# robustrobotics/flame

Measured on AMD Instinct MI355X. Metric: NLTGV2 primal-dual iters/sec on 640x480 Delaunay graph; depth RMS vs CPU, higher is better.
Workload: dtype f32

## Files before the change

flame_amd/csrc/flame_nltgv2_test_options.h:

```cpp
#ifndef FLAME_NLTGV2_TEST_OPTIONS_H_
#define FLAME_NLTGV2_TEST_OPTIONS_H_

enum {
  FLAME_NLTGV2_OPT_BLOCK_WAVES = 103,
  FLAME_NLTGV2_OPT_UNROLL = 104,
  FLAME_NLTGV2_OPT_DUAL_PUBLISH = 106,
  FLAME_NLTGV2_OPT_PRESLEEP = 108,
  FLAME_NLTGV2_OPT_XCDS = 109,
  FLAME_NLTGV2_OPT_FAULT_INJECT = 110,
  FLAME_NLTGV2_OPT_POLL_GAP = 113
};

#endif
```

flame_amd/csrc/nltgv2_context.hip:

```cpp
#include "nltgv2_context.hpp"

namespace flame_hip {
namespace host {

int fail(flame_nltgv2_ctx* ctx, int status) {
  if (ctx) ctx->last_error = status;
  return status;
}

void request_open_stop(flame_nltgv2_ctx* ctx) {
  if (!ctx->open_inflight || ctx->open_stop_sent || !ctx->stop_dev.p || !ctx->ctl_stream) return;
  *ctx->h_stop = ctx->open_tag0;
  if (hipMemcpyAsync(ctx->stop_dev.p, ctx->h_stop, sizeof(unsigned), hipMemcpyHostToDevice, ctx->ctl_stream) != hipSuccess) (void)hipGetLastError();
  ctx->open_stop_sent = true;
}

hipError_t wait_solver_stream(flame_nltgv2_ctx* ctx) {
  request_open_stop(ctx);
  return hipStreamSynchronize(ctx->stream);
}

int ensure(flame_nltgv2_ctx* ctx, DevBuf& b, size_t bytes) {
  if (bytes == 0) bytes = 16;
  if (b.cap >= bytes) return 0;
// ... 170 lines not shown
  const size_t lanes = (size_t)L.wg_count * kWave;
  const size_t fV = sizeof(float) * (size_t)V, fE = sizeof(float) * (size_t)E, iV = sizeof(int32_t) * (size_t)V;
  struct { DevBuf* b; size_t bytes; } req[] = {
      {&ctx->pos, 2 * fV}, {&ctx->src, fE}, {&ctx->dst, fE},
      {&ctx->row_ptr, sizeof(int32_t) * ((size_t)V + 1)}, {&ctx->half, 2 * fE},
      {&ctx->slice_row, sizeof(int32_t) * ((size_t)L.n_slices + 1)}, {&ctx->perm, sizeof(int32_t) * n_packed},
      {&ctx->pdeg, sizeof(int32_t) * n_packed}, {&ctx->iperm, iV}, {&ctx->order_m, iV}, {&ctx->rid_of, iV},
      {&ctx->rec_nbr, sizeof(uint32_t) * n_slots}, {&ctx->rec_edge, sizeof(int32_t) * n_slots}, {&ctx->edge_src_slot, fE},
      {&ctx->hrec, sizeof(int4) * n_slots}, {&ctx->hq, sizeof(float4) * n_slots},
      {&ctx->vstate, sizeof(float4) * n_packed}, {&ctx->vaux, sizeof(float2) * n_packed},
      {&ctx->hq_alt, sizeof(float4) * n_slots}, {&ctx->vstate_alt, sizeof(float4) * n_packed}, {&ctx->photo_err, fV},
      {&ctx->bar0, sizeof(float4) * n_packed}, {&ctx->bar1, sizeof(float4) * n_packed},
      {&ctx->vprev, sizeof(float4) * n_packed}, {&ctx->xbuf, kXbufBytesPerVertex * records_capacity(L) + 64},
      {&ctx->wg_v0, sizeof(int32_t) * n_wg_v0},
      {&ctx->wg_vfirst, n_wg_vfirst + 16}, {&ctx->abort_flag, sizeof(int)}, {&ctx->err, kErrBytes}, {&ctx->cost_out, 2 * sizeof(float)},
      {&ctx->wg_slot, sizeof(int32_t) * lanes}, {&ctx->wg_vid, sizeof(int32_t) * lanes}, {&ctx->wg_meta, sizeof(uint32_t) * lanes},
      {&ctx->wg_nbr, sizeof(int32_t) * lanes}, {&ctx->wg_fetch, sizeof(int32_t) * lanes},
      {&ctx->wg_info, sizeof(int32_t) * n_wg_info}};
  for (auto& r : req) {
    const int rc = ensure(ctx, *r.b, r.bytes);
    if (rc) return rc;
  }
  if (want_e2) {
    const size_t lanes2 = (size_t)L.wg2_count * kWave;
    struct { DevBuf* b; size_t bytes; } req2[] = {
        {&ctx->wg2_info, sizeof(int32_t) * n_wg2_info}, {&ctx->wg2_vfirst, n_wg2_vfirst + 16}, {&ctx->wg2_rmax, 64},
        {&ctx->wg2_slot, sizeof(int32_t) * 2 * lanes2}, {&ctx->wg2_nbr, sizeof(int32_t) * 2 * lanes2}, {&ctx->wg2_vid, sizeof(int32_t) * lanes2},
        {&ctx->wg2_meta, sizeof(uint32_t) * lanes2}, {&ctx->wg2_fetch, sizeof(int32_t) * lanes2}};
    for (auto& r : req2) {
      const int rc = ensure(ctx, *r.b, r.bytes);
      if (rc) return rc;
    }
  }
  ctx->topo++;
  ctx->layout_pos_saved = false;
  ctx->tv_built = ctx->wg2_built = false;
  drop_graphs(ctx);
  refresh_args(ctx);
  return 0;
}

void expansion_fills(const PackedLayout& L, void* rec_edge, void* rec_nbr, void* wg2_rmax, std::vector<StageFill>* fills) {
  fills->push_back(StageFill{(char*)rec_edge + sizeof(int32_t) * (size_t)L.rows * kWave, sizeof(int32_t) * kRowPad * kWave, 0xffffffffu});
  fills->push_back(StageFill{(char*)rec_nbr + sizeof(uint32_t) * (size_t)L.rows * kWave, sizeof(uint32_t) * kRowPad * kWave, 0u});
  if (wg2_rmax) fills->push_back(StageFill{wg2_rmax, 64, 0u});
}

void topology_fills(flame_nltgv2_ctx* ctx, bool want_e2, std::vector<StageFill>* fills, bool early) {
  const PackedLayout& L = ctx->L;
  const size_t n_slots = (size_t)(L.rows + kRowPad) * kWave, n_packed = (size_t)L.n_slices * kWave;
  const StageFill base[] = {
      {ctx->err.p, kErrBytes, 0u}, {ctx->abort_flag.p, sizeof(int), 0u}, {ctx->xbuf.p, kXbufBytesPerVertex * records_capacity(L) + 64, 0u},
      {ctx->hq_alt.p, sizeof(float4) * n_slots, 0u}, {ctx->vstate_alt.p, sizeof(float4) * n_packed, 0u}};
  fills->insert(fills->end(), base, base + sizeof(base) / sizeof(base[0]));
  if (!early) expansion_fills(L, ctx->rec_edge.p, ctx->rec_nbr.p, want_e2 ? ctx->wg2_rmax.p : nullptr, fills);
  if (ctx->place_base) {
    fills->push_back(StageFill{ctx->place_base, (size_t)2 * kPlacePages * 4096, 0u});
    fills->push_back(StageFill{(int*)ctx->place_fill.p + 2 * kPlacePages, 64, 0u});
  }
}

bool placement_applies(const flame_nltgv2_ctx* ctx, const PackedLayout& L) {
  return L.wg_ok && ctx->place_state == 1 && ctx->opt_place && L.wg_count > 2 * (ctx->prop.multiProcessorCount / 8) &&
         (ctx->opt_xcds == 0 || ctx->opt_xcds == 8);
}

ExpandTables live_tables(flame_nltgv2_ctx* ctx) {
  ExpandTables t;
  t.c = ctx->c, t.f = ctx->f;
  t.iperm = (const int32_t*)ctx->iperm.p, t.wg_v0 = (const int32_t*)ctx->wg_v0.p, t.order_m = (const int32_t*)ctx->order_m.p;
  t.rid_of = (const int32_t*)ctx->rid_of.p, t.wg_vfirst = (const uint8_t*)ctx->wg_vfirst.p;
  t.wg2_info = (int32_t*)ctx->wg2_info.p, t.wg2_vfirst = (const uint8_t*)ctx->wg2_vfirst.p;
  t.wg2_slot = (int32_t*)ctx->wg2_slot.p, t.wg2_vid = (int32_t*)ctx->wg2_vid.p, t.wg2_nbr = (int32_t*)ctx->wg2_nbr.p;
  t.wg2_fetch = (int32_t*)ctx->wg2_fetch.p, t.wg2_meta = (uint32_t*)ctx->wg2_meta.p, t.wg2_rmax = (int*)ctx->wg2_rmax.p;
  return t;
}

int expand_launches(flame_nltgv2_ctx* ctx, const PackedLayout& L, const ExpandTables& t, bool want_e2, hipStream_t stream) {
  LAUNCHCHK(ctx, launch_build_sell(t.c, t.f, t.iperm, stream));
  if (L.wg_ok) LAUNCHCHK(ctx, launch_build_patches(t.c, t.f, t.wg_v0, t.order_m, t.rid_of, t.wg_vfirst, t.iperm, stream));
  if (want_e2)
    LAUNCHCHK(ctx, launch_build_patches2(t.c, t.f, L.wg2_count, t.wg2_info, t.order_m, t.rid_of, t.wg2_vfirst, t.iperm, t.wg2_slot, t.wg2_vid,
                                         t.wg2_meta, t.wg2_nbr, t.wg2_fetch, t.wg2_rmax, stream));
  if (t.rec_off)
    LAUNCHCHK(ctx, launch_place_records(t.c, t.f, t.per_xcd, t.order_m, t.rid_of, t.place_patch, (int8_t*)(t.place_patch + t.stride),
                                        (const uint16_t*)ctx->place_rank.p, kPlacePages, t.place_fill, t.rec_off, (int)t.stride, stream));
  return 0;
}

int topology_expand(flame_nltgv2_ctx* ctx, bool want_e2, bool launched) {
  const PackedLayout& L = ctx->L;
  if (!launched) {
    const int rc = expand_launches(ctx, L, live_tables(ctx), want_e2, ctx->stream);
    if (rc) return rc;
  }
  ctx->pv2_args = Pv2Args{};
  ctx->wg2_usable = false;
  if (want_e2) {
    ctx->pv2_args.slot = (const int32_t*)ctx->wg2_slot.p, ctx->pv2_args.vid = (const int32_t*)ctx->wg2_vid.p;
    ctx->pv2_args.meta = (const uint32_t*)ctx->wg2_meta.p, ctx->pv2_args.nbr = (const int32_t*)ctx->wg2_nbr.p;
    ctx->pv2_args.fetch = (const int32_t*)ctx->wg2_fetch.p, ctx->pv2_args.info = (const int32_t*)ctx->wg2_info.p;
    ctx->pv2_args.count = L.wg2_count, ctx->pv2_args.lcap = L.wg2_lcap;
    if (ctx->pv2_occ == 0 || ctx->pv2_occ_lcap != L.wg2_lcap)
      ctx->pv2_occ = pv2_patches_per_cu(L.wg2_lcap, false), ctx->pv2_occ_verify = pv2_patches_per_cu(L.wg2_lcap, true), ctx->pv2_occ_lcap = L.wg2_lcap;
    ctx->wg2_built = true;
  }
  if (!launched && placement_applies(ctx, L)) {
    refresh_args(ctx);
    const int rc = place_records(ctx, (L.wg_count + 7) / 8);
    if (rc) return rc;
  }
  ctx->pending = flame_nltgv2_ctx::PendingRun{};
  ctx->tag_next = 1;
  ctx->xbuf_form = 0;
  ctx->static_stale = false;
  return 0;
}

bool wants_e2(const flame_nltgv2_ctx* ctx) { return wants_e2(ctx, ctx->L); }
bool wants_e2(const flame_nltgv2_ctx* ctx, const PackedLayout& L) {
  const int cus = ctx->prop.multiProcessorCount;
  const int64_t est_patches = L.wg_rowpack ? (int64_t)L.wg_count : ((static_cast<int64_t>(2) * L.E + L.V / 32) / 54 + 1);
  return L.wg_ok && L.max_degree <= 32 && ctx->opt_probe == 0 &&
         (ctx->opt_persistent == 6 || (ctx->opt_persistent == 1 && est_patches > (int64_t)kPv2FromPerCu * cus));
}

int upload_topology(flame_nltgv2_ctx* ctx, const flame_nltgv2_graph* g, const StageCopy* extra, size_t n_extra, bool long_lived) {
  const int32_t V = g->V, E = g->E;
  (void)long_lived;
  int rc = cancel_prepared(ctx);
  if (!rc) rc = wait_raster(ctx);
  if (rc) return rc;
  rc = build_layout(g, &ctx->L, false, true,
                        ctx->opt_persistent == 4 ? 0x7fffffff : kPvDensePerCu * ctx->prop.multiProcessorCount);
  if (rc) return fail(ctx, rc);
  if (ctx->L.wg_ok && ctx->L.wg_rowpack && ctx->opt_persistent != 4 && ctx->L.wg_count > kPvDensePerCu * ctx->prop.multiProcessorCount) {
    rc = build_layout(g, &ctx->L, false, false, 0);
    if (rc) return fail(ctx, rc);
  }
  bool want_e2 = wants_e2(ctx);
  if (want_e2) {
    build_patch_walk2(&ctx->L);
    want_e2 = ctx->L.wg2_ok && ctx->L.wg2_count <= kPv2WavesPerCu * ctx->prop.multiProcessorCount * 4;
  }
  const PackedLayout& L = ctx->L;
  rc = topology_buffers(ctx, want_e2, L.wg_info.size(), L.wg_v0.size(), L.wg_vfirst.size(), L.wg2_info.size(), L.wg2_vfirst.size());
  if (rc) return rc;
  const size_t n_packed = (size_t)L.n_slices * kWave;
  const size_t fV = sizeof(float) * (size_t)V, fE = sizeof(float) * (size_t)E, iV = sizeof(int32_t) * (size_t)V;
  std::vector<StageCopy> cp = {
      {&ctx->pos, g->pos, 2 * fV}, {&ctx->src, g->src, fE}, {&ctx->dst, g->dst, fE},
      {&ctx->row_ptr, L.row_ptr.data(), sizeof(int32_t) * ((size_t)V + 1)}, {&ctx->half, L.half.data(), 2 * fE},
      {&ctx->slice_row, L.slice_row.data(), sizeof(int32_t) * ((size_t)L.n_slices + 1)},
      {&ctx->perm, L.perm.data(), sizeof(int32_t) * n_packed}, {&ctx->pdeg, L.pdeg.data(), sizeof(int32_t) * n_packed},
      {&ctx->iperm, L.iperm.data(), iV}, {&ctx->order_m, L.order_m.data(), iV}, {&ctx->rid_of, L.rid_of.data(), iV},
      {&ctx->wg_info, L.wg_info.data(), sizeof(int32_t) * L.wg_info.size()},
      {&ctx->wg_v0, L.wg_v0.data(), sizeof(int32_t) * L.wg_v0.size()},
      {&ctx->wg_vfirst, L.wg_vfirst.data(), L.wg_vfirst.size()}};
  if (want_e2) {
    cp.push_back(StageCopy{&ctx->wg2_info, L.wg2_info.data(), sizeof(int32_t) * L.wg2_info.size()});
    cp.push_back(StageCopy{&ctx->wg2_vfirst, L.wg2_vfirst.data(), L.wg2_vfirst.size()});
  }
  cp.insert(cp.end(), extra, extra + n_extra);
  std::vector<StageFill> fills;
  topology_fills(ctx, want_e2, &fills);
  rc = staged_h2d(ctx, cp.data(), cp.size(), fills.data(), fills.size());
  if (rc) return rc;
  rc = topology_expand(ctx, want_e2);
  if (rc) return rc;
  ctx->h_src.assign(g->src, g->src + E);
  ctx->h_dst.assign(g->dst, g->dst + E);
  ctx->host_layout_valid = true;
  ctx->feat_dev_valid = false;
  HIPCHK(ctx, hipEventRecord(ctx->ev_topo_ready, ctx->stream));
  return 0;
}

int ensure_form_rows(flame_nltgv2_ctx* ctx, int form) {
  PackedLayout& L = ctx->L;
  if ((form == 4 && !ctx->wg2_built) || (form == 2 && !ctx->tv_built)) {
    const int rc = ensure_host_layout(ctx);
    if (rc) return rc;
  }
  if (form == 4 && !ctx->wg2_built) {
    build_patch_rows2(&L);
    ctx->pv2_args = Pv2Args{};
    if (L.wg2_ok) {
      struct { DevBuf* b; const void* src; size_t bytes; } cp[] = {
          {&ctx->wg2_slot, L.wg2_slot.data(), sizeof(int32_t) * L.wg2_slot.size()}, {&ctx->wg2_vid, L.wg2_vid.data(), sizeof(int32_t) * L.wg2_vid.size()},
          {&ctx->wg2_meta, L.wg2_meta.data(), sizeof(uint32_t) * L.wg2_meta.size()}, {&ctx->wg2_nbr, L.wg2_nbr.data(), sizeof(int32_t) * L.wg2_nbr.size()},
          {&ctx->wg2_fetch, L.wg2_fetch.data(), sizeof(int32_t) * L.wg2_fetch.size()}, {&ctx->wg2_info, L.wg2_info.data(), sizeof(int32_t) * L.wg2_info.size()}};
// ... 9 lines not shown
      ctx->pv2_args.count = L.wg2_count, ctx->pv2_args.lcap = L.wg2_lcap;
      ctx->pv2_occ = pv2_patches_per_cu(L.wg2_lcap, false), ctx->pv2_occ_verify = pv2_patches_per_cu(L.wg2_lcap, true), ctx->pv2_occ_lcap = L.wg2_lcap;
    }
    ctx->wg2_built = true;
    ctx->wg2_usable = L.wg2_ok, ctx->wg2_checked_topo = ctx->topo;
  }
  if (form == 2 && !ctx->tv_built) {
    build_tv_rows(&L);
    struct { DevBuf* b; const void* src; size_t bytes; } cp[] = {
        {&ctx->tv_slot, L.tv_slot.data(), sizeof(int32_t) * L.tv_slot.size()}, {&ctx->tv_vid, L.tv_vid.data(), sizeof(int32_t) * L.tv_vid.size()},
        {&ctx->tv_meta, L.tv_meta.data(), sizeof(uint32_t) * L.tv_meta.size()}, {&ctx->tv_wave, L.tv_wave.data(), sizeof(uint32_t) * L.tv_wave.size()}};
    HIPCHK(ctx, wait_solver_stream(ctx));
    for (auto& c : cp) {
      int rc = ensure(ctx, *c.b, c.bytes);
      if (!rc) rc = h2d(ctx, *c.b, c.src, c.bytes);
      if (rc) return rc;
    }
    HIPCHK(ctx, wait_solver_stream(ctx));
    ctx->tv_built = true;
    refresh_args(ctx);
  }
  return 0;
}

bool params_ok(const flame_nltgv2_params* p) { return p != nullptr; }

}
}

extern "C" {

int flame_nltgv2_abi_version(void) { return FLAME_NLTGV2_ABI_VERSION; }

void flame_nltgv2_default_params(flame_nltgv2_params* p) {
  if (!p) return;
  p->data_factor = 0.1f, p->step_x = 0.001f, p->step_q = 125.0f;
  p->theta = 0.25f, p->x_min = 0.0f, p->x_max = 10.0f;
}

const char* flame_nltgv2_status_string(int status) {
  switch (status) {
    case FLAME_NLTGV2_OK: return "ok";
    case FLAME_NLTGV2_ERR_INVALID_ARG: return "invalid argument";
    case FLAME_NLTGV2_ERR_NO_DEVICE: return "no usable HIP device";
    case FLAME_NLTGV2_ERR_HIP: return "HIP runtime error";
    case FLAME_NLTGV2_ERR_NO_GRAPH: return "no graph uploaded";
    case FLAME_NLTGV2_ERR_NAN: return "dual variable became NaN/Inf (reference FLAME_ASSERT, h:174)";
    case FLAME_NLTGV2_ERR_OOM: return "out of device memory";
    case FLAME_NLTGV2_ERR_TIMEOUT: return "persistent run: neighbour wait timed out";
    case FLAME_NLTGV2_ERR_ASSERT: return "input on which the reference asserts (FLAME_ASSERT)";
    default: return "unknown status";
  }
}

int flame_nltgv2_create(flame_nltgv2_ctx** out, int device) {
  if (!out) return FLAME_NLTGV2_ERR_INVALID_ARG;
  *out = nullptr;
  int count = 0;
  if (hipGetDeviceCount(&count) != hipSuccess || count <= 0) return FLAME_NLTGV2_ERR_NO_DEVICE;
  if (device < 0 || device >= count) return FLAME_NLTGV2_ERR_NO_DEVICE;
  flame_nltgv2_ctx* ctx = new (std::nothrow) flame_nltgv2_ctx();
  if (!ctx) return FLAME_NLTGV2_ERR_OOM;
  ctx->device = device;
  bool ok = hipSetDevice(device) == hipSuccess;
  ok = ok && hipGetDeviceProperties(&ctx->prop, device) == hipSuccess;
  int prio_least = 0, prio_greatest = 0;
  ok = ok && hipDeviceGetStreamPriorityRange(&prio_least, &prio_greatest) == hipSuccess;
  ok = ok && hipStreamCreateWithPriority(&ctx->own_stream, hipStreamNonBlocking, prio_greatest) == hipSuccess;
  ok = ok && hipEventCreate(&ctx->ev0) == hipSuccess && hipEventCreate(&ctx->ev1) == hipSuccess;
  ok = ok && hipStreamCreateWithFlags(&ctx->topo_stream, hipStreamNonBlocking) == hipSuccess;
  ok = ok && hipStreamCreateWithFlags(&ctx->raster_stream, hipStreamNonBlocking) == hipSuccess;
  ok = ok && hipEventCreateWithFlags(&ctx->ev_canon, hipEventDisableTiming) == hipSuccess;
  ok = ok && hipEventCreateWithFlags(&ctx->ev_snap, hipEventDisableTiming) == hipSuccess;
  ok = ok && hipEventCreateWithFlags(&ctx->ev_raster_done, hipEventDisableTiming) == hipSuccess;
  ok = ok && hipEventCreateWithFlags(&ctx->ev_topo_ready, hipEventDisableTiming) == hipSuccess;
  ok = ok && hipEventCreate(&ctx->ev_mesh0) == hipSuccess && hipEventCreate(&ctx->ev_mesh1) == hipSuccess;
  ok = ok && hipEventCreate(&ctx->ev_dbg0) == hipSuccess && hipEventCreate(&ctx->ev_dbg1) == hipSuccess;
  ok = ok && hipEventCreateWithFlags(&ctx->ev_expanded, hipEventDisableTiming) == hipSuccess;
  ok = ok && hipEventCreateWithFlags(&ctx->ev_run[0], hipEventDisableTiming) == hipSuccess;
  ok = ok && hipEventCreateWithFlags(&ctx->ev_run[1], hipEventDisableTiming) == hipSuccess;
  ok = ok && hipHostMalloc((void**)&ctx->h_err, kErrBytes, hipHostMallocDefault) == hipSuccess;
  ok = ok && hipHostMalloc((void**)&ctx->h_cost, 2 * sizeof(float), hipHostMallocDefault) == hipSuccess;
  ok = ok && hipHostMalloc((void**)&ctx->h_stop, 64, hipHostMallocDefault) == hipSuccess;
  if (ctx->h_stop) *ctx->h_stop = 0u;
  ok = ok && hipStreamCreateWithPriority(&ctx->ctl_stream, hipStreamNonBlocking, -1) == hipSuccess;
  if (!ok) {
    flame_nltgv2_destroy(ctx);
    return FLAME_NLTGV2_ERR_HIP;
  }
  ctx->stream = ctx->own_stream;
  *ctx->h_err = 0;
  {
    static std::once_flag warm;
    if (!std::getenv("FLAME_NLTGV2_NO_WARM"))
    std::call_once(warm, [ctx] {
      warm_module_kernels(), warm_module_persistent(ctx->own_stream, cooperative_allowed()), warm_module_persistent_tv(), warm_module_persistent_pv2();
      warm_module_layout(), warm_module_topo();
    });
    if (!std::getenv("FLAME_NLTGV2_LAZY_CALIBRATION") && ctx->prop.multiProcessorCount >= 64 && place_calibrate_at_create(device) && place_calibrate(ctx) != 0) {
      ctx->last_error = 0, ctx->last_hip = 0;
      (void)hipGetLastError();
    }
    if (ctx->place_state < 0) ctx->place_state = 0;
  }
  ctx->all = {&ctx->pos, &ctx->x, &ctx->w1, &ctx->w2, &ctx->xb, &ctx->w1b, &ctx->w2b, &ctx->xp, &ctx->w1p,
              &ctx->w2p, &ctx->data, &ctx->weight, &ctx->src, &ctx->dst, &ctx->alpha, &ctx->beta, &ctx->q1,
              &ctx->q2, &ctx->q3, &ctx->row_ptr, &ctx->half, &ctx->slice_row, &ctx->perm, &ctx->pdeg,
              &ctx->rec_nbr, &ctx->rec_edge, &ctx->edge_src_slot, &ctx->hrec, &ctx->hq, &ctx->vstate, &ctx->hq_alt, &ctx->vstate_alt, &ctx->cost_terms, &ctx->run_tail,
              &ctx->vaux, &ctx->bar0, &ctx->bar1, &ctx->vprev, &ctx->xbuf, &ctx->abort_flag, &ctx->tv_slot, &ctx->tv_vid, &ctx->tv_meta, &ctx->tv_wave, &ctx->wg2_slot, &ctx->wg2_vid, &ctx->wg2_meta, &ctx->wg2_nbr, &ctx->wg2_fetch, &ctx->wg2_info, &ctx->wg2_vfirst, &ctx->wg2_rmax, &ctx->err,
              &ctx->cost_out, &ctx->img_ref, &ctx->img_cmp, &ctx->photo_err, &ctx->r_tris, &ctx->r_valid, &ctx->r_tvalid, &ctx->r_keys,
              &ctx->r_img, &ctx->r_cov, &ctx->r_vtx, &ctx->r_val, &ctx->wg_slot, &ctx->wg_vid, &ctx->wg_meta, &ctx->wg_nbr,
              &ctx->wg_fetch, &ctx->wg_info, &ctx->wg_v0, &ctx->probe, &ctx->snap_hq, &ctx->snap_vstate, &ctx->snap_bar, &ctx->iperm,
              &ctx->order_m, &ctx->rid_of, &ctx->stage[0].d, &ctx->stage[1].d, &ctx->sync_init, &ctx->sync_vmap, &ctx->sync_emap, &ctx->sync_need,
              &ctx->wg_vfirst, &ctx->place_pool, &ctx->place_rank, &ctx->place_fill, &ctx->place_rec_off, &ctx->place_patch, &ctx->place_meas, &ctx->progress};
  for (DevBuf* b : {&ctx->feat_stamp_d, &ctx->feat_key_d, &ctx->feat_val_d, &ctx->topo_scratch, &ctx->topo_dims, &ctx->layout_pos}) ctx->all.push_back(b);
  for (auto& b : ctx->nx) ctx->all.push_back(&b);
  for (auto& b : ctx->ex) ctx->all.push_back(&b);
  ctx->all.push_back(&ctx->pos_undo);
  for (DevBuf* b : {&ctx->m_P, &ctx->m_idepth, &ctx->m_normals, &ctx->m_tvalid, &ctx->m_nvalid, &ctx->m_tnormal, &ctx->m_offset, &ctx->m_cursor,
                    &ctx->m_incident, &ctx->m_keys, &ctx->m_img, &ctx->m_cov})
    ctx->all.push_back(b);
  for (DevBuf* b : {&ctx->d_gray, &ctx->d_idimg, &ctx->d_nimg, &ctx->d_w1map, &ctx->d_w2map, &ctx->d_keys, &ctx->d_cov}) ctx->all.push_back(b);
  ctx->all.push_back(&ctx->stop_dev);
  ctx->all.push_back(&ctx->place_patch_nx), ctx->all.push_back(&ctx->place_fill_nx);
  for (auto& b : ctx->sp_v) ctx->all.push_back(&b);
  for (auto& b : ctx->sp_q) ctx->all.push_back(&b);
  for (auto& b : ctx->sp_ab) ctx->all.push_back(&b);
  *out = ctx;
  return FLAME_NLTGV2_OK;
}

int flame_nltgv2_destroy(flame_nltgv2_ctx* ctx) {
  if (!ctx) return FLAME_NLTGV2_OK;
  (void)hipSetDevice(ctx->device);
  request_open_stop(ctx);
  if (ctx->stream) (void)hipStreamSynchronize(ctx->stream);
  place_pool_release(ctx);
  drop_graphs(ctx);
  for (DevBuf* b : ctx->all)
    if (b->p) (void)hipFree(b->p);
  if (ctx->h_err) (void)hipHostFree(ctx->h_err);
  if (ctx->h_cost) (void)hipHostFree(ctx->h_cost);
  if (ctx->h_keep) (void)hipHostFree(ctx->h_keep);
  if (ctx->h_stop) (void)hipHostFree(ctx->h_stop);
  if (ctx->ctl_stream) (void)hipStreamSynchronize(ctx->ctl_stream), (void)hipStreamDestroy(ctx->ctl_stream);
  for (auto& st : ctx->stage)
    if (st.h) (void)hipHostFree(st.h);
  if (ctx->topo_stream) (void)hipStreamSynchronize(ctx->topo_stream), (void)hipStreamDestroy(ctx->topo_stream);
  if (ctx->ev_topo_ready) (void)hipEventDestroy(ctx->ev_topo_ready);
  if (ctx->ev_expanded) (void)hipEventDestroy(ctx->ev_expanded);
  if (ctx->raster_stream) (void)hipStreamSynchronize(ctx->raster_stream), (void)hipStreamDestroy(ctx->raster_stream);
  if (ctx->ev_canon) (void)hipEventDestroy(ctx->ev_canon);
  if (ctx->ev_snap) (void)hipEventDestroy(ctx->ev_snap);
  if (ctx->ev_raster_done) (void)hipEventDestroy(ctx->ev_raster_done);
  for (hipEvent_t e : ctx->ev_run)
    if (e) (void)hipEventDestroy(e);
  if (ctx->h_img) (void)hipHostFree(ctx->h_img);
  if (ctx->h_mesh) (void)hipHostFree(ctx->h_mesh);
  if (ctx->ev_mesh0) (void)hipEventDestroy(ctx->ev_mesh0);
  if (ctx->ev_mesh1) (void)hipEventDestroy(ctx->ev_mesh1);
  if (ctx->h_dbg) (void)hipHostFree(ctx->h_dbg);
  if (ctx->ev_dbg0) (void)hipEventDestroy(ctx->ev_dbg0);
  if (ctx->ev_dbg1) (void)hipEventDestroy(ctx->ev_dbg1);
  if (ctx->h_dims) (void)hipHostFree(ctx->h_dims);
  if (ctx->ev0) (void)hipEventDestroy(ctx->ev0);
  if (ctx->ev1) (void)hipEventDestroy(ctx->ev1);
  if (ctx->own_stream) (void)hipStreamDestroy(ctx->own_stream);
  delete ctx;
  return FLAME_NLTGV2_OK;
}

int flame_nltgv2_set_stream(flame_nltgv2_ctx* ctx, void* hip_stream) {
  int rc = enter(ctx);
  if (rc) return rc;
  HIPCHK(ctx, wait_solver_stream(ctx));
  ctx->stream = hip_stream ? (hipStream_t)hip_stream : ctx->own_stream;
  return FLAME_NLTGV2_OK;
}

int flame_nltgv2_set_option(flame_nltgv2_ctx* ctx, int option, int value) {
  if (!ctx) return FLAME_NLTGV2_ERR_INVALID_ARG;
  switch (option) {
    case FLAME_NLTGV2_OPT_SOLVER:
      if (value != 0 && value != 1) return fail(ctx, FLAME_NLTGV2_ERR_INVALID_ARG);
      ctx->opt_solver = value;
      return 0;
    case FLAME_NLTGV2_OPT_USE_HIPGRAPH:
      ctx->opt_use_graph = value ? 1 : 0;
      return 0;
    case FLAME_NLTGV2_OPT_BLOCK_WAVES:
      if (value != 0 && value != 1 && value != 2 && value != 4) return fail(ctx, FLAME_NLTGV2_ERR_INVALID_ARG);
      ctx->opt_block_waves = value;
      return 0;
    case FLAME_NLTGV2_OPT_PERSISTENT:
      if (value < 0 || value > 6 || value == 2 || value == 5) return fail(ctx, FLAME_NLTGV2_ERR_INVALID_ARG);
      ctx->opt_persistent = value;
      return 0;
    case FLAME_NLTGV2_OPT_PLACEMENT:
      if (value < 0 || value > 1) return fail(ctx, FLAME_NLTGV2_ERR_INVALID_ARG);
      ctx->opt_place = value;
      return 0;
    case FLAME_NLTGV2_OPT_POLL_GAP:
      if (value < 0 || value > 256) return fail(ctx, FLAME_NLTGV2_ERR_INVALID_ARG);
      ctx->opt_poll_gap = value;
      return 0;
    case FLAME_NLTGV2_OPT_VERIFY_RECORDS:
      if (value < 0 || value > 2) return fail(ctx, FLAME_NLTGV2_ERR_INVALID_ARG);
      ctx->opt_verify = value;
      if (value != 2) ctx->persist_refused_topo = ctx->persist_backoff_topo = ~0ull;
      return 0;
    case FLAME_NLTGV2_OPT_PROBE:
      ctx->opt_probe = value ? 1 : 0;
      return 0;
    case FLAME_NLTGV2_OPT_DUAL_PUBLISH:
      if (value < 0 || value > 2) return fail(ctx, FLAME_NLTGV2_ERR_INVALID_ARG);
      ctx->opt_dual = value;
      return 0;
    case FLAME_NLTGV2_OPT_FAULT_INJECT:
      if (value < 0 || value > (1 << 24)) return fail(ctx, FLAME_NLTGV2_ERR_INVALID_ARG);
      ctx->opt_fault = value;
      if (value == 0) ctx->persist_refused_topo = ctx->persist_backoff_topo = ~0ull;
      return 0;
    case FLAME_NLTGV2_OPT_XCDS:
      if (value < 0 || value > 8) return fail(ctx, FLAME_NLTGV2_ERR_INVALID_ARG);
      ctx->opt_xcds = value;
      ctx->coop_checked_key = ~0ull;
      return 0;
    case FLAME_NLTGV2_OPT_PRESLEEP:
      if (value < 0 || value > 256) return fail(ctx, FLAME_NLTGV2_ERR_INVALID_ARG);
      ctx->opt_presleep = value;
      return 0;
    case FLAME_NLTGV2_OPT_MESH_STATE:
      if (value < 0 || value > 1) return fail(ctx, FLAME_NLTGV2_ERR_INVALID_ARG);
      ctx->opt_mesh_state = value;
      return 0;
    case FLAME_NLTGV2_OPT_COST_SUM:
      if (value < 0 || value > 1) return fail(ctx, FLAME_NLTGV2_ERR_INVALID_ARG);
      ctx->opt_cost_sum = value;
      return 0;
    case FLAME_NLTGV2_OPT_SYNC_PATH:
      if (value < 0 || value > 2) return fail(ctx, FLAME_NLTGV2_ERR_INVALID_ARG);
      ctx->opt_sync_path = value;
      return 0;
    case FLAME_NLTGV2_OPT_UNROLL:
      if (value != 0 && value != 4 && value != 8 && value != 16) return fail(ctx, FLAME_NLTGV2_ERR_INVALID_ARG);
      ctx->opt_unroll = value;
      return 0;
    default:
      return fail(ctx, FLAME_NLTGV2_ERR_INVALID_ARG);
  }
}


int flame_nltgv2_get_info(flame_nltgv2_ctx* ctx, flame_nltgv2_info* info) {
  if (!ctx || !info) return FLAME_NLTGV2_ERR_INVALID_ARG;
  std::memset(info, 0, sizeof(*info));
  info->abi_version = FLAME_NLTGV2_ABI_VERSION;
  info->device = ctx->device;
  info->V = ctx->L.V, info->E = ctx->L.E;
  info->n_slices = ctx->L.n_slices;
  info->max_degree = ctx->L.max_degree;
  info->padded_half_edges = ctx->L.rows * kWave;
  info->device_bytes = (int64_t)ctx->device_bytes;
  info->algorithmic_bytes_per_iter = 64ll * ctx->L.V + 40ll * ctx->L.E;
  info->compute_units = ctx->prop.multiProcessorCount;
  std::snprintf(info->device_name, sizeof(info->device_name), "%s", ctx->prop.name);
  std::snprintf(info->gcn_arch, sizeof(info->gcn_arch), "%s", ctx->prop.gcnArchName);
  info->last_run_path = ctx->last_run_path;
  info->he_waves = 0;
  if (ctx->have_graph && !ctx->tv_built && ctx->tv_counted_topo != ctx->topo) {
    if (ensure_host_layout(ctx) == 0) {
      ctx->L.tv_waves = 0;
      build_tv_rows(&ctx->L);
      ctx->tv_counted_topo = ctx->topo;
    }
  }
  info->tv_waves = ctx->L.tv_ok ? ctx->L.tv_waves : 0;
  info->patches = ctx->L.wg_ok ? ctx->L.wg_count : 0;
  info->tv_wave_capacity = kTvLdsWavesPerCu * ctx->prop.multiProcessorCount;
  info->last_run_groups = ctx->last_run_groups;
  info->timeouts_recovered = ctx->timeouts_recovered;
  info->torn_records_detected = ctx->torn_records_detected;
  info->last_sync_path = ctx->last_sync_path;
// ... 31 lines not shown
  rc = ensure_canon(ctx);
  if (!rc) rc = ensure_host_layout(ctx);
  if (rc) return rc;
  const int32_t V = ctx->L.V, E = ctx->L.E;
  std::vector<float> pos(2 * (size_t)V);
  HIPCHK(ctx, hipMemcpyAsync(pos.data(), ctx->layout_pos_saved ? ctx->layout_pos.p : ctx->pos.p, sizeof(float) * pos.size(), hipMemcpyDeviceToHost, ctx->stream));
  HIPCHK(ctx, wait_solver_stream(ctx));
  flame_nltgv2_graph g{};
  g.V = V, g.E = E, g.pos = pos.data(), g.src = ctx->h_src.data(), g.dst = ctx->h_dst.data();
  PackedLayout H;
  rc = build_layout(&g, &H, true, ctx->L.wg_rowpack);
  if (rc) return fail(ctx, rc);
  int64_t bad = 0;
  auto cmp = [&](const DevBuf& b, const void* host, size_t bytes) -> int {
    if (bytes == 0) return 0;
    std::vector<uint32_t> d(bytes / 4);
    if (hipMemcpy(d.data(), b.p, bytes, hipMemcpyDeviceToHost) != hipSuccess) return 1;
    const uint32_t* h = static_cast<const uint32_t*>(host);
    for (size_t i = 0; i < d.size(); ++i) bad += d[i] != h[i];
    return 0;
  };
  const PackedLayout& L = ctx->L;
  bad += (H.rows != L.rows) + (H.n_slices != L.n_slices) + (H.wg_ok != L.wg_ok) + (H.wg_count != L.wg_count) +
         (H.wg_lcap != L.wg_lcap) + (H.wg_slab_slots != L.wg_slab_slots) + (H.n_rec != L.n_rec) +
         (H.wg_v0 != L.wg_v0) + (H.wg_vfirst != L.wg_vfirst) + (H.wg_rowpack != L.wg_rowpack);
  if (bad == 0) {
    const size_t iV = 4 * (size_t)V;
    int e = cmp(ctx->row_ptr, H.row_ptr.data(), iV + 4) | cmp(ctx->half, H.half.data(), 8 * (size_t)E) | cmp(ctx->order_m, H.order_m.data(), iV) |
            cmp(ctx->rid_of, H.rid_of.data(), iV) | cmp(ctx->iperm, H.iperm.data(), iV) | cmp(ctx->pdeg, H.pdeg.data(), 4 * H.pdeg.size()) |
            cmp(ctx->wg_v0, H.wg_v0.data(), 4 * H.wg_v0.size()) | cmp(ctx->wg_vfirst, H.wg_vfirst.data(), H.wg_vfirst.size() & ~size_t(3));
    if (e) return fail(ctx, FLAME_NLTGV2_ERR_HIP);
    std::vector<int32_t> hs(ctx->h_src.size()), hd(ctx->h_dst.size());
    if (E && (hipMemcpy(hs.data(), ctx->src.p, 4 * (size_t)E, hipMemcpyDeviceToHost) != hipSuccess ||
              hipMemcpy(hd.data(), ctx->dst.p, 4 * (size_t)E, hipMemcpyDeviceToHost) != hipSuccess))
      return fail(ctx, FLAME_NLTGV2_ERR_HIP);
    bad += (hs != ctx->h_src) + (hd != ctx->h_dst);
  }
  if (bad == 0) {
    const size_t n = (size_t)L.rows * kWave, lanes = (size_t)L.wg_count * kWave;
    int e = cmp(ctx->rec_nbr, H.rec_nbr.data(), 4 * n) | cmp(ctx->rec_edge, H.rec_edge.data(), 4 * n) |
            cmp(ctx->edge_src_slot, H.edge_src_slot.data(), 4 * (size_t)E) | cmp(ctx->perm, H.perm.data(), 4 * H.perm.size()) |
            cmp(ctx->slice_row, H.slice_row.data(), 4 * H.slice_row.size());
    if (L.wg_ok)
      e |= cmp(ctx->wg_slot, H.wg_slot.data(), 4 * lanes) | cmp(ctx->wg_vid, H.wg_vid.data(), 4 * lanes) |
           cmp(ctx->wg_meta, H.wg_meta.data(), 4 * lanes) | cmp(ctx->wg_nbr, H.wg_nbr.data(), 4 * lanes) |
           cmp(ctx->wg_fetch, H.wg_fetch.data(), 4 * lanes) | cmp(ctx->wg_info, H.wg_info.data(), 4 * H.wg_info.size());
    if (ctx->wg2_built) {
      build_patch_rows2(&H);
      bad += (H.wg2_ok != L.wg2_ok) + (H.wg2_count != L.wg2_count) + (H.wg2_lcap != L.wg2_lcap) + (H.wg2_vfirst != L.wg2_vfirst);
      if (bad == 0 && H.wg2_ok) {
        const size_t lanes2 = (size_t)H.wg2_count * kWave;
        e |= cmp(ctx->wg2_slot, H.wg2_slot.data(), 8 * lanes2) | cmp(ctx->wg2_nbr, H.wg2_nbr.data(), 8 * lanes2) |
             cmp(ctx->wg2_vid, H.wg2_vid.data(), 4 * lanes2) | cmp(ctx->wg2_meta, H.wg2_meta.data(), 4 * lanes2) |
             cmp(ctx->wg2_fetch, H.wg2_fetch.data(), 4 * lanes2) | cmp(ctx->wg2_info, H.wg2_info.data(), 4 * H.wg2_info.size());
      }
    }
    if (e) return fail(ctx, FLAME_NLTGV2_ERR_HIP);
  }
  if (bad == 0 && ctx->place_state == 1 && ctx->place_topo == ctx->topo && L.wg_ok) {
    const size_t stride = records_capacity(L);
    std::vector<int32_t> off(2 * stride);
    if (hipMemcpy(off.data(), ctx->place_rec_off.p, sizeof(int32_t) * off.size(), hipMemcpyDeviceToHost) != hipSuccess)
      return fail(ctx, FLAME_NLTGV2_ERR_HIP);
    std::vector<int32_t> patch_of_rec((size_t)V, -1);
    for (int32_t q = 0; q < H.wg_count; ++q)
      for (int32_t i = 0; i < (H.wg_info[(size_t)q * 4 + 2] & 0xffff); ++i) patch_of_rec[(size_t)H.wg_info[(size_t)q * 4] + i] = q;
    const int32_t per = ctx->place_per_xcd;
    for (int par = 0; par < 2; ++par) {
      std::vector<int32_t> used;
      for (int32_t u = 0; u < V; ++u) {
        const int32_t r = H.rid_of[(size_t)u], a = patch_of_rec[(size_t)r] / per;
        bool crosses = false;
        for (int32_t h = H.row_ptr[(size_t)u]; h < H.row_ptr[(size_t)u + 1] && !crosses; ++h)
          crosses = patch_of_rec[(size_t)H.rid_of[(size_t)H.half_nbr[(size_t)h]]] / per != a;
        const int32_t o = off[(size_t)par * stride + r];
        bad += crosses != (o >= 0);
        if (o < 0) continue;
        bad += (o & 15) != 0 || o < par * kPlacePages * 4096 || o >= (par + 1) * kPlacePages * 4096;
        used.push_back(o);
      }
      std::sort(used.begin(), used.end());
      for (size_t i = 1; i < used.size(); ++i) bad += used[i] == used[i - 1];
    }
  }
  *mismatches = bad;
  return FLAME_NLTGV2_OK;
}

int flame_nltgv2_placement_info(flame_nltgv2_ctx* ctx, int32_t* state, int32_t* placed_records, float* us) {
  int rc = enter(ctx);
  if (rc) return rc;
  if (state) *state = ctx->place_state;
  if (us) us[0] = ctx->place_best_us, us[1] = ctx->place_mean_us, us[2] = ctx->place_worst_us;
  if (placed_records) {
    *placed_records = 0;
    if (ctx->have_graph && ctx->place_state == 1 && ctx->place_topo == ctx->topo) {
      std::vector<int32_t> off((size_t)ctx->L.V);
      HIPCHK(ctx, hipMemcpyAsync(off.data(), ctx->place_rec_off.p, sizeof(int32_t) * off.size(), hipMemcpyDeviceToHost, ctx->stream));
      HIPCHK(ctx, wait_solver_stream(ctx));
      for (int32_t o : off) *placed_records += o >= 0;
    }
  }
  return FLAME_NLTGV2_OK;
}

int flame_nltgv2_pack_probe(const flame_nltgv2_graph* g, int32_t* perm, int32_t* slice_row, int32_t* rec_nbr,
                            int32_t* rec_edge, int64_t capacity_rows, int64_t* rows_out) {
  PackedLayout L;
  int rc = build_layout(g, &L);
  if (rc) return rc;
  if (rows_out) *rows_out = L.rows;
  if (perm) std::memcpy(perm, L.perm.data(), sizeof(int32_t) * L.perm.size());
  if (slice_row) std::memcpy(slice_row, L.slice_row.data(), sizeof(int32_t) * L.slice_row.size());
  if ((rec_nbr || rec_edge) && capacity_rows < L.rows) return FLAME_NLTGV2_ERR_INVALID_ARG;
  const size_t n = (size_t)L.rows * kWave;
  if (rec_nbr) std::memcpy(rec_nbr, L.rec_nbr.data(), sizeof(int32_t) * n);
  if (rec_edge) std::memcpy(rec_edge, L.rec_edge.data(), sizeof(int32_t) * n);
  return L.n_slices;
}

}
```

flame_amd/csrc/nltgv2_context.hpp:

```cpp
#ifndef FLAME_AMD_NLTGV2_CONTEXT_HPP_
#define FLAME_AMD_NLTGV2_CONTEXT_HPP_

#include <hip/hip_runtime.h>

#include <cstdio>
#include <cstdlib>
#include <cstring>
#include <algorithm>
#include <chrono>
#include <cmath>
#include <new>
#include <memory>
#include <mutex>
#include <functional>
#include <vector>

#include "flame_nltgv2.h"
#include "flame_nltgv2_test_options.h"
#include "nltgv2_kernels.h"
#include "nltgv2_pack.hpp"
#include "roctx_ranges.hpp"

namespace flame_hip {
namespace host {

constexpr int kGraphChunk = 256;
constexpr int kMaxCachedGraphs = 6;
constexpr int kTvLdsWavesPerCu = 16;
constexpr size_t kXbufBytesPerVertex = 8 * 16 + 4;
constexpr int kPv2FromPerCu = 14;
constexpr int kPv2PaceAbovePerCu = 10, kPv2DensePreSleep = 2, kPv2DenseGap = 2;
constexpr int kPv2MaxGroups = 2;
constexpr int kPv2WavesPerCu = 19;
constexpr int kCrowdedWavesPerCu = 16, kCrowdedTopologies = 64;
constexpr int kPvDensePerCu = 27;
constexpr int kPvPaceAbovePerCu = 13;
constexpr int kPvDensePreSleep = 3, kPvDenseGap = 2;
constexpr int kPvPaceMoreAbovePerCu = 23;
constexpr int kPvDenserPreSleep = 5, kPvDenserGap = 4;
constexpr int kPvPreSleep = 0;
constexpr int kPvPollGap = 2;
constexpr int kDualMinWavesPerCu = 0;
constexpr int kPreSleepTv = 2;
constexpr int32_t kFeatDirectMax = 1 << 22;
constexpr size_t kErrBytes = 16 * sizeof(int);
constexpr unsigned kMaxSpins = 1u << 20;

struct DevBuf {
  void* p = nullptr;
  size_t cap = 0;
};

struct CachedGraph {
  hipGraphExec_t exec = nullptr;
  int n = 0, parity = 0, unroll = 0, wpb = 0, gen = 0;
  uint64_t topo = 0;
  flame_nltgv2_params params{};
  uint64_t stamp = 0;
};

class FlatMap {
 public:
  FlatMap() = default;
  explicit FlatMap(size_t n) { reset(n); }
  void reset(size_t n) {
    size_t cap = 16;
    while (cap < 2 * n + 2) cap <<= 1;
    if (cap > slots_.size() || gen_ == 0xffffffffu) {
      slots_.assign(std::max(cap, slots_.size()), Slot{0, 0, 0});
      gen_ = 0;
    }
    mask_ = slots_.size() - 1;
    ++gen_;
  }
  std::pair<int32_t*, bool> emplace(uint64_t k, int32_t v) {
    size_t i = hash(k) & mask_;
    for (;; i = (i + 1) & mask_) {
      Slot& s = slots_[i];
      if (s.gen != gen_) {
        s = Slot{k, v, gen_};
        return {&s.val, true};
      }
      if (s.key == k) return {&s.val, false};
    }
  }
  const int32_t* find(uint64_t k) const {
    size_t i = hash(k) & mask_;
    for (;; i = (i + 1) & mask_) {
      const Slot& s = slots_[i];
      if (s.gen != gen_) return nullptr;
      if (s.key == k) return &s.val;
    }
  }

 private:
  struct Slot {
    uint64_t key;
    int32_t val;
    uint32_t gen;
  };
  static size_t hash(uint64_t z) {
    z = (z ^ (z >> 30)) * 0xbf58476d1ce4e5b9ull;
    z = (z ^ (z >> 27)) * 0x94d049bb133111ebull;
    return (size_t)(z ^ (z >> 31));
  }
  size_t mask_ = 0;
  uint32_t gen_ = 0;
  std::vector<Slot> slots_;
};

}
}

using namespace flame_hip;
using namespace flame_hip::host;

struct flame_nltgv2_ctx {
  int device = 0;
  hipStream_t own_stream = nullptr;
  hipStream_t stream = nullptr;
  hipEvent_t ev0 = nullptr, ev1 = nullptr;
  int last_error = 0;
  int last_hip = 0;
  hipDeviceProp_t prop{};

  bool have_graph = false;
  bool canon_valid = false, fused_valid = false, have_prev = false;
  DevBuf sp_v[9], sp_q[3], sync_init, sync_vmap, sync_emap, sync_need;
  DevBuf sp_ab[2];
  std::vector<int32_t> h_old_of_new, h_old_of_new_edge, h_old_edge_of_pair, h_first_pair_of_old, h_bucket_start, h_bucket_item, h_bucket_at;
  FlatMap feat_maps[3];
  int feat_cur = 0;
  bool feat_map_valid = false;
  std::vector<int32_t> feat_tab;
  std::vector<uint32_t> feat_stamp;
  uint32_t feat_stamp_now = 0;
  bool feat_tab_valid = false;
  int parity = 0;
  uint64_t topo = 0, stamp = 0;

  int opt_solver = 0, opt_use_graph = 1, opt_block_waves = 0, opt_unroll = 0, opt_persistent = 1, opt_dual = 1;
  int xbuf_form = 0;
  int opt_xcds = 0;
  bool photo_fused = false;
  PhotoGeometry photo_geo{};
  float photo_scale = 1.0f;
  int photo_border = 3;
  bool photo_fresh = false;
  float* export_ptr = nullptr;
  float export_scale = 1.0f;
  int opt_fault = 0;
  int opt_presleep = 0;
  int opt_poll_gap = 0;
  mutable int pv_occ = 0;
  mutable uint64_t pv_occ_topo = ~0ull;
  int opt_probe = 0;
  size_t probe_words = 0;
  uint32_t tag_next = 1;
  int last_run_path = 0, last_run_groups = 0;
  uint64_t persist_refused_topo = ~0ull;
  uint64_t persist_backoff_topo = ~0ull;
  int persist_backoff_left = 0, persist_timeout_streak = 0;
  int replaying = 0;
  uint64_t crowded_until_topo = 0;
  int last_run_waves_per_cu = 0;
  bool static_stale = false;
  uint64_t coop_checked_key = 0;
  int buf_gen = 0;
  int replay_attempt = 0;
  int replays_per_step = 0;
  int timeouts_recovered = 0;
  int torn_records_detected = 0;
  int opt_verify = 0;
  int opt_place = 1;
  int place_state = 0;
  uint64_t place_topo = ~0ull;
  int place_per_xcd = 0;
  char* place_base = nullptr;
  float place_best_us = 0.0f, place_mean_us = 0.0f, place_worst_us = 0.0f;
  DevBuf place_pool, place_rank, place_fill, place_rec_off, place_patch, place_meas;
  std::vector<uint16_t> place_rank_host;
  struct PendingOp {
    int kind = 0;
    flame_nltgv2_params params{};
    int n = 0;
    bool open = false;
    uint32_t tag0 = 0;
    float* dst = nullptr;
    float scale = 1.0f;
  };
  struct PendingRun {
    bool active = false;
    bool snapshotted = false;
    int parity_before = 0;
    bool have_prev_before = false;
    std::vector<PendingOp> ops;
  } pending;
  DevBuf snap_hq, snap_vstate, snap_bar;
  DevBuf iperm, order_m, rid_of;
  bool tv_built = false;
  bool wg2_built = false;
  Pv2Args pv2_args;
  int pv2_occ_lcap = -1;
  int pv2_occ = 0, pv2_occ_verify = 0;
  uint64_t wg2_checked_topo = ~0ull;
  bool wg2_usable = false;
  struct StageSlot {
    void* h = nullptr;
    size_t cap = 0;
    DevBuf d;
  } stage[2];

  PackedLayout L;
  std::vector<int32_t> h_src, h_dst, h_feat;
  DevBuf layout_pos;
  bool layout_pos_saved = false;
  bool host_layout_valid = true;
  uint64_t tv_counted_topo = ~0ull;
  int opt_mesh_state = 0;
  uint64_t snap_topo = ~0ull;
  hipEvent_t ev_snap = nullptr;
  int opt_cost_sum = 0;
  int opt_sync_path = 0;
  int last_sync_path = 0;
  DevBuf feat_stamp_d, feat_key_d, feat_val_d, topo_scratch, topo_dims;
  std::vector<int32_t> dup_key;
  std::vector<uint32_t> dup_stamp;
  uint32_t dup_now = 0;
  enum { NX_POS, NX_SRC, NX_DST, NX_ROW_PTR, NX_HALF, NX_ORDER_M, NX_RID_OF, NX_PERM, NX_IPERM, NX_PDEG, NX_SLICE_ROW, NX_WG_INFO, NX_WG_V0,
         NX_WG_VFIRST, NX_WG2_INFO, NX_WG2_VFIRST, NX_DATA, NX_WEIGHT, NX_COUNT };
  DevBuf nx[NX_COUNT];
  DevBuf* nx_live(int i) {
    DevBuf* const live[NX_COUNT] = {&pos, &src, &dst, &row_ptr, &half, &order_m, &rid_of, &perm, &iperm, &pdeg, &slice_row, &wg_info, &wg_v0,
                                    &wg_vfirst, &wg2_info, &wg2_vfirst, &data, &weight};
    return live[i];
  }
  enum { EX_REC_NBR, EX_REC_EDGE, EX_EDGE_SRC_SLOT, EX_WG_SLOT, EX_WG_VID, EX_WG_META, EX_WG_NBR, EX_WG_FETCH, EX_WG2_SLOT, EX_WG2_NBR,
         EX_WG2_VID, EX_WG2_META, EX_WG2_FETCH, EX_WG2_RMAX, EX_PLACE_REC_OFF, EX_COUNT };
  DevBuf ex[EX_COUNT];
  DevBuf* ex_live(int i) {
    DevBuf* const live[EX_COUNT] = {&rec_nbr, &rec_edge, &edge_src_slot, &wg_slot, &wg_vid, &wg_meta, &wg_nbr, &wg_fetch, &wg2_slot, &wg2_nbr,
                                    &wg2_vid, &wg2_meta, &wg2_fetch, &wg2_rmax, &place_rec_off};
    return live[i];
  }
  DevBuf place_patch_nx, place_fill_nx;
  hipEvent_t ev_expanded = nullptr;
  std::vector<char> prep_host;
  const void *prep_vmap = nullptr, *prep_emap = nullptr, *prep_init = nullptr;
  hipStream_t raster_stream = nullptr;
  hipEvent_t ev_canon = nullptr, ev_raster_done = nullptr;
  bool raster_inflight = false;
  float* h_img = nullptr;
  size_t h_img_cap = 0;
  int map_rows = 0, map_cols = 0;
  int img_pending_rows = 0, img_pending_cols = 0;
  int32_t tris_T = -1;
  uint64_t tris_topo = ~0ull;
  DevBuf m_P, m_idepth, m_normals, m_tvalid, m_nvalid, m_tnormal, m_offset, m_cursor, m_incident, m_keys, m_img, m_cov;
  char* h_mesh = nullptr;
  size_t h_mesh_cap = 0;
  struct MeshPending {
    bool active = false;
    int32_t V = 0, T = 0;
    int rows = 0, cols = 0;
// ... 57 lines not shown
  unsigned* h_stop = nullptr;
  DevBuf stop_dev;
  hipStream_t ctl_stream = nullptr;
  bool open_inflight = false;
  bool open_stop_sent = false;
  uint32_t open_tag0 = 0;
  int want_open = 0;
  int last_open_iters = 0;
  int64_t iters_total = 0;
  DevBuf pos_undo;
  size_t h_keep_cap = 0;
  std::vector<CachedGraph> graphs;
  size_t device_bytes = 0;
};

#define HIPCHK(ctx, expr)                              \
  do {                                                 \
    hipError_t _e = (expr);                            \
    if (_e != hipSuccess) {                            \
      (ctx)->last_hip = (int)_e;                       \
      (ctx)->last_error = FLAME_NLTGV2_ERR_HIP;        \
      return FLAME_NLTGV2_ERR_HIP;                     \
    }                                                  \
  } while (0)

#define LAUNCHCHK(ctx, expr)                           \
  do {                                                 \
    int _e = (expr);                                   \
    if (_e != 0) {                                     \
      (ctx)->last_hip = _e;                            \
      (ctx)->last_error = FLAME_NLTGV2_ERR_HIP;        \
      return FLAME_NLTGV2_ERR_HIP;                     \
    }                                                  \
  } while (0)

namespace flame_hip {
namespace host {

int fail(flame_nltgv2_ctx* ctx, int status);
int ensure(flame_nltgv2_ctx* ctx, DevBuf& b, size_t bytes);
void drop_graphs(flame_nltgv2_ctx* ctx);
SolverParams to_sp(const flame_nltgv2_params* p);
int enter(flame_nltgv2_ctx* ctx);
void refresh_args(flame_nltgv2_ctx* ctx);
int h2d(flame_nltgv2_ctx* ctx, DevBuf& b, const void* src, size_t bytes);
size_t records_capacity(const PackedLayout& L);
int wait_raster(flame_nltgv2_ctx* ctx);
enum { kBehindNotLaunched = 0, kBehindDone = 1, kBehindSpoiled = 2 };
int ensure_canon(flame_nltgv2_ctx* ctx, const std::function<int()>* behind = nullptr, int* behind_state = nullptr);
void request_open_stop(flame_nltgv2_ctx* ctx);
hipError_t wait_solver_stream(flame_nltgv2_ctx* ctx);
int ensure_fused(flame_nltgv2_ctx* ctx);
bool params_ok(const flame_nltgv2_params* p);
struct StageCopy {
  DevBuf* b;
  const void* src;
  size_t bytes;
};
struct StageFill {
  void* dst;
  size_t bytes;
  uint32_t word;
};
int staged_h2d(flame_nltgv2_ctx* ctx, const StageCopy* cp, size_t n, const StageFill* fills = nullptr, size_t n_fills = 0, int slot = 0,
               hipStream_t stream = nullptr, size_t* host_off = nullptr);
int upload_topology(flame_nltgv2_ctx* ctx, const flame_nltgv2_graph* g, const StageCopy* extra, size_t n_extra, bool long_lived);
int topology_buffers(flame_nltgv2_ctx* ctx, bool want_e2, size_t n_wg_info, size_t n_wg_v0, size_t n_wg_vfirst, size_t n_wg2_info,
                     size_t n_wg2_vfirst);
struct ExpandTables {
  CanonArgs c;
  FusedArgs f;
  const int32_t *iperm = nullptr, *wg_v0 = nullptr, *order_m = nullptr, *rid_of = nullptr;
  const uint8_t* wg_vfirst = nullptr;
  int32_t* wg2_info = nullptr;
  const uint8_t* wg2_vfirst = nullptr;
  int32_t *wg2_slot = nullptr, *wg2_vid = nullptr, *wg2_nbr = nullptr, *wg2_fetch = nullptr;
  uint32_t* wg2_meta = nullptr;
  int* wg2_rmax = nullptr;
  int32_t* rec_off = nullptr;
  int32_t* place_patch = nullptr;
  int* place_fill = nullptr;
  int per_xcd = 0;
  size_t stride = 0;
};
ExpandTables live_tables(flame_nltgv2_ctx* ctx);
bool placement_applies(const flame_nltgv2_ctx* ctx, const PackedLayout& L);
void topology_fills(flame_nltgv2_ctx* ctx, bool want_e2, std::vector<StageFill>* fills, bool early = false);
void expansion_fills(const PackedLayout& L, void* rec_edge, void* rec_nbr, void* wg2_rmax, std::vector<StageFill>* fills);
int expand_launches(flame_nltgv2_ctx* ctx, const PackedLayout& L, const ExpandTables& t, bool want_e2, hipStream_t stream);
int topology_expand(flame_nltgv2_ctx* ctx, bool want_e2, bool launched = false);
bool wants_e2(const flame_nltgv2_ctx* ctx);
bool wants_e2(const flame_nltgv2_ctx* ctx, const PackedLayout& L);
int ensure_host_layout(flame_nltgv2_ctx* ctx);
int topo_prepare(flame_nltgv2_ctx* ctx, const flame_nltgv2_sync_input* in, bool* applicable);
int topo_upload(flame_nltgv2_ctx* ctx, const flame_nltgv2_graph* g, const StageCopy* extra, size_t n_extra, bool* done);
int topo_commit(flame_nltgv2_ctx* ctx, bool* done);
int cancel_prepared(flame_nltgv2_ctx* ctx);
int sync_graph_host(flame_nltgv2_ctx* ctx, const flame_nltgv2_sync_input* in);
void set_init_map(flame_nltgv2_ctx* ctx, bool on, SyncArgs* sa);
int ensure_form_rows(flame_nltgv2_ctx* ctx, int form);

constexpr size_t kMaxChain = 256;
bool persistent_eligible(flame_nltgv2_ctx* ctx, int n);
int prepare_run(flame_nltgv2_ctx* ctx, const flame_nltgv2_params* p, int n);
PhotoFuse photo_target(const flame_nltgv2_ctx* ctx);
struct PhotoStale {
  flame_nltgv2_ctx* ctx;
  ~PhotoStale() { ctx->photo_fresh = false; }
};
int enqueue_photo_sweep(flame_nltgv2_ctx* ctx, bool packed_current);
int enqueue_run(flame_nltgv2_ctx* ctx, const flame_nltgv2_params* p, int n);
int finish(flame_nltgv2_ctx* ctx, bool unpack_behind = false, bool* unpacked = nullptr, const std::function<int()>* behind = nullptr,
           bool* behind_launched = nullptr);
int snapshot_chain_start(flame_nltgv2_ctx* ctx);
int place_records(flame_nltgv2_ctx* ctx, int per_xcd);
int place_calibrate(flame_nltgv2_ctx* ctx);
void place_pool_release(flame_nltgv2_ctx* ctx);
bool cooperative_allowed();
bool place_calibrate_at_create(int device);

}
}

#endif
```

flame_amd/csrc/nltgv2_kernels.h:

```cpp
#pragma once

#include <hip/hip_runtime.h>
#include <hip/hip_ext.h>
#include <stdint.h>

namespace flame_hip {

struct SolverParams {
  float data_factor, step_x, step_q, theta, x_min, x_max;
};

struct PhotoGeometry {
  float KRKinv[9];
  float Kt[3];
};

struct PhotoFuse {
  const float2* pos = nullptr;
  const uint8_t* ref = nullptr;
  const uint8_t* cmp = nullptr;
  float* err = nullptr;
  PhotoGeometry geo{};
  float graph_scale = 1.0f;
  int rows = 0, cols = 0, step = 0, border = 0;
};

struct RunTail {
  float* export_out = nullptr;
  float export_scale = 1.0f;
  int reserved_ = 0;
  PhotoFuse photo;
  unsigned* progress = nullptr;
  const unsigned* stop_req = nullptr;
};

struct ProjectGeometry {
  float K[9], Kinv[9], KRKinv[9];
  float q[4];
  float t[3];
  float rx, ry, rw, rh;
};

struct CanonArgs {
  int V = 0, E = 0;
  float2* pos = nullptr;
  float *x = nullptr, *w1 = nullptr, *w2 = nullptr;
  float *xb = nullptr, *w1b = nullptr, *w2b = nullptr;
  float *xp = nullptr, *w1p = nullptr, *w2p = nullptr;
  float *data = nullptr, *weight = nullptr;
  int32_t *src = nullptr, *dst = nullptr;
  float *alpha = nullptr, *beta = nullptr;
  float *q1 = nullptr, *q2 = nullptr, *q3 = nullptr;
  int32_t* row_ptr = nullptr;
  uint32_t* half = nullptr;
  int* err = nullptr;
};

struct FusedArgs {
  hipEvent_t stop_event = nullptr;
  int open_run = 0;
  int n_slices = 0;
  int64_t n_slots = 0;
  int32_t* slice_row = nullptr;
  int32_t* perm = nullptr;
  int32_t* pdeg = nullptr;
  uint32_t* rec_nbr = nullptr;
  int32_t* rec_edge = nullptr;
  int32_t* edge_src_slot = nullptr;
  int4* hrec = nullptr;
  float4* hq = nullptr;
  float4* vstate = nullptr;
  float4* hq_out = nullptr;
  float4* vstate_out = nullptr;
  float2* vaux = nullptr;
  float4* bar[2] = {nullptr, nullptr};
  float4* vprev = nullptr;
  void* xbuf = nullptr;
  int tv_waves = 0;
  int32_t* tv_slot = nullptr;
  int32_t* tv_vid = nullptr;
  uint32_t* tv_meta = nullptr;
  uint32_t* tv_wave = nullptr;
  int wg_count = 0, wg_lcap = 0, wg_slab_slots = 0;
  int wg_rowpack = 0;
  int32_t* wg_slot = nullptr;
  int32_t* wg_vid = nullptr;
  uint32_t* wg_meta = nullptr;
  int32_t* wg_nbr = nullptr;
  int32_t* wg_fetch = nullptr;
  int32_t* wg_info = nullptr;
  int n_rec = 0;
  int wg_poll_gap = 1;
  char* place_pool = nullptr;
  const int32_t* rec_off = nullptr;
  int rec_off_stride = 0;
  unsigned* rot_word = nullptr;
  unsigned* probe = nullptr;
  int* abort_flag = nullptr;
  int* err = nullptr;
};
inline int persistent_rec_bytes(const FusedArgs& a) { return (a.n_rec > a.n_slices * 64 ? a.n_rec : a.n_slices * 64) * 16; }

int launch_fused_step(const FusedArgs& a, const SolverParams& p, int parity, bool write_prev, int unroll,
                      int waves_per_block, hipStream_t stream);
int launch_persistent_run(const FusedArgs& a, const SolverParams& p, int form, int wave_begin, int n_waves,
                          int parity_in, unsigned tag0, int n_iters, int waves_per_block, unsigned max_spins,
                          int presleep, int dual, int xcds, const RunTail* tail, bool cooperative,
                          hipStream_t stream);
constexpr int kPlacePages = 96;
int launch_place_calibrate(char* pool, int n_pages, int iters, unsigned* out, int* xcc_out, int* fail, hipStream_t s);
int launch_place_records(const CanonArgs& c, const FusedArgs& a, int per_xcd, const int32_t* order_m, const int32_t* rid_of,
                         int32_t* patch_of_rec, int8_t* cls, const uint16_t* ranking, int n_pages, int* fill, int32_t* rec_off,
                         int stride, hipStream_t s);
constexpr uint32_t kScatterFill = 0xffffffffu;
struct ScatterEntry {
  void* dst;
  uint32_t src_off;
  uint32_t fill;
  size_t bytes;
};
constexpr int kScatterMax = 48;
struct ScatterTable {
  int n = 0;
  ScatterEntry e[kScatterMax];
};
int launch_scatter(const ScatterTable& t, const void* blob, hipStream_t s);
struct CopyTable {
  int n = 0;
  struct { void* dst; const void* src; size_t bytes; } e[4];
};
int launch_copy_arrays(const CopyTable& t, hipStream_t s);
struct SyncArgs {
  int V = 0, E = 0;
  const int32_t* old_of_new = nullptr;
  const int32_t* old_of_new_edge = nullptr;
  const float* data = nullptr;
  const float* weight = nullptr;
  const float* init_x = nullptr;
  const float* init_map = nullptr;
  int map_rows = 0, map_cols = 0;
  int check_sticky = 0;
  float sticky_threshold = 0.0f;
  float graph_scale = 0.0f;
  const float* o[9] = {};
  float* n[9] = {};
  const float* oq[3] = {};
  float* nq[3] = {};
  const int32_t *src = nullptr, *dst = nullptr, *row_ptr = nullptr;
  const uint32_t* half = nullptr;
  const float2* pos = nullptr;
  float *alpha = nullptr, *beta = nullptr;
  uint8_t* need_nbr = nullptr;
};
int launch_sync_state(const SyncArgs& a, hipStream_t s);
int pv_patches_per_cu(const FusedArgs& a, bool verify);
struct Pv2Args {
  const int32_t* slot = nullptr;
  const int32_t* vid = nullptr;
  const uint32_t* meta = nullptr;
  const int32_t* nbr = nullptr;
  const int32_t* fetch = nullptr;
  const int32_t* info = nullptr;
  int count = 0, lcap = 0;
};
int launch_build_patches2(const CanonArgs& c, const FusedArgs& a, int n_patches, int32_t* wg_info, const int32_t* order_m, const int32_t* rid_tab,
                          const uint8_t* vfirst, const int32_t* iperm, int32_t* wg_slot, int32_t* wg_vid, uint32_t* wg_meta, int32_t* wg_nbr,
                          int32_t* wg_fetch, int* rmax, hipStream_t s);
int pv2_patches_per_cu(int lcap, bool verify);
int launch_persistent_pv2(const FusedArgs& a, const Pv2Args& w, const SolverParams& p, int wg_begin, int n_wgs, int parity_in, unsigned tag0,
                          int n_iters, unsigned max_spins, int poll_gap, int dual, const RunTail* tail, bool cooperative, hipStream_t stream);
int pv_real_waves_per_simd(bool verify_or_probe);
const void* persistent_tv_kernel(int waves_per_block, unsigned* lds_bytes);
int launch_build_sell(const CanonArgs& c, const FusedArgs& a, const int32_t* iperm, hipStream_t s);
int launch_build_patches(const CanonArgs& c, const FusedArgs& a, const int32_t* wg_v0, const int32_t* order_m,
                         const int32_t* rid_tab, const uint8_t* vfirst, const int32_t* iperm, hipStream_t s);
struct TopoDims {
  int32_t n_edges;
  int32_t n_keep;
  int32_t rows;
  int32_t max_degree;
  int32_t wg_count, wg_lcap;
  int32_t wg2_count, wg2_lcap;
  int32_t flags;
  int32_t pad_[7];
};
constexpr int32_t kTopoBadDegree = 1;
constexpr int32_t kTopoBadEdges = 2;
constexpr int kTopoInf = 0x7f7f7f7f;
struct TopoBuild {
  int V = 0, E = 0;
  int Vo = 0, Eo = 0;
  int n_slices = 0;
  const int32_t* fid = nullptr;
  const float2* pos = nullptr;
// ... 69 lines not shown
```

flame_amd/csrc/nltgv2_layout.hip:

```cpp
#include <hip/hip_runtime.h>
#include <stdint.h>

#include "nltgv2_kernels.h"

namespace flame_hip {

namespace {

constexpr uint32_t kRole = 0x80000000u;
constexpr uint32_t kWgTail = 1u << 24, kWgActive = 1u << 25, kWgValid = 1u << 26, kWgPublish = 1u << 27, kWgHead = 1u << 28;

__global__ void __launch_bounds__(256)
k_build_sell(const int n_packed, const int32_t* __restrict__ perm, const int32_t* __restrict__ slice_row,
             const int32_t* __restrict__ row_ptr, const uint32_t* __restrict__ half, const int32_t* __restrict__ src,
             const int32_t* __restrict__ dst, const int32_t* __restrict__ iperm, uint32_t* __restrict__ rec_nbr,
             int32_t* __restrict__ rec_edge, int32_t* __restrict__ edge_src_slot) {
  const int p = blockIdx.x * blockDim.x + threadIdx.x;
  if (p >= n_packed) return;
  const int s = p >> 6, l = p & 63;
  const int row0 = slice_row[s], row1 = slice_row[s + 1];
  const int o = perm[p];
  int base = 0, deg = 0;
  if (o >= 0) {
    base = row_ptr[o];
// ... 200 lines not shown
      int lo = 0, hi = n_list - 1;
      while (lo < hi) {
        const int mid = (lo + hi) >> 1;
        if (s_list[mid] < cand[sl]) lo = mid + 1; else hi = mid;
      }
      nbr[sl] = (int)(0x80000000u | (unsigned)lo);
    }
    wg_slot[hl2 + (size_t)sl * 64] = slot[sl];
    wg_nbr[hl2 + (size_t)sl * 64] = nbr[sl];
  }
  if (j >= 0 && s_pub[j]) meta |= kWgPublish;
  wg_vid[hl] = vid, wg_meta[hl] = meta;
  if (lane == 0) {
    wg_info[4 * p + 1] = n_fetch;
    if (n_fetch > 64) atomicMax(rmax, n_fetch);
  }
}

__device__ __forceinline__ unsigned place_xcc_id() {
  unsigned v;
  asm volatile("s_getreg_b32 %0, hwreg(HW_REG_XCC_ID)" : "=s"(v));
  return v & 15u;
}

__global__ void __launch_bounds__(64)
k_place_calibrate(char* pool, const int n_pages, const int iters, unsigned* __restrict__ out, int* __restrict__ xcc_out,
                  int* fail) {
  const int b = blockIdx.x, x = b & 7, j = b >> 3;
  if (threadIdx.x == 0) xcc_out[b] = (int)place_xcc_id();
  if (j == 0) return;
  const int pb = ((8 - j) & 7) * 8 + ((x + j) & 7);
  const bool first = b < pb;
  const int line = (first ? b : pb) * 64;
  const __amdgpu_buffer_rsrc_t r = __builtin_amdgcn_make_buffer_rsrc(pool, 0, 0x7fffffff, 0x00020000);
  typedef int v4i_t __attribute__((ext_vector_type(4)));
  int tag = 0;
  bool dead = false;
  unsigned stamp = 0;
  auto wait_tag = [&](const int off, const int want) {
    for (unsigned spin = 0; spin < (1u << 17); ++spin) {
      int o = off;
      asm volatile("" : "+v"(o)::"memory");
      const v4i_t g = __builtin_amdgcn_raw_buffer_load_b128(r, o, 0, 16);
      if (g.w == want) {
        stamp = (unsigned)g.x;
        return true;
      }
      if ((spin & 1023u) == 1023u && __hip_atomic_load(fail, __ATOMIC_RELAXED, __HIP_MEMORY_SCOPE_AGENT) != 0) break;
    }
    return false;
  };
  for (int pg = 0; pg < n_pages && !dead; ++pg) {
    const int mine = pg * 4096 + line + (first ? 0 : 16), theirs = pg * 4096 + line + (first ? 16 : 0);
    unsigned sum = 0;
    for (int it = 0; it < iters + 2; ++it) {
      ++tag;
      if (!first) {
        if (!wait_tag(theirs, tag)) {
          dead = true;
          break;
        }
        if (it >= 2) sum += (unsigned)wall_clock64() - stamp;
      }
      const v4i_t rec = {(int)(unsigned)wall_clock64(), 0, 0, tag};
      __builtin_amdgcn_raw_buffer_store_b128(rec, r, mine, 0, 16);
      if (first) {
        if (!wait_tag(theirs, tag)) {
          dead = true;
          break;
        }
        if (it >= 2) sum += (unsigned)wall_clock64() - stamp;
      }
    }
    if (threadIdx.x == 0) out[(size_t)b * n_pages + pg] = dead ? 0u : sum;
  }
  if (dead && threadIdx.x == 0) __hip_atomic_store(fail, 1, __ATOMIC_RELAXED, __HIP_MEMORY_SCOPE_AGENT);
}

__global__ void __launch_bounds__(256)
k_place_patch_of_record(const int n_patches, const int32_t* __restrict__ wg_info, int32_t* __restrict__ patch_of_rec,
                        int32_t* __restrict__ rec_off, const int stride, int* __restrict__ fill, const int n_fill) {
  const int p = blockIdx.x * blockDim.x + threadIdx.x;
  if (p < n_fill) fill[p] = 0;
  if (p < 128) fill[n_fill + 16 + p] = 0;
  if (p >= n_patches) return;
  const int r0 = wg_info[4 * p], n = wg_info[4 * p + 2] & 0xffff;
  for (int i = 0; i < n; ++i) patch_of_rec[r0 + i] = p, rec_off[r0 + i] = -1, rec_off[stride + r0 + i] = -1;
}

__global__ void __launch_bounds__(256)
k_place_classify(const int V, const int per_xcd, const int32_t* __restrict__ order_m, const int32_t* __restrict__ rid_of,
                 const int32_t* __restrict__ row_ptr, const uint32_t* __restrict__ half, const int32_t* __restrict__ src,
                 const int32_t* __restrict__ dst, const int32_t* __restrict__ patch_of_rec, int8_t* __restrict__ cls) {
  const int r = blockIdx.x * blockDim.x + threadIdx.x;
  if (r >= V) return;
  const int o = order_m[r];
  const int a = patch_of_rec[r] / per_xcd;
  int c = -1;
  for (int h = row_ptr[o]; h < row_ptr[o + 1] && c < 0; ++h) {
    const uint32_t hh = half[h];
    const int e = (int)(hh & ~kRole);
    const int other = (hh & kRole) ? src[e] : dst[e];
    const int xb = patch_of_rec[rid_of[other]] / per_xcd;
    if (xb != a) c = a * 8 + xb;
  }
  cls[r] = (int8_t)c;
}

__global__ void __launch_bounds__(64)
k_place_assign(const int n_patches, const int32_t* __restrict__ wg_info, const int8_t* __restrict__ cls_of_rec,
               const uint16_t* __restrict__ ranking, const int n_pages, int* __restrict__ fill, int32_t* __restrict__ rec_off,
               const int stride) {
  const int p = blockIdx.x, lane = threadIdx.x;
  if (p >= n_patches) return;
  const int r0 = wg_info[4 * p], n = min(wg_info[4 * p + 2] & 0xffff, 64);
  const int c_mine = lane < n ? (int)cls_of_rec[r0 + lane] : -1;
  unsigned long long todo = __ballot(c_mine >= 0);
  while (todo) {
    const int leader = __ffsll((long long)todo) - 1;
    const int c = __shfl(c_mine, leader, 64);
    const unsigned long long members = __ballot(c_mine == c);
    todo &= ~members;
    const int m = __popcll(members);
    const int m8 = (m + 7) & ~7;
    for (int par = 0; par < 2; ++par) {
      int base = -1;
      if (lane == leader) {
        const uint16_t* const rk = ranking + ((size_t)par * 64 + c) * n_pages;
        int* const cursor = fill + 2 * n_pages + 16 + par * 64 + c;
        for (int t = __hip_atomic_load(cursor, __ATOMIC_RELAXED, __HIP_MEMORY_SCOPE_AGENT); t < n_pages && base < 0; ++t) {
          const int pg = rk[t];
          const int s0 = atomicAdd(&fill[par * n_pages + pg], m8);
          if (s0 + m8 <= 256) base = (par * n_pages + pg) * 4096 + s0 * 16;
          else atomicMax(cursor, t + 1);
        }
      }
      base = __shfl(base, leader, 64);
      if (c_mine == c && base >= 0)
        rec_off[(size_t)par * stride + r0 + lane] = base + 16 * __popcll(members & ((1ull << lane) - 1ull));
    }
  }
}

inline dim3 grid1d(long n, int block = 256) { return dim3((unsigned)((n + block - 1) / block)); }

}


int launch_build_sell(const CanonArgs& c, const FusedArgs& a, const int32_t* iperm, hipStream_t s) {
  const int n_packed = a.n_slices * 64;
  if (n_packed <= 0) return 0;
  hipLaunchKernelGGL(k_build_sell, grid1d(n_packed), dim3(256), 0, s, n_packed, a.perm, a.slice_row, c.row_ptr, c.half,
                     c.src, c.dst, iperm, a.rec_nbr, a.rec_edge, a.edge_src_slot);
  return (int)hipGetLastError();
}

int launch_place_calibrate(char* pool, int n_pages, int iters, unsigned* out, int* xcc_out, int* fail, hipStream_t s) {
  hipLaunchKernelGGL(k_place_calibrate, dim3(64), dim3(64), 0, s, pool, n_pages, iters, out, xcc_out, fail);
  return (int)hipGetLastError();
}

int launch_place_records(const CanonArgs& c, const FusedArgs& a, int per_xcd, const int32_t* order_m, const int32_t* rid_of,
                         int32_t* patch_of_rec, int8_t* cls, const uint16_t* ranking, int n_pages, int* fill, int32_t* rec_off,
                         int stride, hipStream_t s) {
  if (a.wg_count <= 0 || per_xcd <= 0) return 0;
  const int n0 = a.wg_count > 2 * n_pages ? a.wg_count : 2 * n_pages;
  hipLaunchKernelGGL(k_place_patch_of_record, grid1d(n0), dim3(256), 0, s, a.wg_count, a.wg_info, patch_of_rec, rec_off, stride, fill,
                     2 * n_pages);
  hipLaunchKernelGGL(k_place_classify, grid1d(c.V), dim3(256), 0, s, c.V, per_xcd, order_m, rid_of, c.row_ptr, c.half, c.src, c.dst,
                     patch_of_rec, cls);
  hipLaunchKernelGGL(k_place_assign, dim3((unsigned)a.wg_count), dim3(64), 0, s, a.wg_count, a.wg_info, cls, ranking, n_pages, fill, rec_off,
                     stride);
  return (int)hipGetLastError();
}

int launch_build_patches2(const CanonArgs& c, const FusedArgs& a, int n_patches, int32_t* wg_info, const int32_t* order_m, const int32_t* rid_tab,
                          const uint8_t* vfirst, const int32_t* iperm, int32_t* wg_slot, int32_t* wg_vid, uint32_t* wg_meta, int32_t* wg_nbr,
                          int32_t* wg_fetch, int* rmax, hipStream_t s) {
  if (n_patches <= 0) return 0;
  hipLaunchKernelGGL(k_build_patch2, dim3((unsigned)n_patches), dim3(64), 0, s, n_patches, wg_info, order_m, rid_tab, vfirst, iperm,
                     a.slice_row, c.row_ptr, c.half, c.src, c.dst, wg_slot, wg_vid, wg_meta, wg_nbr, wg_fetch, rmax);
  return (int)hipGetLastError();
}

int launch_build_patches(const CanonArgs& c, const FusedArgs& a, const int32_t* wg_v0, const int32_t* order_m,
                         const int32_t* rid_tab, const uint8_t* vfirst, const int32_t* iperm, hipStream_t s) {
  if (a.wg_count <= 0) return 0;
  hipLaunchKernelGGL(k_build_patch, dim3((unsigned)a.wg_count), dim3(64), 0, s, a.wg_count, a.wg_info, wg_v0, order_m, rid_tab, vfirst,
                     c.V, iperm, a.slice_row, c.row_ptr, c.half, c.src, c.dst, a.wg_slot, a.wg_vid, a.wg_meta, a.wg_nbr,
                     a.wg_fetch);
  return (int)hipGetLastError();
}

}

namespace flame_hip {
namespace {
__global__ void __launch_bounds__(256) k_scatter(const ScatterTable t, const uint8_t* __restrict__ blob) {
  const ScatterEntry e = t.e[blockIdx.y];
  const size_t n16 = e.bytes >> 4;
  uint4* __restrict__ d16 = static_cast<uint4*>(e.dst);
  const size_t stride = (size_t)gridDim.x * blockDim.x;
  const size_t i0 = (size_t)blockIdx.x * blockDim.x + threadIdx.x;
  if (e.src_off == kScatterFill) {
    const uint4 v = make_uint4(e.fill, e.fill, e.fill, e.fill);
    for (size_t i = i0; i < n16; i += stride) d16[i] = v;
    uint32_t* d4 = static_cast<uint32_t*>(e.dst);
    for (size_t i = (n16 << 2) + i0; i < (e.bytes >> 2); i += stride) d4[i] = e.fill;
  } else {
    const uint4* __restrict__ s16 = reinterpret_cast<const uint4*>(blob + e.src_off);
    for (size_t i = i0; i < n16; i += stride) d16[i] = s16[i];
    uint32_t* d4 = static_cast<uint32_t*>(e.dst);
    const uint32_t* s4 = reinterpret_cast<const uint32_t*>(blob + e.src_off);
    for (size_t i = (n16 << 2) + i0; i < (e.bytes >> 2); i += stride) d4[i] = s4[i];
    if (i0 == 0)
      for (size_t b = e.bytes & ~size_t(3); b < e.bytes; ++b) static_cast<uint8_t*>(e.dst)[b] = blob[e.src_off + b];
  }
}
}

namespace {
__global__ void __launch_bounds__(256) k_copy_arrays(const CopyTable t) {
  const uint4* __restrict__ src = static_cast<const uint4*>(t.e[blockIdx.y].src);
  uint4* __restrict__ dst = static_cast<uint4*>(t.e[blockIdx.y].dst);
  const size_t n16 = t.e[blockIdx.y].bytes >> 4, stride = (size_t)gridDim.x * blockDim.x;
  for (size_t i = (size_t)blockIdx.x * blockDim.x + threadIdx.x; i < n16; i += stride) dst[i] = src[i];
}
}

int launch_copy_arrays(const CopyTable& t, hipStream_t s) {
  if (t.n <= 0) return 0;
  size_t mx = 0;
  for (int i = 0; i < t.n; ++i) mx = t.e[i].bytes > mx ? t.e[i].bytes : mx;
  unsigned gx = (unsigned)((mx / 16 + 4 * 256 - 1) / (4 * 256));
  gx = gx < 1 ? 1 : (gx > 512 ? 512 : gx);
  hipLaunchKernelGGL(k_copy_arrays, dim3(gx, (unsigned)t.n), dim3(256), 0, s, t);
  return (int)hipGetLastError();
}

int launch_scatter(const ScatterTable& t, const void* blob, hipStream_t s) {
  if (t.n <= 0) return 0;
  size_t mx = 0;
  for (int i = 0; i < t.n; ++i) mx = t.e[i].bytes > mx ? t.e[i].bytes : mx;
  unsigned gx = (unsigned)((mx / 16 + 4 * 256 - 1) / (4 * 256));
  gx = gx < 1 ? 1 : (gx > 256 ? 256 : gx);
  hipLaunchKernelGGL(k_scatter, dim3(gx, (unsigned)t.n), dim3(256), 0, s, t, static_cast<const uint8_t*>(blob));
  return (int)hipGetLastError();
}
}

namespace flame_hip {
namespace {

// ... 108 lines not shown
```

flame_amd/csrc/nltgv2_persistent.hip:

```cpp
#include "nltgv2_persistent_common.hpp"

namespace flame_hip {

namespace {


template <bool PROBE, bool VERIFY, bool OPEN = false>
__global__ void __launch_bounds__(64) __attribute__((amdgpu_num_sgpr(92)))
k_persistent_pv(const int wg_begin, const int n_wgs, const int wgs_per_xcd, const int lcap, const int slab_slots,
                const int32_t* __restrict__ wg_slot, const int32_t* __restrict__ wg_vid,
                const uint32_t* __restrict__ wg_meta, const int32_t* __restrict__ wg_nbr,
                const int32_t* __restrict__ wg_fetch, const int32_t* __restrict__ wg_info, const int4* hrec,
                const float4* hq, const float4* vstate,
                float4* hq_out, float4* vstate_out, const float2* vaux, const float4* bar_in, float4* bar_out, float4* vprev,
                void* xbuf, const int rec_bytes, const int dual_arg, const unsigned tag0, const int n_iters,
                const unsigned max_spins_arg, const int poll_gap_arg, const SolverParams p,
                int* __restrict__ err, int* __restrict__ abort_flag, const int32_t* __restrict__ perm,
                const RunTail* __restrict__ tail, unsigned* __restrict__ probe, char* place_pool,
                const int32_t* __restrict__ rec_off, const int rec_off_stride, unsigned* rot_word) {
  extern __shared__ float4 lds[];
  constexpr int T = 64;
  const unsigned max_spins = max_spins_arg & 0x7fffffffu;
  const int dual = dual_arg & 1, verify = VERIFY ? dual_arg >> 1 : 0;
  const int poll_gap = poll_gap_arg & 255, pv_presleep = (poll_gap_arg >> 8) & 255;
  const int lane = (int)threadIdx.x;
  int b = blockIdx.x;
  if (rot_word) {
    const unsigned want = (tag0 & 0x0fffffffu) << 4;
    if (b == 0 && lane == 0) __hip_atomic_store(rot_word, want | read_xcc_id(), __ATOMIC_RELAXED, __HIP_MEMORY_SCOPE_AGENT);
    unsigned v = 0;
    for (unsigned spins = 0;; ++spins) {
      v = __builtin_amdgcn_readfirstlane(__hip_atomic_load(rot_word, __ATOMIC_RELAXED, __HIP_MEMORY_SCOPE_AGENT));
      if ((v & ~15u) == want) break;
      if (spins > (max_spins_arg & 0x7fffffffu)) {
        if (lane == 0) {
          give_up(abort_flag, err, false);
          report_expired(err, 1, (int)blockIdx.x, -1, 0ull, -1, v, want);
        }
        return;
      }
      __builtin_amdgcn_s_sleep(2);
    }
    b += (int)(v & 7u);
    if (b >= (int)gridDim.x) b -= (int)gridDim.x;
  }
  const int xcd = b & 7, idx = b >> 3;
  if (idx >= wgs_per_xcd) return;
  if (xcd * wgs_per_xcd + idx >= n_wgs) return;
  const int wg = wg_begin + xcd * wgs_per_xcd + idx;
  const int rid_base = wg_info[4 * wg], n_fetch = wg_info[4 * wg + 1];
  const int count_flags = wg_info[4 * wg + 2];
  if ((count_flags & 0xffff) == 0) return;
  if (unsigned* const pg = tail->progress) {
    if (lane == 0) pg[n_wgs + (wg - wg_begin)] = (unsigned)(wall_clock64() / 100u) | 1u;
  }
  const int stride = wg_info[4 * wg + 3];
  const int rec_stride = lcap + T;
  const int o_ovfA = 2 * rec_stride + slab_slots;
  const __amdgpu_buffer_rsrc_t rx = make_rsrc(xbuf);

  constexpr int kPar = 2;
  const int S = rec_bytes, par = 2 * rec_bytes, tab_off = kPar * par;
  const unsigned xcc_want = (tag0 & 0x0fffffffu) << 4;
  const unsigned p0 = tag0 & 1u;

  const size_t hl = (size_t)wg * T + lane;
  const unsigned meta = wg_meta[hl];
  const int slot = wg_slot[hl];
  const int pv = wg_vid[hl];
  const int nbr_code = wg_nbr[hl];
  const int frid = (lane < n_fetch) ? wg_fetch[hl] : -1;
  const int loc = (int)((meta >> 13) & 2047u);
  const bool active = (meta & kWgActiveBit) != 0u;
  const bool valid = (meta & kWgValidBit) != 0u, publishes = (meta & kWgPublishBit) != 0u;
  const bool state_lane = (meta & kWgHeadBit) != 0u;
  const unsigned degx = (meta & kWgHeadBit) ? ((meta >> 6) & 127u) : (active ? 255u : 0u);
  const unsigned long long rm1 = __ballot(degx > 1u), rm2 = __ballot(degx > 2u), rm3 = __ballot(degx > 3u), rm4 = __ballot(degx > 4u),
                           rm5 = __ballot(degx > 5u), rm6 = __ballot(degx > 6u), rm7 = __ballot(degx > 7u), rm8 = __ballot(degx > 8u);
  const int nbr_idx = active ? ((nbr_code < 0) ? lcap + (nbr_code & 0x7fffffff) : nbr_code) : (valid ? loc : 0);

  int4 rec = make_int4(0, 0, 0, 0);
  float4 q = make_float4(0.f, 0.f, 0.f, 0.f);
  if (active) {
    rec = hrec[slot];
    q = hq[slot];
  }
  const bool is_target = rec.x < 0;
  const float alpha = __int_as_float(rec.y), dx = __int_as_float(rec.z), dy = __int_as_float(rec.w);
  const float beta = q.w;
  float q1 = q.x;
  v2f_t q23 = {q.y, q.z};
  const float as = is_target ? -alpha : alpha, bs = is_target ? -beta : beta, ac = is_target ? alpha : -alpha;
  const v2f_t P12 = {alpha * dx, alpha * dy};
  const v2f_t C2 = !active ? v2f_t{0.0f, 0.0f} : is_target ? v2f_t{beta, beta} : v2f_t{-dx, -dy};
  const float nbeta = -beta;

  float4 st = make_float4(0.f, 0.f, 0.f, 0.f), bs4 = make_float4(0.f, 0.f, 0.f, 0.f);
  float2 aux = make_float2(0.f, 0.f);
  if (valid) {
    st = vstate[pv];
    aux = vaux[pv];
    bs4 = bar_in[pv];
  }
  const float data = st.w;
  const float thr = p.step_x * (p.data_factor * aux.x);
  float x = st.x;
  v2f_t w12 = {st.y, st.z};
  float xb = bs4.x;
  v2f_t wb12 = {bs4.y, bs4.z};
  float x_prev = x;
  v2f_t w_prev = w12;
  bool ok = true;
  bool timed_out = n_fetch > T;
  bool torn = false;

  const int my_off = (rid_base + loc) << 4;
  const int rec_w = valid ? loc : o_ovfA + lane, rec_wstride = valid ? rec_stride : 0;

  lds[lcap + lane] = make_float4(0.f, 0.f, 0.f, 0.f);
  lds[rec_stride + lcap + lane] = make_float4(0.f, 0.f, 0.f, 0.f);

  int off0 = (frid >= 0) ? (frid << 4) : 0;
  bool fetch_remote = frid >= 0;
  if (dual) {
    const unsigned my_xcc = read_xcc_id();
    if (state_lane && publishes)
      __builtin_amdgcn_raw_buffer_store_b32((int)(xcc_want | my_xcc), rx, tab_off + (my_off >> 2), 0, kAuxSc1);
    if (n_fetch > 0 && !timed_out) {
      bool pend = frid >= 0;
      unsigned g0 = 0, spins = 0;
      for (;;) {
        if (pend) {
// ... 300 lines not shown
      step(tag0 + (unsigned)it + 1u, rdB_nbr, dstB, wrA_rec, areaB + lcap, it + 1, srcB, pubA, wrB_rec);
    }
    if (it < n_iters && !timed_out) step(tag0 + (unsigned)it, rdA_nbr, dstA, wrB_rec, areaA + lcap, it, srcA, pubB, wrA_rec);
  }
  asm volatile("s_waitcnt vmcnt(0)" ::: "memory");

  if (timed_out) {
    if (lane == 0) {
      give_up(abort_flag, err, torn);
      unsigned* const pg = tail->progress;
      if (pg) pg[wg - wg_begin] = 0x80000000u | (unsigned)(it + 1);
    }
    return;
  }

  if (state_lane) write_back_vertex(pv, x, w12, xb, wb12, x_prev, w_prev, data, vstate_out, bar_out, vprev, perm, tail);
  if (active) hq_out[slot] = make_float4(q1, q23.x, q23.y, beta);
  if (!ok && active) atomicOr(err, 1);
}

}

int pv_real_waves_per_simd(bool verify_or_probe) {
  return verify_or_probe ? 5 : 7;
}

static unsigned pv_lds_bytes(int lcap, int slab_slots) { return 16u * (unsigned)(2 * (lcap + 64) + slab_slots + 64); }

int pv_patches_per_cu(const FusedArgs& a, bool verify) {
  if (!a.wg_rowpack) return 0;
  const size_t ldsv = pv_lds_bytes(a.wg_lcap, a.wg_slab_slots);
  int n = 0;
  const void* fv = verify ? (const void*)k_persistent_pv<false, true> : (const void*)k_persistent_pv<false, false>;
  if (hipOccupancyMaxActiveBlocksPerMultiprocessor(&n, fv, 64, ldsv) != hipSuccess) {
    (void)hipGetLastError();
    return 0;
  }
  return n < 4 * pv_real_waves_per_simd(verify) ? n : 4 * pv_real_waves_per_simd(verify);
}

int launch_persistent_run(const FusedArgs& a, const SolverParams& p, int form, int wave_begin, int n_waves,
                          int parity_in, unsigned tag0, int n_iters, int waves_per_block, unsigned max_spins,
                          int presleep, int dual, int xcds, const RunTail* tail, bool cooperative,
                          hipStream_t stream) {
  if (n_waves <= 0 || n_iters <= 0) return (int)hipSuccess;
  if (xcds < 1 || xcds > 8) xcds = 8;
  int wpx = (n_waves + xcds - 1) / xcds;
  const int bpx = (wpx + waves_per_block - 1) / waves_per_block;
  const dim3 grid((unsigned)(bpx * 8)), block((unsigned)(64 * waves_per_block));
  if (form != 2 && form != 3) return (int)hipErrorInvalidValue;
  const int32_t* i0 = a.tv_slot;
  const int32_t* i1 = a.tv_vid;
  const uint32_t* i2 = a.tv_meta;
  const void* i3 = (const void*)a.tv_wave;
  const int4* hrec = a.hrec;
  const float4* hq = a.hq;
  const float4* vstate = a.vstate;
  float4* hq_out = a.hq_out;
  float4* vstate_out = a.vstate_out;
  const float2* vaux = a.vaux;
  const float4* bin = a.bar[parity_in];
  float4* bout = a.bar[parity_in ^ 1];
  float4* vprev = a.vprev;
  void* xbuf = a.xbuf;
  int rec_bytes = persistent_rec_bytes(a);
  SolverParams pp = p;
  int* err = a.err;
  int* abort_flag = a.abort_flag;
  const int32_t* perm = a.perm;
  void* args[] = {&wave_begin, &n_waves, &wpx, &i0, &i1, &i2, &i3, &hrec, &hq, &vstate, &hq_out, &vstate_out, &vaux,
                  &bin, &bout, &vprev, &xbuf, &rec_bytes, &dual, &tag0, &n_iters, &max_spins, &presleep, &pp, &err,
                  &abort_flag, &perm, &tail};
  if (form == 3) {
    int wgx = (n_waves + xcds - 1) / xcds;
    const dim3 gv((unsigned)(wgx * 8)), bv(64u);
    int lcap = a.wg_lcap, slab_slots = a.wg_slab_slots, poll_gap = a.wg_poll_gap;
    const int32_t *w0 = a.wg_slot, *w1 = a.wg_vid, *w3 = a.wg_nbr, *w4 = a.wg_fetch, *w5 = a.wg_info;
    const uint32_t* w2 = a.wg_meta;
    unsigned* probe = a.probe;
    char* place_pool = (a.rec_off && wave_begin == 0 && xcds == 8) ? a.place_pool : nullptr;
    const int32_t* rec_off = a.rec_off;
    int rec_off_stride = a.rec_off_stride;
    unsigned* rot_word = place_pool ? a.rot_word : nullptr;
    const unsigned ldsv = pv_lds_bytes(lcap, slab_slots);
    void* vargs[] = {&wave_begin, &n_waves, &wgx, &lcap, &slab_slots, &w0, &w1, &w2, &w3, &w4, &w5, &hrec, &hq, &vstate,
                     &hq_out, &vstate_out, &vaux, &bin, &bout, &vprev, &xbuf, &rec_bytes, &dual, &tag0, &n_iters,
                     &max_spins, &poll_gap, &pp, &err, &abort_flag, &perm, &tail, &probe, &place_pool, &rec_off, &rec_off_stride, &rot_word};
    const bool vr = (dual >> 1) != 0;
    if (!a.wg_rowpack) return (int)hipErrorInvalidConfiguration;
    const void* fv = probe ? (const void*)k_persistent_pv<true, true>
                           : vr ? (const void*)k_persistent_pv<false, true>
                                : a.open_run ? (const void*)k_persistent_pv<false, false, true> : (const void*)k_persistent_pv<false, false>;
    if (cooperative) return (int)hipLaunchCooperativeKernel(fv, gv, bv, vargs, ldsv, stream);
    return (int)hipExtLaunchKernel(fv, gv, bv, vargs, ldsv, stream, nullptr, a.stop_event, 0);
  }
  unsigned lds_bytes = 0u;
  const void* fn = persistent_tv_kernel(waves_per_block, &lds_bytes);
  if (cooperative) return (int)hipLaunchCooperativeKernel(fn, grid, block, args, lds_bytes, stream);
  return (int)hipExtLaunchKernel(fn, grid, block, args, lds_bytes, stream, nullptr, a.stop_event, 0);
}

namespace {
__global__ void k_warm_cooperative() {}
}
void warm_module_persistent(hipStream_t stream, bool cooperative) {
  hipFuncAttributes fa;
  if (hipFuncGetAttributes(&fa, (const void*)k_persistent_pv<false, false>) != hipSuccess) (void)hipGetLastError();
  FusedArgs a;
  a.wg_rowpack = 1, a.wg_lcap = 16;
  (void)pv_patches_per_cu(a, false);
  void* no_args[] = {nullptr};
  if (cooperative && hipLaunchCooperativeKernel((const void*)k_warm_cooperative, dim3(8), dim3(64), no_args, 0, stream) != hipSuccess) (void)hipGetLastError();
}

}
```

flame_amd/csrc/nltgv2_run.hip:

```cpp
#include "nltgv2_context.hpp"

namespace flame_hip {
namespace host {

void pick_config(const flame_nltgv2_ctx* ctx, int* unroll, int* wpb) {
  const bool small = ctx->L.n_slices <= 8 * ctx->prop.multiProcessorCount;
  *unroll = ctx->opt_unroll ? ctx->opt_unroll : (small ? 8 : 4);
  *wpb = ctx->opt_block_waves ? ctx->opt_block_waves : (small ? 1 : 4);
}

struct WaveGroup {
  int begin, count;
};

int ensure_form_rows(flame_nltgv2_ctx* ctx, int form);
int plan_groups(flame_nltgv2_ctx* ctx, int form, int total, int cap, const std::vector<int32_t>& cw, std::vector<WaveGroup>* groups);

bool cooperative_allowed() {
  static const bool ok = [] {
    if (std::getenv("FLAME_NLTGV2_NO_COOPERATIVE")) return false;
    if (std::getenv("FLAME_NLTGV2_COOPERATIVE")) return true;
    if (std::getenv("ROCP_TOOL_LIBRARIES")) return false;
    if (void* h = dlopen("librocprofiler-sdk.so.1", RTLD_NOLOAD | RTLD_LAZY)) {
      dlclose(h);
// ... 150 lines not shown
      return 0;
    }
  }
  hipGraph_t graph = nullptr;
  HIPCHK(ctx, hipStreamBeginCapture(ctx->stream, hipStreamCaptureModeRelaxed));
  int rc = enqueue_fused_eager(ctx, p, n, parity, unroll, wpb, true);
  hipError_t e = hipStreamEndCapture(ctx->stream, &graph);
  if (rc != 0) {
    if (graph) (void)hipGraphDestroy(graph);
    return rc;
  }
  HIPCHK(ctx, e);
  hipGraphExec_t exec = nullptr;
  e = hipGraphInstantiate(&exec, graph, nullptr, nullptr, 0);
  (void)hipGraphDestroy(graph);
  HIPCHK(ctx, e);
  if ((int)ctx->graphs.size() >= kMaxCachedGraphs) {
    size_t victim = 0;
    for (size_t i = 1; i < ctx->graphs.size(); ++i)
      if (ctx->graphs[i].stamp < ctx->graphs[victim].stamp) victim = i;
    (void)hipGraphExecDestroy(ctx->graphs[victim].exec);
    ctx->graphs.erase(ctx->graphs.begin() + (long)victim);
  }
  CachedGraph cg;
  cg.exec = exec, cg.n = n, cg.parity = parity, cg.unroll = unroll, cg.wpb = wpb, cg.topo = ctx->topo;
  cg.gen = ctx->buf_gen;
  cg.params = *p, cg.stamp = ++ctx->stamp;
  ctx->graphs.push_back(cg);
  *out = exec;
  return 0;
}

int prepare_run(flame_nltgv2_ctx* ctx, const flame_nltgv2_params* p, int n) {
  if (ctx->opt_solver != 0 || !ctx->opt_use_graph || persistent_eligible(ctx, n)) return 0;
  int unroll, wpb;
  pick_config(ctx, &unroll, &wpb);
  int parity = ctx->parity;
  hipGraphExec_t exec;
  if (n >= kGraphChunk) {
    int rc = get_graph(ctx, p, kGraphChunk, parity, unroll, wpb, &exec);
    if (rc) return rc;
  }
  const int rem = n % kGraphChunk;
  if (rem >= 4) {
    int rc = get_graph(ctx, p, rem, parity, unroll, wpb, &exec);
    if (rc) return rc;
  }
  return 0;
}

PhotoFuse photo_target(const flame_nltgv2_ctx* ctx) {
  PhotoFuse f;
  std::memset(static_cast<void*>(&f), 0, sizeof f);
  f.graph_scale = 1.0f;
  if (!ctx->photo_fused || ctx->img_rows == 0) return f;
  f.pos = (const float2*)ctx->pos.p;
  f.ref = (const uint8_t*)ctx->img_ref.p, f.cmp = (const uint8_t*)ctx->img_cmp.p;
  f.err = (float*)ctx->photo_err.p;
  f.geo = ctx->photo_geo;
  f.graph_scale = ctx->photo_scale;
  f.rows = ctx->img_rows, f.cols = ctx->img_cols, f.step = ctx->img_step, f.border = ctx->photo_border;
  return f;
}

int enqueue_photo_sweep(flame_nltgv2_ctx* ctx, bool packed_current) {
  const PhotoFuse f = photo_target(ctx);
  if (!f.err) return 0;
  if (packed_current) {
    LAUNCHCHK(ctx, launch_photo_residual_packed(ctx->f, f, ctx->stream));
  } else {
    LAUNCHCHK(ctx, launch_photo_residual(ctx->c, f.graph_scale, f.geo, f.ref, f.cmp, f.rows, f.cols, f.step, f.border, f.err,
                                         ctx->stream));
  }
  ctx->photo_fresh = true;
  return 0;
}

namespace {
struct PlacePool {
  int device = -1;
  void* mem = nullptr;
  std::vector<uint16_t> rank;
  float best = 0.f, mean = 0.f, worst = 0.f;
};
std::mutex& g_place_mu = *new std::mutex;
std::vector<PlacePool>& g_place_free = *new std::vector<PlacePool>;
std::vector<int>& g_place_seen = *new std::vector<int>;
}

bool place_calibrate_at_create(int device) {
  std::lock_guard<std::mutex> lock(g_place_mu);
  bool first = true;
  for (int d : g_place_seen) first = first && d != device;
  if (first) g_place_seen.push_back(device);
  for (const PlacePool& e : g_place_free)
    if (e.device == device) return true;
  return first;
}

void place_pool_release(flame_nltgv2_ctx* ctx) {
  if (!ctx->place_pool.p || ctx->place_state != 1 || ctx->place_rank_host.empty()) return;
  PlacePool e;
  e.device = ctx->device, e.mem = ctx->place_pool.p, e.rank.swap(ctx->place_rank_host);
  e.best = ctx->place_best_us, e.mean = ctx->place_mean_us, e.worst = ctx->place_worst_us;
  ctx->device_bytes -= ctx->place_pool.cap;
  ctx->place_pool = DevBuf{};
  ctx->place_base = nullptr, ctx->place_state = 0;
  std::lock_guard<std::mutex> lock(g_place_mu);
  g_place_free.push_back(std::move(e));
}

int place_calibrate(flame_nltgv2_ctx* ctx) {
  ctx->place_state = -1;
  constexpr int P = kPlacePages, kIters = 12;
  const size_t pool_bytes = (size_t)2 * P * 4096;
  if (!ctx->place_pool.p && !std::getenv("FLAME_NLTGV2_RECALIBRATE")) {
    PlacePool e;
    {
      std::lock_guard<std::mutex> lock(g_place_mu);
      for (size_t i = 0; i < g_place_free.size(); ++i)
        if (g_place_free[i].device == ctx->device) {
          e = std::move(g_place_free[i]);
          g_place_free.erase(g_place_free.begin() + (long)i);
          break;
        }
    }
    if (e.mem) {
      ctx->place_pool.p = e.mem, ctx->place_pool.cap = pool_bytes + 4096;
      ctx->device_bytes += ctx->place_pool.cap;
      ctx->place_best_us = e.best, ctx->place_mean_us = e.mean, ctx->place_worst_us = e.worst;
      ctx->place_rank_host.swap(e.rank);
      int rc = ensure(ctx, ctx->place_rank, sizeof(uint16_t) * 2 * 64 * P);
      if (!rc) rc = ensure(ctx, ctx->place_fill, sizeof(int) * (2 * P + 16 + 128));
      if (rc) return rc;
      ctx->place_base = reinterpret_cast<char*>((reinterpret_cast<uintptr_t>(ctx->place_pool.p) + 4095) & ~uintptr_t(4095));
      HIPCHK(ctx, hipMemsetAsync(ctx->place_base, 0, pool_bytes, ctx->stream));
      HIPCHK(ctx, hipMemsetAsync(ctx->place_fill.p, 0, sizeof(int) * (2 * P + 16 + 128), ctx->stream));
      HIPCHK(ctx, hipMemcpyAsync(ctx->place_rank.p, ctx->place_rank_host.data(), sizeof(uint16_t) * ctx->place_rank_host.size(), hipMemcpyHostToDevice,
                                 ctx->stream));
      HIPCHK(ctx, wait_solver_stream(ctx));
      ctx->place_state = 1;
      return 0;
    }
  }
  int rc = ensure(ctx, ctx->place_pool, pool_bytes + 4096);
  if (!rc) rc = ensure(ctx, ctx->place_meas, sizeof(unsigned) * 64 * 2 * P + sizeof(int) * 64 + sizeof(int));
  if (!rc) rc = ensure(ctx, ctx->place_rank, sizeof(uint16_t) * 2 * 64 * P);
  if (!rc) rc = ensure(ctx, ctx->place_fill, sizeof(int) * (2 * P + 16 + 128));
  if (rc) return rc;
  ctx->place_base = reinterpret_cast<char*>((reinterpret_cast<uintptr_t>(ctx->place_pool.p) + 4095) & ~uintptr_t(4095));
  unsigned* d_out = (unsigned*)ctx->place_meas.p;
  int* d_xcc = (int*)(d_out + (size_t)64 * 2 * P);
  int* d_fail = d_xcc + 64;
  HIPCHK(ctx, hipMemsetAsync(ctx->place_base, 0, pool_bytes, ctx->stream));
  HIPCHK(ctx, hipMemsetAsync(ctx->place_meas.p, 0, sizeof(unsigned) * 64 * 2 * P + sizeof(int) * 65, ctx->stream));
  HIPCHK(ctx, hipMemsetAsync(ctx->place_fill.p, 0, sizeof(int) * (2 * P + 16 + 128), ctx->stream));
  LAUNCHCHK(ctx, launch_place_calibrate(ctx->place_base, 2 * P, kIters, d_out, d_xcc, d_fail, ctx->stream));
  std::vector<unsigned> out((size_t)64 * 2 * P);
  int xcc[65];
  HIPCHK(ctx, hipMemcpyAsync(out.data(), d_out, sizeof(unsigned) * out.size(), hipMemcpyDeviceToHost, ctx->stream));
  HIPCHK(ctx, hipMemcpyAsync(xcc, d_xcc, sizeof(int) * 65, hipMemcpyDeviceToHost, ctx->stream));
  HIPCHK(ctx, wait_solver_stream(ctx));
  HIPCHK(ctx, hipMemsetAsync(ctx->place_base, 0, pool_bytes, ctx->stream));
  if (xcc[64] != 0) return 0;
  std::vector<unsigned> lat((size_t)64 * 2 * P, 0u);
  bool have[64] = {false};
  for (int b = 8; b < 64; ++b) {
    const int x = b & 7, j = b >> 3, pb = ((8 - j) & 7) * 8 + ((x + j) & 7);
    const int from = xcc[pb], to = xcc[b];
    if (from < 0 || from > 7 || to < 0 || to > 7 || from == to) return 0;
    for (int pg = 0; pg < 2 * P; ++pg) {
      const unsigned t = out[(size_t)b * 2 * P + pg];
      if (t == 0u || t > (1u << 24)) return 0;
      lat[(size_t)(from * 8 + to) * 2 * P + pg] = t;
    }
    have[from * 8 + to] = true;
  }
  for (int a = 0; a < 8; ++a)
    for (int b = 0; b < 8; ++b)
      if (a != b && !have[a * 8 + b]) return 0;
  std::vector<uint16_t> rank((size_t)2 * 64 * P);
  double best = 0.0, mean = 0.0, worst = 0.0;
  for (int par = 0; par < 2; ++par)
    for (int c = 0; c < 64; ++c) {
      uint16_t* r = &rank[((size_t)par * 64 + c) * P];
      for (int t = 0; t < P; ++t) r[t] = (uint16_t)t;
      if (c / 8 == c % 8) continue;
      const unsigned* l = &lat[(size_t)c * 2 * P + (size_t)par * P];
      std::stable_sort(r, r + P, [&](uint16_t u, uint16_t v) { return l[u] < l[v]; });
      double m = 0.0;
      for (int t = 0; t < P; ++t) m += l[t];
      best += l[r[0]], worst += l[r[P - 1]], mean += m / P;
    }
  if (std::getenv("FLAME_NLTGV2_TRACE")) {
    for (int a = 0; a < 8; ++a) {
      std::fprintf(stderr, "[flame_nltgv2] hand-off from XCD %d to 0..7, best page (us):", a);
      for (int b = 0; b < 8; ++b) {
        if (a == b) { std::fprintf(stderr, "   -  "); continue; }
        const unsigned* l = &lat[(size_t)(a * 8 + b) * 2 * P];
        unsigned best_t = ~0u, worst_t = 0u;
        for (int t = 0; t < P; ++t) best_t = std::min(best_t, l[t]), worst_t = std::max(worst_t, l[t]);
        std::fprintf(stderr, " %.3f/%.3f", best_t / (100.0 * kIters), worst_t / (100.0 * kIters));
      }
      std::fprintf(stderr, "\n");
    }
  }
  const double to_us = 1.0 / (100.0 * kIters) / (2.0 * 56.0);
  ctx->place_best_us = (float)(best * to_us), ctx->place_mean_us = (float)(mean * to_us), ctx->place_worst_us = (float)(worst * to_us);
  HIPCHK(ctx, hipMemcpyAsync(ctx->place_rank.p, rank.data(), sizeof(uint16_t) * rank.size(), hipMemcpyHostToDevice, ctx->stream));
  HIPCHK(ctx, wait_solver_stream(ctx));
  ctx->place_state = 1;
  ctx->place_rank_host.swap(rank);
  return 0;
}

int place_records(flame_nltgv2_ctx* ctx, int per_xcd) {
  const size_t stride = records_capacity(ctx->L);
  int rc = ensure(ctx, ctx->place_rec_off, sizeof(int32_t) * 2 * stride);
  if (!rc) rc = ensure(ctx, ctx->place_patch, sizeof(int32_t) * stride + stride);
  if (rc) return rc;
  LAUNCHCHK(ctx, launch_place_records(ctx->c, ctx->f, per_xcd, (const int32_t*)ctx->order_m.p, (const int32_t*)ctx->rid_of.p,
                                      (int32_t*)ctx->place_patch.p, (int8_t*)((int32_t*)ctx->place_patch.p + stride),
                                      (const uint16_t*)ctx->place_rank.p, kPlacePages, (int*)ctx->place_fill.p,
                                      (int32_t*)ctx->place_rec_off.p, (int)stride, ctx->stream));
  ctx->place_topo = ctx->topo, ctx->place_per_xcd = per_xcd;
  return 0;
}

static bool open_run_applies(const flame_nltgv2_ctx* ctx, int form, const std::vector<WaveGroup>& groups) {
  if (groups.size() != 1) return false;
  const int cus = ctx->prop.multiProcessorCount;
  return (form == 3 && groups[0].count <= 20 * cus) || (form == 4 && groups[0].count <= 14 * cus);
}

int enqueue_run(flame_nltgv2_ctx* ctx, const flame_nltgv2_params* p, int n) {
  if (n <= 0) return 0;
  if (ctx->open_inflight) {
    const int rc0 = finish(ctx);
    if (rc0) return rc0;
  }
  if (ctx->opt_solver == 1) {
    int rc = ensure_canon(ctx);
    if (rc) return rc;
    const SolverParams sp = to_sp(p);
    for (int it = 0; it < n; ++it) {
      LAUNCHCHK(ctx, launch_save_prev(ctx->c, ctx->stream));
      LAUNCHCHK(ctx, launch_dual(ctx->c, sp, ctx->stream));
      LAUNCHCHK(ctx, launch_primal(ctx->c, sp, ctx->stream));
      LAUNCHCHK(ctx, launch_extragradient(ctx->c, sp, ctx->stream));
    }
    ctx->fused_valid = false;
    ctx->last_run_path = 4;
    if (ctx->replaying == 0) ctx->iters_total += n;
    if (ctx->export_ptr) LAUNCHCHK(ctx, launch_export(ctx->c, ctx->f, false, ctx->export_scale, ctx->export_ptr, ctx->stream));
    return enqueue_photo_sweep(ctx, false);
  }
  if (ctx->opt_mesh_state == 1 && ctx->canon_valid) {
    HIPCHK(ctx, hipEventRecord(ctx->ev_snap, ctx->stream));
    ctx->snap_topo = ctx->topo;
  }
  int rc = ensure_fused(ctx);
  if (rc) return rc;
  if (ctx->pending.active) {
    if (ctx->pending.ops.size() >= kMaxChain) {
      rc = finish(ctx);
    } else {
      rc = snapshot_chain_start(ctx);
    }
    if (rc) return rc;
  }
  int unroll, wpb;
  pick_config(ctx, &unroll, &wpb);
  std::vector<WaveGroup> groups;
  const int form = plan_persistent(ctx, n, &groups, true);
  const bool open_run = ctx->want_open != 0 && open_run_applies(ctx, form, groups) && !ctx->pending.active && ctx->opt_probe == 0 &&
                        ctx->opt_verify == 0 && ctx->replaying == 0 && (n & 1) == 0 && ctx->h_stop != nullptr && ctx->ctl_stream != nullptr;
  if (ctx->want_open != 0 && !open_run) {
    ctx->want_open = 0;
    return 0;
  }
  if (form != 0) {
    if ((uint64_t)ctx->tag_next + (uint64_t)n >= 0x07ff0000ull || (ctx->xbuf_form != 0 && ctx->xbuf_form != form)) {
      const size_t bytes = kXbufBytesPerVertex * records_capacity(ctx->L);
      HIPCHK(ctx, hipMemsetAsync(ctx->xbuf.p, 0, bytes, ctx->stream));
      if (ctx->place_base) {
        HIPCHK(ctx, hipMemsetAsync(ctx->place_base, 0, (size_t)2 * kPlacePages * 4096, ctx->stream));
        HIPCHK(ctx, hipMemsetAsync((int*)ctx->place_fill.p + 2 * kPlacePages, 0, 64, ctx->stream));
      }
      HIPCHK(ctx, hipMemsetAsync((int*)ctx->err.p + 12, 0, 2 * sizeof(int), ctx->stream));
      ctx->tag_next = 1;
    }
    ctx->xbuf_form = form;
    const uint32_t tag0 = ctx->tag_next + 2;
    const uint64_t key = ctx->topo * 1024 + (uint64_t)form * 64 + (ctx->opt_verify != 0 ? 16 : 0) + (ctx->opt_probe != 0 ? 8 : 0) +
                         (ctx->opt_dual == 2 ? 4 : ctx->opt_dual == 1 ? 2 : 0) + (ctx->opt_xcds > 0 ? 1 : 0);
    const RunTail* tail_dev = nullptr;
    {
      RunTail want;
      std::memset(static_cast<void*>(&want), 0, sizeof want);
      want.export_out = ctx->export_ptr, want.export_scale = ctx->export_scale;
      if (open_run) {
        const bool fresh = ctx->stop_dev.p == nullptr;
        rc = ensure(ctx, ctx->stop_dev, 64);
        if (rc) return rc;
        if (fresh) HIPCHK(ctx, hipMemsetAsync(ctx->stop_dev.p, 0, 64, ctx->stream));
        ctx->open_tag0 = tag0;
      }
      want.stop_req = open_run ? (const unsigned*)ctx->stop_dev.p : nullptr;
      const PhotoFuse pf = photo_target(ctx);
      std::memcpy(static_cast<void*>(&want.photo), &pf, sizeof pf);
      if (form == 3 && std::getenv("FLAME_NLTGV2_TRACE")) {
        rc = ensure(ctx, ctx->progress, 2 * sizeof(unsigned) * (size_t)ctx->L.wg_count);
        if (rc) return rc;
        HIPCHK(ctx, hipMemsetAsync(ctx->progress.p, 0, 2 * sizeof(unsigned) * (size_t)ctx->L.wg_count, ctx->stream));
        want.progress = (unsigned*)ctx->progress.p;
      }
      constexpr size_t kTailStride = (sizeof(RunTail) + 255) / 256 * 256;
      rc = ensure(ctx, ctx->run_tail, kTailStride * flame_nltgv2_ctx::kTailSlots);
      if (rc) return rc;
      int slot = -1;
      for (int i = 0; i < flame_nltgv2_ctx::kTailSlots && slot < 0; ++i)
        if (ctx->tail_valid[i] && std::memcmp(&want, &ctx->tail_sent[i], sizeof(RunTail)) == 0) slot = i;
      if (slot < 0) {
        slot = ctx->tail_next, ctx->tail_next = (ctx->tail_next + 1) % flame_nltgv2_ctx::kTailSlots;
        HIPCHK(ctx, hipMemcpyAsync((char*)ctx->run_tail.p + kTailStride * (size_t)slot, &want, sizeof(RunTail), hipMemcpyHostToDevice, ctx->stream));
        ctx->tail_sent[slot] = want;
        ctx->tail_valid[slot] = true;
      }
      tail_dev = (const RunTail*)((const char*)ctx->run_tail.p + kTailStride * (size_t)slot);
    }
    int e = 0;
    for (const WaveGroup& gr : groups) {
      const bool carries = &gr == &groups.back() && ctx->coop_checked_key == key && ctx->run_ev_pick >= 0 && ctx->ev_run[ctx->run_ev_pick] != nullptr;
      ctx->f.stop_event = carries ? ctx->ev_run[ctx->run_ev_pick] : nullptr;
      const int pw = gr.count <= 4 * ctx->prop.multiProcessorCount ? 1 : 4;
      const int dual = (ctx->opt_dual == 2 || (ctx->opt_dual == 1 && gr.count > kDualMinWavesPerCu * ctx->prop.multiProcessorCount) ? 1 : 0) |
                       (ctx->opt_verify == 2 ? 6 : ctx->opt_verify == 1 ? 2 : 0);
      const int cus_per_xcd = ctx->prop.multiProcessorCount / 8;
      const bool one_xcd = form == 3 && gr.count <= 2 * cus_per_xcd;
      const int xcds = ctx->opt_xcds > 0 ? ctx->opt_xcds : one_xcd ? 1 : 8;
      const int presleep = ctx->opt_presleep > 0 ? ctx->opt_presleep - 1 : kPreSleepTv;
      const unsigned spins_arg = (ctx->opt_fault > 0 && (ctx->replaying == 0 || ctx->opt_fault >= (1 << 22)))
                                     ? (0x80000000u | (unsigned)(ctx->opt_fault & ((1 << 22) - 1))) : kMaxSpins;
      if (form == 3) {
        const bool dense = gr.count > kPvPaceAbovePerCu * ctx->prop.multiProcessorCount;
        const bool denser = gr.count > kPvPaceMoreAbovePerCu * ctx->prop.multiProcessorCount;
        const int dense_gap = denser ? kPvDenserGap : kPvDenseGap, dense_pre = denser ? kPvDenserPreSleep : kPvDensePreSleep;
        const int gap = ctx->opt_poll_gap > 0 ? ctx->opt_poll_gap - 1 : dense ? (3 | ((dense_gap - 1) << 4)) : kPvPollGap;
        ctx->f.wg_poll_gap = gap | ((ctx->opt_presleep > 0 ? ctx->opt_presleep - 1 : dense ? dense_pre : kPvPreSleep) << 8);
        ctx->f.rec_off = nullptr, ctx->f.place_pool = nullptr;
        if (ctx->opt_place && groups.size() == 1 && gr.begin == 0 && xcds == 8 && (dual & 1)) {
          if (ctx->place_state == 0) {
            rc = place_calibrate(ctx);
            if (rc) return rc;
          }
          const int per_xcd = (gr.count + xcds - 1) / xcds;
          if (ctx->place_state == 1 && (ctx->place_topo != ctx->topo || ctx->place_per_xcd != per_xcd)) {
            rc = place_records(ctx, per_xcd);
            if (rc) return rc;
          }
          if (ctx->place_state == 1) {
            ctx->f.place_pool = ctx->place_base, ctx->f.rec_off = (const int32_t*)ctx->place_rec_off.p;
            ctx->f.rec_off_stride = (int)records_capacity(ctx->L);
            ctx->f.rot_word = (unsigned*)ctx->place_fill.p + 2 * kPlacePages;
          }
        }
        ctx->f.probe = nullptr;
        if (ctx->opt_probe) {
          const size_t words = (size_t)ctx->L.wg_count * (size_t)n * 8;
          rc = ensure(ctx, ctx->probe, words * sizeof(unsigned));
          if (rc) return rc;
          ctx->f.probe = (unsigned*)ctx->probe.p;
          ctx->probe_words = words;
          HIPCHK(ctx, hipMemsetAsync(ctx->probe.p, 0, words * sizeof(unsigned), ctx->stream));
        }
      }
      if (form == 4) {
        const bool dense = gr.count > kPv2PaceAbovePerCu * ctx->prop.multiProcessorCount;
        const int gap = ctx->opt_poll_gap > 0 ? ctx->opt_poll_gap - 1 : dense ? (3 | ((kPv2DenseGap - 1) << 4)) : kPvPollGap;
        const int poll_gap = gap | ((ctx->opt_presleep > 0 ? ctx->opt_presleep - 1 : dense ? kPv2DensePreSleep : kPvPreSleep) << 8);
        ctx->f.open_run = open_run ? 1 : 0;
        e = launch_persistent_pv2(ctx->f, ctx->pv2_args, to_sp(p), gr.begin, gr.count, ctx->parity, tag0, n, spins_arg, poll_gap, dual,
                                  tail_dev, cooperative_allowed() && ctx->coop_checked_key != key, ctx->stream);
        ctx->f.open_run = 0;
        if (e != 0) break;
        continue;
      }
      ctx->f.open_run = open_run ? 1 : 0;
      e = launch_persistent_run(ctx->f, to_sp(p), form, gr.begin, gr.count, ctx->parity, tag0, n, pw, spins_arg, presleep, dual,
                                xcds, tail_dev, cooperative_allowed() && ctx->coop_checked_key != key, ctx->stream);
      ctx->f.open_run = 0;
      if (e != 0) break;
    }
    ctx->run_event_bound = e == 0 && ctx->f.stop_event != nullptr;
    ctx->f.stop_event = nullptr;
    ctx->tag_next = tag0 + (uint32_t)n;
    if (e == 0) {
      if (!ctx->pending.active) {
        ctx->pending.active = true, ctx->pending.snapshotted = false;
        ctx->pending.ops.clear();
        ctx->pending.parity_before = ctx->parity, ctx->pending.have_prev_before = ctx->have_prev;
      }
      {
        flame_nltgv2_ctx::PendingOp op;
        op.kind = 0, op.params = *p, op.n = n;
        op.open = open_run, op.tag0 = tag0;
        op.dst = ctx->export_ptr, op.scale = ctx->export_scale;
        ctx->pending.ops.push_back(op);
      }
      ctx->photo_fresh = photo_target(ctx).err != nullptr;
      ctx->open_inflight = open_run, ctx->open_stop_sent = false;
      if (open_run) ctx->want_open = 2;
      if (!open_run && ctx->replaying == 0) ctx->iters_total += n;
      std::swap(ctx->hq, ctx->hq_alt);
      std::swap(ctx->vstate, ctx->vstate_alt);
      ctx->buf_gen ^= 1;
      refresh_args(ctx);
      ctx->coop_checked_key = key;
      ctx->last_run_path = form == 4 ? 7 : form == 3 ? 6 : 5;
      ctx->last_run_groups = (int)groups.size();
      ctx->last_run_waves_per_cu = 0;
      for (const WaveGroup& gr : groups) ctx->last_run_waves_per_cu = std::max(ctx->last_run_waves_per_cu, (gr.count + ctx->prop.multiProcessorCount - 1) / ctx->prop.multiProcessorCount);
      ctx->parity ^= 1;
      ctx->have_prev = true;
      ctx->canon_valid = false;
      return 0;
    }
    if (std::getenv("FLAME_NLTGV2_TRACE")) std::fprintf(stderr, "[flame_nltgv2] persistent launch refused: hip error %d (%s), form %d, pv_occ %d\n", e, hipGetErrorString((hipError_t)e), form, ctx->pv_occ);
    (void)hipGetLastError();
    ctx->persist_refused_topo = ctx->topo;
    if (groups.size() > 1 && !ctx->pending.active) {
      HIPCHK(ctx, hipMemsetAsync(ctx->abort_flag.p, 0xff, sizeof(int), ctx->stream));
      HIPCHK(ctx, wait_solver_stream(ctx));
      HIPCHK(ctx, hipMemsetAsync(ctx->err.p, 0, kErrBytes, ctx->stream));
      HIPCHK(ctx, hipMemsetAsync(ctx->abort_flag.p, 0, sizeof(int), ctx->stream));
    }
  }
  if (ctx->pending.active) {
    flame_nltgv2_ctx::PendingOp op;
    op.kind = 0, op.params = *p, op.n = n;
    op.dst = ctx->export_ptr, op.scale = ctx->export_scale;
    ctx->pending.ops.push_back(op);
  }
  int left = n;
  while (left > 0) {
    const int chunk = left >= kGraphChunk ? kGraphChunk : left;
    if (ctx->opt_use_graph && chunk >= 4) {
// ... 368 lines not shown
```

flame_amd/csrc/nltgv2_topo_capi.hip:

```cpp
#include "nltgv2_context.hpp"

namespace flame_hip {
namespace host {

namespace {

struct Carve {
  size_t off = 0;
  size_t take(size_t bytes) {
    const size_t at = off;
    off += (bytes + 255) & ~size_t(255);
    return at;
  }
};

constexpr size_t kWalkPad = 256 * 64;

struct ScratchMap {
  size_t fid, edges, init, old_edge, first_k, scan, deg, cur, parent, minid, morton, key_out, width, wflag, vf0, vf1, seg0, seg1, counters, wg2_v0, vmap,
      emap, old_feat, sort, total, sort_bytes, vpad;
  int cc_bits, n_slices;
};
ScratchMap make_scratch(int32_t V, int32_t E, int32_t Vo, int32_t Eo, bool sync) {
  ScratchMap m{};
// ... 236 lines not shown
    rc = ensure(ctx, *r.b, r.bytes);
    if (rc) return rc;
  }
  if (!ctx->h_dims) request_open_stop(ctx);
  if (!ctx->h_dims && hipHostMalloc((void**)&ctx->h_dims, sizeof(TopoDims), hipHostMallocDefault) != hipSuccess) {
    (void)hipGetLastError();
    return fail(ctx, FLAME_NLTGV2_ERR_OOM);
  }
  if (ctx->raster_inflight) HIPCHK(ctx, hipStreamWaitEvent(ctx->stream, ctx->ev_raster_done, 0));
  std::vector<StageCopy> cp = {{&ctx->pos, g->pos, 2 * fV}, {&ctx->src, g->src, fE}, {&ctx->dst, g->dst, fE}};
  cp.insert(cp.end(), extra, extra + n_extra);
  rc = staged_h2d(ctx, cp.data(), cp.size());
  if (rc) return rc;
  char* const sc = static_cast<char*>(ctx->topo_scratch.p);
  TopoBuild t;
  t.V = V, t.E = E;
  t.pos = (const float2*)ctx->pos.p;
  t.minx = minx, t.miny = miny;
  t.sx = (maxx > minx) ? 65535.0f / (maxx - minx) : 0.0f, t.sy = (maxy > miny) ? 65535.0f / (maxy - miny) : 0.0f;
  bind_scratch(&t, sc, sm);
  t.src = (int32_t*)ctx->src.p, t.dst = (int32_t*)ctx->dst.p, t.row_ptr = (int32_t*)ctx->row_ptr.p, t.half = (uint32_t*)ctx->half.p;
  t.order_m = (int32_t*)ctx->order_m.p, t.rid_of = (int32_t*)ctx->rid_of.p, t.perm = (int32_t*)ctx->perm.p, t.iperm = (int32_t*)ctx->iperm.p;
  t.pdeg = (int32_t*)ctx->pdeg.p, t.slice_row = (int32_t*)ctx->slice_row.p;
  t.wg_info = (int32_t*)ctx->wg_info.p, t.wg_v0 = (int32_t*)ctx->wg_v0.p, t.wg_vfirst = (uint8_t*)ctx->wg_vfirst.p;
  t.wg2_info = (int32_t*)ctx->wg2_info.p, t.wg2_vfirst = (uint8_t*)ctx->wg2_vfirst.p;
  t.dims = (TopoDims*)ctx->topo_dims.p;
  LAUNCHCHK(ctx, launch_topo_upload_front(t, ctx->stream));
  LAUNCHCHK(ctx, launch_topo_back(t, ctx->stream));
  HIPCHK(ctx, hipMemcpyAsync(ctx->h_dims, ctx->topo_dims.p, sizeof(TopoDims), hipMemcpyDeviceToHost, ctx->stream));
  HIPCHK(ctx, wait_solver_stream(ctx));
  const TopoDims dm = *ctx->h_dims;
  if (dm.flags != 0 || (ctx->opt_persistent != 4 && dm.wg_count > kPvDensePerCu * cus)) return 0;
  PackedLayout& L = ctx->L;
  L.V = V, L.E = E, L.n_slices = sm.n_slices, L.rows = dm.rows, L.max_degree = dm.max_degree;
  L.wg_ok = true, L.wg_rowpack = true, L.wg_count = dm.wg_count, L.wg_lcap = dm.wg_lcap, L.wg_slab_slots = 0, L.n_rec = V;
  L.wg2_walked = true, L.wg2_ok = dm.max_degree <= 32 && dm.wg2_count > 0, L.wg2_count = dm.wg2_count, L.wg2_lcap = dm.wg2_lcap;
  L.tv_ok = false, L.tv_waves = 0;
  ctx->host_layout_valid = false;
  const bool want_e2 = wants_e2(ctx) && L.wg2_ok && L.wg2_count <= kPv2WavesPerCu * cus * 4;
  rc = topology_buffers(ctx, want_e2, 4 * (size_t)L.wg_count, (size_t)L.wg_count, (size_t)V, 4 * (size_t)L.wg2_count, (size_t)V);
  if (rc) return rc;
  std::vector<StageFill> fills;
  topology_fills(ctx, want_e2, &fills);
  rc = staged_h2d(ctx, nullptr, 0, fills.data(), fills.size());
  if (rc) return rc;
  rc = topology_expand(ctx, want_e2);
  if (rc) return rc;
  ctx->feat_dev_valid = false;
  HIPCHK(ctx, hipEventRecord(ctx->ev_topo_ready, ctx->stream));
  *done = true;
  return 0;
}

int topo_commit(flame_nltgv2_ctx* ctx, bool* done) {
  *done = false;
  using C = flame_nltgv2_ctx;
  C::PreparedSync& P = ctx->prepared;
  if (!P.active || !P.device || P.topo != ctx->topo) return fail(ctx, FLAME_NLTGV2_ERR_INVALID_ARG);
  hipStream_t ts = ctx->topo_stream;
  const bool trace = std::getenv("FLAME_NLTGV2_TRACE") != nullptr;
  const auto t0 = std::chrono::steady_clock::now();
  HIPCHK(ctx, hipStreamSynchronize(ctx->topo_stream));
  const auto t1 = std::chrono::steady_clock::now();
  P.active = false;
  const int32_t V = P.V, E = P.E;
  const TopoDims dm = *ctx->h_dims;
  const int cus = ctx->prop.multiProcessorCount;
  const bool rowpack = ctx->opt_persistent == 4 || (static_cast<int64_t>(2) * E + V / 32) / 54 + 1 <= (int64_t)kPvDensePerCu * cus;
  if (dm.flags != 0 || dm.n_edges != E || !rowpack || (ctx->opt_persistent != 4 && dm.wg_count > kPvDensePerCu * cus)) {
    if (trace) std::fprintf(stderr, "[flame_nltgv2] sync_graph: device build declined (flags %d, edges %d of %d, patches %d), host path\n", dm.flags, dm.n_edges, E, dm.wg_count);
    return 0;
  }
  if (std::getenv("FLAME_NLTGV2_LATE_EXPAND")) {
    const int rc0 = ensure_canon(ctx);
    if (rc0) return rc0;
  }
  const int n_slices = (V + kWave - 1) / kWave;
  PackedLayout Ln;
  Ln.V = V, Ln.E = E, Ln.n_slices = n_slices, Ln.rows = dm.rows, Ln.max_degree = dm.max_degree;
  Ln.wg_ok = true, Ln.wg_rowpack = true, Ln.wg_count = dm.wg_count, Ln.wg_lcap = dm.wg_lcap, Ln.wg_slab_slots = 0, Ln.n_rec = V;
  Ln.wg2_walked = true, Ln.wg2_ok = dm.max_degree <= 32 && dm.wg2_count > 0, Ln.wg2_count = dm.wg2_count, Ln.wg2_lcap = dm.wg2_lcap;
  Ln.tv_ok = false, Ln.tv_waves = 0;
  const bool want_e2 = wants_e2(ctx, Ln) && Ln.wg2_ok && Ln.wg2_count <= kPv2WavesPerCu * cus * 4;
  const bool placed = placement_applies(ctx, Ln);
  int rc = 0;
  {
    const size_t n_slots = (size_t)(Ln.rows + kRowPad) * kWave, lanes = (size_t)Ln.wg_count * kWave, lanes2 = (size_t)Ln.wg2_count * kWave;
    if (n_slots > (size_t)0x7fffffff) return fail(ctx, FLAME_NLTGV2_ERR_INVALID_ARG);
    const size_t stride = records_capacity(Ln);
    struct { int i; size_t bytes; } req[] = {
        {C::EX_REC_NBR, sizeof(uint32_t) * n_slots}, {C::EX_REC_EDGE, sizeof(int32_t) * n_slots}, {C::EX_EDGE_SRC_SLOT, sizeof(int32_t) * (size_t)E},
        {C::EX_WG_SLOT, sizeof(int32_t) * lanes}, {C::EX_WG_VID, sizeof(int32_t) * lanes}, {C::EX_WG_META, sizeof(uint32_t) * lanes},
        {C::EX_WG_NBR, sizeof(int32_t) * lanes}, {C::EX_WG_FETCH, sizeof(int32_t) * lanes},
        {C::EX_WG2_SLOT, want_e2 ? sizeof(int32_t) * 2 * lanes2 : 0}, {C::EX_WG2_NBR, want_e2 ? sizeof(int32_t) * 2 * lanes2 : 0},
        {C::EX_WG2_VID, want_e2 ? sizeof(int32_t) * lanes2 : 0}, {C::EX_WG2_META, want_e2 ? sizeof(uint32_t) * lanes2 : 0},
        {C::EX_WG2_FETCH, want_e2 ? sizeof(int32_t) * lanes2 : 0}, {C::EX_WG2_RMAX, want_e2 ? (size_t)64 : 0},
        {C::EX_PLACE_REC_OFF, placed ? sizeof(int32_t) * 2 * stride : 0}};
    for (auto& r : req)
      if (r.bytes && (rc = ensure(ctx, ctx->ex[r.i], r.bytes)) != 0) return rc;
    if (placed) {
      rc = ensure(ctx, ctx->place_patch_nx, sizeof(int32_t) * stride + stride);
      if (!rc && ctx->place_fill_nx.cap == 0) {
        rc = ensure(ctx, ctx->place_fill_nx, sizeof(int) * (2 * kPlacePages + 16 + 128));
        if (!rc) HIPCHK(ctx, hipMemsetAsync(ctx->place_fill_nx.p, 0, sizeof(int) * (2 * kPlacePages + 16 + 128), ts));
      }
      if (rc) return rc;
    }
    ExpandTables t;
    t.c = ctx->c, t.f = ctx->f;
    t.c.V = V, t.c.E = E;
    t.c.src = (int32_t*)ctx->nx[C::NX_SRC].p, t.c.dst = (int32_t*)ctx->nx[C::NX_DST].p;
    t.c.row_ptr = (int32_t*)ctx->nx[C::NX_ROW_PTR].p, t.c.half = (uint32_t*)ctx->nx[C::NX_HALF].p;
    t.f.n_slices = n_slices, t.f.n_slots = (int)n_slots;
    t.f.slice_row = (int32_t*)ctx->nx[C::NX_SLICE_ROW].p, t.f.perm = (int32_t*)ctx->nx[C::NX_PERM].p, t.f.pdeg = (int32_t*)ctx->nx[C::NX_PDEG].p;
    t.f.rec_nbr = (uint32_t*)ctx->ex[C::EX_REC_NBR].p, t.f.rec_edge = (int32_t*)ctx->ex[C::EX_REC_EDGE].p;
    t.f.edge_src_slot = (int32_t*)ctx->ex[C::EX_EDGE_SRC_SLOT].p;
    t.f.wg_count = Ln.wg_count, t.f.n_rec = Ln.n_rec, t.f.wg_lcap = Ln.wg_lcap, t.f.wg_slab_slots = 0, t.f.wg_rowpack = 1;
    t.f.wg_slot = (int32_t*)ctx->ex[C::EX_WG_SLOT].p, t.f.wg_vid = (int32_t*)ctx->ex[C::EX_WG_VID].p, t.f.wg_meta = (uint32_t*)ctx->ex[C::EX_WG_META].p;
    t.f.wg_nbr = (int32_t*)ctx->ex[C::EX_WG_NBR].p, t.f.wg_fetch = (int32_t*)ctx->ex[C::EX_WG_FETCH].p;
    t.f.wg_info = (int32_t*)ctx->nx[C::NX_WG_INFO].p;
    t.iperm = (const int32_t*)ctx->nx[C::NX_IPERM].p, t.wg_v0 = (const int32_t*)ctx->nx[C::NX_WG_V0].p;
    t.order_m = (const int32_t*)ctx->nx[C::NX_ORDER_M].p, t.rid_of = (const int32_t*)ctx->nx[C::NX_RID_OF].p;
    t.wg_vfirst = (const uint8_t*)ctx->nx[C::NX_WG_VFIRST].p;
    t.wg2_info = (int32_t*)ctx->nx[C::NX_WG2_INFO].p, t.wg2_vfirst = (const uint8_t*)ctx->nx[C::NX_WG2_VFIRST].p;
    t.wg2_slot = (int32_t*)ctx->ex[C::EX_WG2_SLOT].p, t.wg2_vid = (int32_t*)ctx->ex[C::EX_WG2_VID].p, t.wg2_nbr = (int32_t*)ctx->ex[C::EX_WG2_NBR].p;
    t.wg2_fetch = (int32_t*)ctx->ex[C::EX_WG2_FETCH].p, t.wg2_meta = (uint32_t*)ctx->ex[C::EX_WG2_META].p, t.wg2_rmax = (int*)ctx->ex[C::EX_WG2_RMAX].p;
    if (placed) {
      t.rec_off = (int32_t*)ctx->ex[C::EX_PLACE_REC_OFF].p, t.place_patch = (int32_t*)ctx->place_patch_nx.p, t.place_fill = (int*)ctx->place_fill_nx.p;
      t.per_xcd = (Ln.wg_count + 7) / 8, t.stride = stride;
    }
    std::vector<StageFill> fills;
    expansion_fills(Ln, t.f.rec_edge, t.f.rec_nbr, want_e2 ? t.wg2_rmax : nullptr, &fills);
    rc = staged_h2d(ctx, nullptr, 0, fills.data(), fills.size(), 0, ts);
    if (!rc) rc = expand_launches(ctx, Ln, t, want_e2, ts);
    if (rc) return rc;
    HIPCHK(ctx, hipEventRecord(ctx->ev_expanded, ts));
  }
  const size_t fV = sizeof(float) * (size_t)V, fE = sizeof(float) * (size_t)E;
  DevBuf* cur_v[9] = {&ctx->x, &ctx->w1, &ctx->w2, &ctx->xb, &ctx->w1b, &ctx->w2b, &ctx->xp, &ctx->w1p, &ctx->w2p};
  DevBuf* cur_q[3] = {&ctx->q1, &ctx->q2, &ctx->q3};
  for (int i = 0; i < 9 && !rc; ++i) rc = ensure(ctx, ctx->sp_v[i], fV);
  for (int i = 0; i < 3 && !rc; ++i) rc = ensure(ctx, ctx->sp_q[i], fE);
  for (int i = 0; i < 2 && !rc; ++i) rc = ensure(ctx, ctx->sp_ab[i], fE);
  if (!rc) rc = ensure(ctx, ctx->sync_need, (size_t)V);
  if (rc) return rc;
  SyncArgs sa;
  sa.V = V, sa.E = E;
  sa.old_of_new = (const int32_t*)ctx->prep_vmap, sa.old_of_new_edge = (const int32_t*)ctx->prep_emap;
  sa.data = (const float*)ctx->nx[C::NX_DATA].p, sa.weight = (const float*)ctx->nx[C::NX_WEIGHT].p;
  sa.init_x = P.has_init ? (const float*)ctx->prep_init : nullptr;
  set_init_map(ctx, P.init_from_map != 0, &sa);
  if (P.init_from_map != 0 && sa.map_rows == 0) sa.init_map = sa.data;
  sa.check_sticky = P.check_sticky, sa.sticky_threshold = P.sticky_threshold;
  sa.graph_scale = P.init_graph_scale;
  for (int i = 0; i < 9; ++i) sa.o[i] = (const float*)cur_v[i]->p, sa.n[i] = (float*)ctx->sp_v[i].p;
  for (int i = 0; i < 3; ++i) sa.oq[i] = (const float*)cur_q[i]->p, sa.nq[i] = (float*)ctx->sp_q[i].p;
  sa.src = (const int32_t*)ctx->nx[C::NX_SRC].p, sa.dst = (const int32_t*)ctx->nx[C::NX_DST].p, sa.row_ptr = (const int32_t*)ctx->nx[C::NX_ROW_PTR].p;
  sa.half = (const uint32_t*)ctx->nx[C::NX_HALF].p, sa.pos = (const float2*)ctx->nx[C::NX_POS].p;
  sa.alpha = (float*)ctx->sp_ab[0].p, sa.beta = (float*)ctx->sp_ab[1].p, sa.need_nbr = (uint8_t*)ctx->sync_need.p;
  const std::function<int()> gather = [&]() -> int {
    LAUNCHCHK(ctx, launch_sync_state(sa, ctx->stream));
    return 0;
  };
  const auto t1b = std::chrono::steady_clock::now();
  int behind = kBehindNotLaunched;
  rc = ensure_canon(ctx, &gather, &behind);
  if (rc) return rc;
  if (behind != kBehindDone) {
    rc = gather();
    if (rc) return rc;
  }
  const auto t2 = std::chrono::steady_clock::now();
  ctx->have_graph = false;
  PackedLayout& L = ctx->L;
  L.V = V, L.E = E, L.n_slices = n_slices, L.rows = dm.rows, L.max_degree = dm.max_degree;
  L.wg_ok = true, L.wg_rowpack = true, L.wg_count = dm.wg_count, L.wg_lcap = dm.wg_lcap, L.wg_slab_slots = 0, L.n_rec = V;
  L.wg2_walked = true, L.wg2_ok = Ln.wg2_ok, L.wg2_count = dm.wg2_count, L.wg2_lcap = dm.wg2_lcap;
  L.tv_ok = false, L.tv_waves = 0;
  ctx->host_layout_valid = false;
  for (int i = 0; i < C::NX_COUNT; ++i) std::swap(*ctx->nx_live(i), ctx->nx[i]);
  for (int i = 0; i < C::EX_COUNT; ++i) std::swap(*ctx->ex_live(i), ctx->ex[i]);
  rc = topology_buffers(ctx, want_e2, 4 * (size_t)L.wg_count, (size_t)L.wg_count, (size_t)V, 4 * (size_t)L.wg2_count, (size_t)V);
  if (rc) return rc;
  std::vector<StageFill> fills;
  topology_fills(ctx, want_e2, &fills, true);
  rc = staged_h2d(ctx, nullptr, 0, fills.data(), fills.size());
  if (rc) return rc;
  rc = topology_expand(ctx, want_e2, true);
  if (rc) return rc;
  if (placed) ctx->place_topo = ctx->topo, ctx->place_per_xcd = (L.wg_count + 7) / 8;
  HIPCHK(ctx, hipStreamWaitEvent(ctx->stream, ctx->ev_expanded, 0));
  for (int i = 0; i < 9; ++i) std::swap(*cur_v[i], ctx->sp_v[i]);
  for (int i = 0; i < 3; ++i) std::swap(*cur_q[i], ctx->sp_q[i]);
  std::swap(ctx->alpha, ctx->sp_ab[0]), std::swap(ctx->beta, ctx->sp_ab[1]);
  refresh_args(ctx);
  ctx->static_stale = true;
  HIPCHK(ctx, hipEventRecord(ctx->ev_topo_ready, ctx->stream));
  ctx->feat_gen += 1, ctx->feat_dev_valid = true;
  const int32_t* const fid = reinterpret_cast<const int32_t*>(static_cast<const char*>(ctx->stage[1].h) + P.off[0]);
  ctx->h_feat.assign(fid, fid + V);
  ctx->feat_map_valid = false, ctx->feat_tab_valid = false;
  ctx->canon_valid = true, ctx->fused_valid = false, ctx->have_prev = false, ctx->parity = 0;
  ctx->have_graph = true, ctx->last_error = 0, ctx->last_sync_path = 2;
  *done = true;
  if (trace) {
    const auto t2b = std::chrono::steady_clock::now();
    HIPCHK(ctx, wait_solver_stream(ctx));
    const auto t3 = std::chrono::steady_clock::now();
    auto ms = [](auto a, auto b) { return std::chrono::duration<double, std::milli>(b - a).count(); };
    std::fprintf(stderr, "[flame_nltgv2] sync_graph (device): prepare (checks, staging, builder enqueued) %.3f ms; commit: builder awaited %.3f, "
                 "expansion enqueued beside the solver %.3f, solver settled (unpack + state gather behind it) %.3f, swap + clears enqueued %.3f, device done %.3f ms later "
                 "(V=%d E=%d: %d kept, %d patches, %d two-half-edge patches)\n",
                 ms(P.t_begin, P.t_enqueued), ms(t0, t1), ms(t1, t1b), ms(t1b, t2), ms(t2, t2b), ms(t2b, t3), V, E, dm.n_keep, dm.wg_count, dm.wg2_count);
  }
  return 0;
}

}
}
```

flame_amd/regularizer.py:

```python
from __future__ import annotations

import ctypes as C
import os

import numpy as np

_HERE = os.path.dirname(os.path.abspath(__file__))
_LIB = None

_FP = C.POINTER(C.c_float)
_IP = C.POINTER(C.c_int32)

OPT_SOLVER, OPT_USE_HIPGRAPH, OPT_PERSISTENT, OPT_PROBE, OPT_VERIFY_RECORDS, OPT_PLACEMENT, OPT_SYNC_PATH, OPT_COST_SUM, OPT_MESH_STATE = 1, 2, 5, 12, 14, 16, 17, 18, 19
OPT_BLOCK_WAVES, OPT_UNROLL, OPT_DUAL_PUBLISH, OPT_PRESLEEP, OPT_XCDS, OPT_FAULT_INJECT, OPT_POLL_GAP = 103, 104, 106, 108, 109, 110, 113
RUN_PATHS = {0: "none", 1: "persistent (the lane-per-half-edge form, retired in round 3)", 2: "per-step hipGraph", 3: "per-step eager", 4: "canonical 4-sweep",
             5: "persistent-tv", 6: "persistent-pv", 7: "persistent-pv2"}
ERR_NAN = -5

VERTEX_STATE = ("x", "w1", "w2", "x_bar", "w1_bar", "w2_bar", "x_prev", "w1_prev", "w2_prev")
EDGE_STATE = ("q1", "q2", "q3")


def _rows_contiguous_u8(a) -> bool:
    return a.dtype == np.uint8 and a.ndim == 2 and a.strides[1] == 1 and a.strides[0] >= max(a.shape[1], 1)


class NLTGV2Error(RuntimeError):
    def __init__(self, status: int, what: str):
        super().__init__(f"{what}: status {status} ({status_string(status)})")
        self.status = status


class Params(C.Structure):

    _fields_ = [(n, C.c_float) for n in ("data_factor", "step_x", "step_q", "theta", "x_min", "x_max")]

    def __init__(self, data_factor=0.1, step_x=0.001, step_q=125.0, theta=0.25, x_min=0.0, x_max=10.0):
        super().__init__(data_factor, step_x, step_q, theta, x_min, x_max)


class MeshFilterParams(C.Structure):

    _fields_ = [("do_oblique_triangle_filter", C.c_int32), ("oblique_normal_thresh", C.c_float),
                ("oblique_idepth_diff_factor", C.c_float), ("oblique_idepth_diff_abs", C.c_float),
                ("do_edge_length_filter", C.c_int32), ("edge_length_thresh", C.c_float),
                ("do_idepth_triangle_filter", C.c_int32), ("min_triangle_idepth", C.c_float)]

    def __init__(self, do_oblique_triangle_filter=True, oblique_normal_thresh=1.39626, oblique_idepth_diff_factor=0.35,
                 oblique_idepth_diff_abs=0.1, do_edge_length_filter=True, edge_length_thresh=0.333,
                 do_idepth_triangle_filter=True, min_triangle_idepth=0.01):
        super().__init__(int(bool(do_oblique_triangle_filter)), oblique_normal_thresh, oblique_idepth_diff_factor,
                         oblique_idepth_diff_abs, int(bool(do_edge_length_filter)), edge_length_thresh,
                         int(bool(do_idepth_triangle_filter)), min_triangle_idepth)


class _MeshOutputsView(C.Structure):
    _fields_ = [("V", C.c_int32), ("T", C.c_int32), ("tri_valid", C.POINTER(C.c_uint8)), ("normals", _FP), ("vtx_idepth", _FP),
                ("n_valid", C.c_int32), ("rows", C.c_int32), ("cols", C.c_int32), ("filtered_map", _FP),
                ("filtered_coverage", C.c_int32), ("device_ms", C.c_float)]


class DebugImageParams(C.Structure):

    _fields_ = [("scene_color_scale", C.c_float), ("flip", C.c_int32), ("want_idepthmap", C.c_int32), ("want_normals", C.c_int32)]

    def __init__(self, scene_color_scale=1.0, flip=False, want_idepthmap=True, want_normals=True):
        super().__init__(scene_color_scale, int(bool(flip)), int(bool(want_idepthmap)), int(bool(want_normals)))


class _DebugImagesView(C.Structure):
    _fields_ = [("rows", C.c_int32), ("cols", C.c_int32), ("idepthmap_img", C.POINTER(C.c_uint8)), ("normals_img", C.POINTER(C.c_uint8)),
                ("w1_map", _FP), ("w2_map", _FP), ("device_ms", C.c_float)]


class _Graph(C.Structure):
    _fields_ = (
        [("V", C.c_int32), ("E", C.c_int32), ("pos", _FP)]
        + [(n, _FP) for n in VERTEX_STATE + ("data_term", "data_weight")]
        + [("src", _IP), ("dst", _IP)]
        + [(n, _FP) for n in ("alpha", "beta") + EDGE_STATE]
    )


class _SyncInput(C.Structure):
    _fields_ = [("V", C.c_int32), ("feat_id", _IP), ("pos", _FP), ("data_term", _FP), ("data_weight", _FP),
                ("init_x", _FP), ("E", C.c_int32), ("edges", _IP), ("check_sticky_obstacles", C.c_int32),
                ("sticky_threshold", C.c_float), ("init_graph_scale", C.c_float), ("edges_unique", C.c_int32),
                ("init_from_map", C.c_int32)]


class _Projection(C.Structure):
    _fields_ = [("K", C.c_float * 9), ("Kinv", C.c_float * 9), ("KRKinv", C.c_float * 9), ("q_ref_to_cmp", C.c_float * 4),
                ("t_ref_to_cmp", C.c_float * 3), ("region_x", C.c_float), ("region_y", C.c_float), ("region_w", C.c_float),
                ("region_h", C.c_float)]


class _Info(C.Structure):
    _fields_ = [
        ("abi_version", C.c_int32), ("device", C.c_int32), ("V", C.c_int32), ("E", C.c_int32),
        ("n_slices", C.c_int32), ("max_degree", C.c_int32), ("padded_half_edges", C.c_int64),
        ("device_bytes", C.c_int64), ("algorithmic_bytes_per_iter", C.c_int64), ("compute_units", C.c_int32),
        ("device_name", C.c_char * 64), ("gcn_arch", C.c_char * 32), ("last_run_path", C.c_int32), ("he_waves", C.c_int32), ("tv_waves", C.c_int32),
        ("tv_wave_capacity", C.c_int32), ("last_run_groups", C.c_int32), ("timeouts_recovered", C.c_int32),
        ("patches", C.c_int32), ("torn_records_detected", C.c_int32), ("last_sync_path", C.c_int32),
        ("last_run_waves_per_cu", C.c_int32), ("reserved0", C.c_int32), ("reserved1", C.c_int32), ("replays_per_step", C.c_int32),
    ]


def library_path() -> str:
    return os.environ.get("FLAME_AMD_LIBRARY") or os.path.join(_HERE, "libflame_nltgv2_hip.so")


ABI_SYMBOLS = (
    "flame_nltgv2_default_params", "flame_nltgv2_create", "flame_nltgv2_destroy", "flame_nltgv2_set_stream", "flame_nltgv2_stream_wait_run", "flame_nltgv2_runs_in_flight", "flame_nltgv2_run_open", "flame_nltgv2_iterations",
    "flame_nltgv2_upload_graph", "flame_nltgv2_update_data", "flame_nltgv2_upload_state", "flame_nltgv2_run",
    "flame_nltgv2_run_async", "flame_nltgv2_sync", "flame_nltgv2_run_timed", "flame_nltgv2_save_prev",
    "flame_nltgv2_dual_step", "flame_nltgv2_primal_step", "flame_nltgv2_extragradient_step", "flame_nltgv2_step",
    "flame_nltgv2_costs", "flame_nltgv2_download_state", "flame_nltgv2_export_idepth_device",
    "flame_nltgv2_export_idepth_device_async", "flame_nltgv2_set_export_target",
    "flame_nltgv2_set_option", "flame_nltgv2_get_info", "flame_nltgv2_last_error", "flame_nltgv2_last_hip_error",
    "flame_nltgv2_status_string", "flame_nltgv2_abi_version", "flame_nltgv2_pack_probe", "flame_nltgv2_read_probe", "flame_nltgv2_layout_selftest", "flame_nltgv2_placement_info",
    "flame_nltgv2_photo_set_images", "flame_nltgv2_photo_residual", "flame_nltgv2_photo_fuse",
    "flame_nltgv2_photo_residual_last", "flame_nltgv2_sync_graph", "flame_nltgv2_sync_prepare", "flame_nltgv2_sync_commit",
    "flame_nltgv2_get_topology", "flame_nltgv2_graph_size", "flame_nltgv2_set_feature_ids", "flame_nltgv2_interpolate_mesh",
    "flame_nltgv2_interpolate_mesh_begin", "flame_nltgv2_interpolate_mesh_end",
    "flame_nltgv2_interpolate_mesh_arrays", "flame_nltgv2_project_graph", "flame_nltgv2_rescale_data",
    "flame_delaunay_triangulate",
    "flame_nltgv2_default_mesh_filter_params", "flame_nltgv2_oblique_cos_bound", "flame_nltgv2_mesh_outputs_begin",
    "flame_nltgv2_mesh_outputs_end", "flame_nltgv2_mesh_outputs",
    "flame_nltgv2_default_debug_image_params", "flame_nltgv2_debug_images_begin", "flame_nltgv2_debug_images_end",
    "flame_nltgv2_debug_images",
)


def load_library():
    global _LIB
    if _LIB is not None:
        return _LIB
    path = library_path()
    if not os.path.exists(path):
        raise NLTGV2Error(-2, f"HIP library not built: {path} (run __graft_entry__.build())")
    L = C.CDLL(path)
    ctx = C.c_void_p
    PP, GP = C.POINTER(Params), C.POINTER(_Graph)
    sig = {
        "flame_nltgv2_default_params": (None, [PP]),
        "flame_nltgv2_create": (C.c_int, [C.POINTER(ctx), C.c_int]),
        "flame_nltgv2_destroy": (C.c_int, [ctx]),
        "flame_nltgv2_set_stream": (C.c_int, [ctx, C.c_void_p]),
        "flame_nltgv2_stream_wait_run": (C.c_int, [ctx, C.c_void_p]),
        "flame_nltgv2_runs_in_flight": (C.c_int, [ctx, C.POINTER(C.c_int32)]),
        "flame_nltgv2_run_open": (C.c_int, [ctx, C.POINTER(Params), C.c_int, C.POINTER(C.c_int32)]),
        "flame_nltgv2_iterations": (C.c_int, [ctx, C.POINTER(C.c_int64), C.POINTER(C.c_int32)]),
        "flame_nltgv2_upload_graph": (C.c_int, [ctx, GP]),
        "flame_nltgv2_update_data": (C.c_int, [ctx, _FP, _FP]),
        "flame_nltgv2_upload_state": (C.c_int, [ctx, GP]),
        "flame_nltgv2_run": (C.c_int, [ctx, PP, C.c_int]),
        "flame_nltgv2_run_async": (C.c_int, [ctx, PP, C.c_int]),
        "flame_nltgv2_sync": (C.c_int, [ctx]),
        "flame_nltgv2_run_timed": (C.c_int, [ctx, PP, C.c_int, _FP]),
        "flame_nltgv2_save_prev": (C.c_int, [ctx]),
        "flame_nltgv2_dual_step": (C.c_int, [ctx, PP]),
        "flame_nltgv2_primal_step": (C.c_int, [ctx, PP]),
        "flame_nltgv2_extragradient_step": (C.c_int, [ctx, PP]),
        "flame_nltgv2_step": (C.c_int, [ctx, PP]),
        "flame_nltgv2_costs": (C.c_int, [ctx, PP, _FP, _FP]),
        "flame_nltgv2_download_state": (C.c_int, [ctx, GP]),
        "flame_nltgv2_export_idepth_device": (C.c_int, [ctx, C.c_void_p, C.c_float]),
        "flame_nltgv2_export_idepth_device_async": (C.c_int, [ctx, C.c_void_p, C.c_float]),
        "flame_nltgv2_set_export_target": (C.c_int, [ctx, C.c_void_p, C.c_float]),
        "flame_nltgv2_set_option": (C.c_int, [ctx, C.c_int, C.c_int]),
        "flame_nltgv2_get_info": (C.c_int, [ctx, C.POINTER(_Info)]),
        "flame_nltgv2_last_error": (C.c_int, [ctx]),
        "flame_nltgv2_last_hip_error": (C.c_int, [ctx]),
        "flame_nltgv2_status_string": (C.c_char_p, [C.c_int]),
        "flame_nltgv2_abi_version": (C.c_int, []),
        "flame_nltgv2_layout_selftest": (C.c_int, [ctx, C.POINTER(C.c_int64)]),
        "flame_nltgv2_placement_info": (C.c_int, [ctx, C.POINTER(C.c_int32), C.POINTER(C.c_int32), C.POINTER(C.c_float)]),
        "flame_nltgv2_pack_probe": (C.c_int, [GP, _IP, _IP, _IP, _IP, C.c_int64, C.POINTER(C.c_int64)]),
        "flame_nltgv2_read_probe": (C.c_int, [ctx, C.POINTER(C.c_uint32), C.c_int64, C.POINTER(C.c_int64)]),
        "flame_nltgv2_photo_set_images": (C.c_int, [ctx, C.POINTER(C.c_uint8), C.POINTER(C.c_uint8), C.c_int, C.c_int, C.c_int]),
        "flame_nltgv2_photo_residual": (C.c_int, [ctx, _FP, _FP, C.c_float, C.c_int, _FP]),
        "flame_nltgv2_photo_fuse": (C.c_int, [ctx, _FP, _FP, C.c_float, C.c_int, C.c_int]),
        "flame_nltgv2_photo_residual_last": (C.c_int, [ctx, _FP]),
        "flame_nltgv2_sync_graph": (C.c_int, [ctx, C.POINTER(_SyncInput)]),
        "flame_nltgv2_sync_prepare": (C.c_int, [ctx, C.POINTER(_SyncInput)]),
        "flame_nltgv2_sync_commit": (C.c_int, [ctx]),
        "flame_nltgv2_get_topology": (C.c_int, [ctx, _IP, _IP, _IP]),
        "flame_nltgv2_graph_size": (C.c_int, [ctx, C.POINTER(C.c_int32), C.POINTER(C.c_int32)]),
        "flame_nltgv2_set_feature_ids": (C.c_int, [ctx, _IP]),
        "flame_delaunay_triangulate": (C.c_int, [_FP, C.c_int32, _IP, C.c_int32, _IP, _IP, C.c_int32, _IP]),
        "flame_nltgv2_project_graph": (C.c_int, [ctx, C.POINTER(_Projection), C.c_float, C.POINTER(C.c_uint8), _FP]),
        "flame_nltgv2_rescale_data": (C.c_int, [ctx, C.c_float, _FP, PP]),
        "flame_nltgv2_interpolate_mesh": (C.c_int, [ctx, _IP, C.c_int32, C.POINTER(C.c_uint8), C.c_int, C.c_int, C.c_float,
                                                    _FP, _IP]),
        "flame_nltgv2_interpolate_mesh_begin": (C.c_int, [ctx, _IP, C.c_int32, C.POINTER(C.c_uint8), C.c_int, C.c_int, C.c_float]),
        "flame_nltgv2_interpolate_mesh_end": (C.c_int, [ctx, C.POINTER(_FP), _IP]),
        "flame_nltgv2_interpolate_mesh_arrays": (C.c_int, [ctx, _IP, C.c_int32, _FP, _FP, C.c_int32, C.POINTER(C.c_uint8),
                                                           C.POINTER(C.c_uint8), C.c_int, C.c_int, _FP, _IP]),
        "flame_nltgv2_default_mesh_filter_params": (None, [C.POINTER(MeshFilterParams)]),
        "flame_nltgv2_oblique_cos_bound": (C.c_float, [C.c_float]),
        "flame_nltgv2_mesh_outputs_begin": (C.c_int, [ctx, _IP, C.c_int32, _FP, C.POINTER(MeshFilterParams), C.c_int, C.c_int,
                                                      C.c_float, C.c_int]),
        "flame_nltgv2_mesh_outputs_end": (C.c_int, [ctx, C.POINTER(_MeshOutputsView)]),
        "flame_nltgv2_mesh_outputs": (C.c_int, [ctx, _IP, C.c_int32, _FP, C.POINTER(MeshFilterParams), C.c_int, C.c_int, C.c_float,
                                                C.POINTER(C.c_uint8), _FP, _FP, _IP, _FP, _IP]),
        "flame_nltgv2_default_debug_image_params": (None, [C.POINTER(DebugImageParams)]),
        "flame_nltgv2_debug_images_begin": (C.c_int, [ctx, C.c_void_p, C.c_void_p, C.c_int, _FP, C.POINTER(DebugImageParams), C.c_int,
                                                      C.c_int]),
        "flame_nltgv2_debug_images_end": (C.c_int, [ctx, C.POINTER(_DebugImagesView)]),
        "flame_nltgv2_debug_images": (C.c_int, [ctx, C.c_void_p, C.c_void_p, C.c_int, _FP, C.POINTER(DebugImageParams), C.c_int, C.c_int,
                                                C.POINTER(C.c_uint8), C.POINTER(C.c_uint8), _FP, _FP]),
    }
    for name, (res, args) in sig.items():
        fn = getattr(L, name)
        fn.restype, fn.argtypes = res, args
    _LIB = L
    return L


def status_string(status: int) -> str:
    try:
        return load_library().flame_nltgv2_status_string(int(status)).decode()
    except Exception:
        return "?"


def _as(arr, dtype, n, name):
    a = np.ascontiguousarray(arr, dtype=dtype)
    if a.size != n:
        raise ValueError(f"{name}: expected {n} elements, got {a.size}")
    return a


def _graph_view(g: dict, keep: list, need_all=True) -> _Graph:
    V, E = int(g["V"]), int(g["E"])
    cg = _Graph()
    cg.V, cg.E = V, E
    sizes = {"pos": 2 * V, "data_term": V, "data_weight": V, "src": E, "dst": E, "alpha": E, "beta": E}
    sizes.update({k: V for k in VERTEX_STATE})
    sizes.update({k: E for k in EDGE_STATE})
    for name, ctype in _Graph._fields_[2:]:
        if name not in g or g[name] is None:
            if need_all and not name.endswith("_prev"):
                raise KeyError(name)
            continue
        dt = np.int32 if ctype is _IP else np.float32
        a = _as(g[name], dt, sizes[name], name)
        keep.append(a)
        setattr(cg, name, a.ctypes.data_as(ctype))
    return cg


def delaunay(pos, out=None):
    L = load_library()
    p = np.ascontiguousarray(pos, np.float32).reshape(-1, 2)
    n = p.shape[0]
    nt, ne = C.c_int32(0), C.c_int32(0)
    if out is not None and out[0].shape[0] >= 2 * n and out[1].shape[0] >= 3 * n and out[0].dtype == np.int32 and out[1].dtype == np.int32:
        tri, edg = out
    else:
# ... 29 lines not shown

class Regularizer:

    def __init__(self, device: int = 0):
        self._L = load_library()
        self._ctx = C.c_void_p()
        self._mesh_T = -1
        rc = self._L.flame_nltgv2_create(C.byref(self._ctx), int(device))
        if rc != 0:
            self._ctx = None
            raise NLTGV2Error(rc, "flame_nltgv2_create")
        self.V = self.E = 0

    def close(self):
        if getattr(self, "_ctx", None):
            self._L.flame_nltgv2_destroy(self._ctx)
            self._ctx = None

    __del__ = close

    def __enter__(self):
        return self

    def __exit__(self, *a):
        self.close()

    def _chk(self, rc, what):
        if rc != 0:
            raise NLTGV2Error(rc, what)

    def upload_graph(self, g: dict):
        keep = []
        cg = _graph_view(g, keep)
        self._chk(self._L.flame_nltgv2_upload_graph(self._ctx, C.byref(cg)), "upload_graph")
        self.V, self.E = int(g["V"]), int(g["E"])

    def sync_prepare(self, *args, **kw):
        self._sync(self._L.flame_nltgv2_sync_prepare, "sync_prepare", *args, **kw)

    def sync_commit(self):
        self._chk(self._L.flame_nltgv2_sync_commit(self._ctx), "sync_commit")
        self._refresh_size()

    def _refresh_size(self):
        nv, ne = C.c_int32(0), C.c_int32(0)
        self._chk(self._L.flame_nltgv2_graph_size(self._ctx, C.byref(nv), C.byref(ne)), "graph_size")
        self.V, self.E = int(nv.value), int(ne.value)

    def sync_graph(self, *args, **kw):
        self._sync(self._L.flame_nltgv2_sync_graph, "sync_graph", *args, **kw)
        self._refresh_size()

    def _sync(self, fn, what, feat_id, pos, data_term, data_weight, edges, init_x=None, check_sticky_obstacles=False,
              sticky_threshold=0.25, init_graph_scale=0.0, edges_unique=False, init_from_map=False):
        V = int(len(feat_id))
        fid = _as(feat_id, np.int32, V, "feat_id")
        p = _as(pos, np.float32, 2 * V, "pos")
        d = _as(data_term, np.float32, V, "data_term")
        w = _as(data_weight, np.float32, V, "data_weight")
        ed = np.ascontiguousarray(edges, np.int32).reshape(-1, 2)
        si = _SyncInput()
        si.V, si.E = V, int(ed.shape[0])
        si.feat_id, si.pos = fid.ctypes.data_as(_IP), p.ctypes.data_as(_FP)
        si.data_term, si.data_weight = d.ctypes.data_as(_FP), w.ctypes.data_as(_FP)
        ix = None
        if init_x is not None:
            ix = _as(init_x, np.float32, V, "init_x")
            si.init_x = ix.ctypes.data_as(_FP)
        si.edges = ed.ctypes.data_as(_IP)
        si.check_sticky_obstacles = 1 if check_sticky_obstacles else 0
        si.sticky_threshold = sticky_threshold
        si.init_graph_scale = float(init_graph_scale)
        si.edges_unique = 1 if edges_unique else 0
        si.init_from_map = 1 if init_from_map else 0
        self._chk(fn(self._ctx, C.byref(si)), what)

    def placement_info(self) -> dict:
        st, n = C.c_int32(0), C.c_int32(0)
        us = (C.c_float * 3)()
        self._chk(self._L.flame_nltgv2_placement_info(self._ctx, C.byref(st), C.byref(n), us), "placement_info")
        return {"state": int(st.value), "placed_records": int(n.value), "best_us": float(us[0]), "mean_us": float(us[1]),
                "worst_us": float(us[2])}

    def layout_selftest(self) -> int:
        n = C.c_int64(-1)
        self._chk(self._L.flame_nltgv2_layout_selftest(self._ctx, C.byref(n)), "layout_selftest")
        return int(n.value)

    def set_feature_ids(self, feat_id):
        fid = _as(feat_id, np.int32, self.V, "feat_id")
        self._chk(self._L.flame_nltgv2_set_feature_ids(self._ctx, fid.ctypes.data_as(_IP)), "set_feature_ids")

    def topology(self):
        src = np.empty(self.E, np.int32)
        dst = np.empty(self.E, np.int32)
        fid = np.empty(self.V, np.int32)
        self._chk(self._L.flame_nltgv2_get_topology(self._ctx, src.ctypes.data_as(_IP), dst.ctypes.data_as(_IP),
                                                     fid.ctypes.data_as(_IP)), "get_topology")
        return src, dst, fid

    def project_graph(self, K, Kinv, KRKinv, q, t, region, graph_scale=1.0):
        pr = _Projection()
        for name, a, n in (("K", K, 9), ("Kinv", Kinv, 9), ("KRKinv", KRKinv, 9), ("q_ref_to_cmp", q, 4), ("t_ref_to_cmp", t, 3)):
            arr = np.ascontiguousarray(a, np.float32).reshape(n)
            setattr(pr, name, (C.c_float * n)(*arr.tolist()))
        pr.region_x, pr.region_y, pr.region_w, pr.region_h = [float(r) for r in region]
        keep = np.zeros(self.V, np.uint8)
        pos = np.empty((self.V, 2), np.float32)
        self._chk(self._L.flame_nltgv2_project_graph(self._ctx, C.byref(pr), C.c_float(graph_scale),
                                                     keep.ctypes.data_as(C.POINTER(C.c_uint8)), pos.ctypes.data_as(_FP)),
                  "project_graph")
        return keep, pos

    def rescale_data(self, graph_scale, params: Params):
        ns = C.c_float(0)
        self._chk(self._L.flame_nltgv2_rescale_data(self._ctx, C.c_float(graph_scale), C.byref(ns), C.byref(params)),
                  "rescale_data")
        return float(ns.value)

    def update_data(self, data_term, data_weight):
        d = _as(data_term, np.float32, self.V, "data_term")
        w = _as(data_weight, np.float32, self.V, "data_weight")
        self._chk(self._L.flame_nltgv2_update_data(self._ctx, d.ctypes.data_as(_FP), w.ctypes.data_as(_FP)),
                  "update_data")

    def upload_state(self, state: dict):
        keep = []
        s = dict(state)
        s.setdefault("V", self.V)
        s.setdefault("E", self.E)
        cg = _graph_view(s, keep, need_all=False)
        self._chk(self._L.flame_nltgv2_upload_state(self._ctx, C.byref(cg)), "upload_state")

    def download_state(self, keys=VERTEX_STATE + EDGE_STATE) -> dict:
        out = {}
        cg = _Graph()
        for k in keys:
            n = self.V if k in VERTEX_STATE else self.E
            out[k] = np.empty(n, np.float32)
            setattr(cg, k, out[k].ctypes.data_as(_FP))
        self._chk(self._L.flame_nltgv2_download_state(self._ctx, C.byref(cg)), "download_state")
        return out

    def run(self, params: Params, n_iters: int):
        self._chk(self._L.flame_nltgv2_run(self._ctx, C.byref(params), int(n_iters)), "run")

    def step(self, params: Params):
        self._chk(self._L.flame_nltgv2_step(self._ctx, C.byref(params)), "step")

    def run_async(self, params: Params, n_iters: int):
        self._chk(self._L.flame_nltgv2_run_async(self._ctx, C.byref(params), int(n_iters)), "run_async")

    def sync(self):
        self._chk(self._L.flame_nltgv2_sync(self._ctx), "sync")

    def run_timed(self, params: Params, n_iters: int) -> float:
        ms = C.c_float(0)
        self._chk(self._L.flame_nltgv2_run_timed(self._ctx, C.byref(params), int(n_iters), C.byref(ms)), "run_timed")
        return float(ms.value)

    def save_prev(self):
        self._chk(self._L.flame_nltgv2_save_prev(self._ctx), "save_prev")

    def dual_step(self, params: Params):
        self._chk(self._L.flame_nltgv2_dual_step(self._ctx, C.byref(params)), "dual_step")

# ... 212 lines not shown
```

include/flame_nltgv2.h:

```cpp
#ifndef FLAME_NLTGV2_H_
#define FLAME_NLTGV2_H_

#include <stdint.h>

#ifdef __cplusplus
extern "C" {
#endif

#define FLAME_NLTGV2_ABI_VERSION 7

typedef struct flame_nltgv2_ctx flame_nltgv2_ctx;

typedef enum flame_nltgv2_status {
  FLAME_NLTGV2_OK = 0,
  FLAME_NLTGV2_ERR_INVALID_ARG = -1,
  FLAME_NLTGV2_ERR_NO_DEVICE = -2,
  FLAME_NLTGV2_ERR_HIP = -3,
  FLAME_NLTGV2_ERR_NO_GRAPH = -4,
  FLAME_NLTGV2_ERR_NAN = -5,
  FLAME_NLTGV2_ERR_OOM = -6,
  FLAME_NLTGV2_ERR_TIMEOUT = -7,
  FLAME_NLTGV2_ERR_ASSERT = -8
} flame_nltgv2_status;

// ... 140 lines not shown
void flame_nltgv2_default_debug_image_params(flame_nltgv2_debug_image_params* p);

typedef struct flame_nltgv2_debug_images_view {
  int32_t rows, cols;
  const uint8_t* idepthmap_img;
  const uint8_t* normals_img;
  const float* w1_map;
  const float* w2_map;
  float device_ms;
} flame_nltgv2_debug_images_view;

int flame_nltgv2_debug_images_begin(flame_nltgv2_ctx* ctx, const uint8_t* img_host, const void* img_device, int step_bytes,
                                    const float* K, const flame_nltgv2_debug_image_params* params, int rows, int cols);
int flame_nltgv2_debug_images_end(flame_nltgv2_ctx* ctx, flame_nltgv2_debug_images_view* out);
int flame_nltgv2_debug_images(flame_nltgv2_ctx* ctx, const uint8_t* img_host, const void* img_device, int step_bytes, const float* K,
                              const flame_nltgv2_debug_image_params* params, int rows, int cols, uint8_t* idepthmap_img_out,
                              uint8_t* normals_img_out, float* w1_map_out, float* w2_map_out);

int flame_delaunay_triangulate(const float* xy, int32_t n, int32_t* triangles, int32_t tri_capacity,
                               int32_t* n_triangles, int32_t* edges, int32_t edge_capacity, int32_t* n_edges);

int flame_nltgv2_photo_set_images(flame_nltgv2_ctx* ctx, const uint8_t* ref, const uint8_t* cmp, int rows, int cols,
                                  int step_bytes);
int flame_nltgv2_photo_residual(flame_nltgv2_ctx* ctx, const float* KRKinv, const float* Kt, float graph_scale,
                                int border, float* err_out);
int flame_nltgv2_photo_fuse(flame_nltgv2_ctx* ctx, const float* KRKinv, const float* Kt, float graph_scale, int border,
                            int enable);
int flame_nltgv2_photo_residual_last(flame_nltgv2_ctx* ctx, float* err_out);

enum {
  FLAME_NLTGV2_OPT_SOLVER = 1,
  FLAME_NLTGV2_OPT_USE_HIPGRAPH = 2,
  FLAME_NLTGV2_OPT_PERSISTENT = 5,
  FLAME_NLTGV2_OPT_PROBE = 12,
  FLAME_NLTGV2_OPT_VERIFY_RECORDS = 14,
  FLAME_NLTGV2_OPT_PLACEMENT = 16,

  FLAME_NLTGV2_OPT_SYNC_PATH = 17,

  FLAME_NLTGV2_OPT_COST_SUM = 18,

  FLAME_NLTGV2_OPT_MESH_STATE = 19,

  FLAME_NLTGV2_OPT_EXPERIMENTAL = 100
};
int flame_nltgv2_set_option(flame_nltgv2_ctx* ctx, int option, int value);

typedef struct flame_nltgv2_info {
  int32_t abi_version;
  int32_t device;
  int32_t V, E;
  int32_t n_slices;
  int32_t max_degree;
  int64_t padded_half_edges;
  int64_t device_bytes;
  int64_t algorithmic_bytes_per_iter;
  int32_t compute_units;
  char device_name[64];
  char gcn_arch[32];
  int32_t last_run_path;
  int32_t he_waves;
  int32_t tv_waves;
  int32_t tv_wave_capacity;
  int32_t last_run_groups;
  int32_t timeouts_recovered;
  int32_t patches;
  int32_t torn_records_detected;
  int32_t last_sync_path;
  int32_t last_run_waves_per_cu;
  int32_t reserved0, reserved1;
  int32_t replays_per_step;
} flame_nltgv2_info;
int flame_nltgv2_get_info(flame_nltgv2_ctx* ctx, flame_nltgv2_info* info);

int flame_nltgv2_last_error(flame_nltgv2_ctx* ctx);
int flame_nltgv2_last_hip_error(flame_nltgv2_ctx* ctx);
const char* flame_nltgv2_status_string(int status);
int flame_nltgv2_abi_version(void);

int flame_nltgv2_read_probe(flame_nltgv2_ctx* ctx, uint32_t* out, int64_t max_words, int64_t* n_words);

int flame_nltgv2_placement_info(flame_nltgv2_ctx* ctx, int32_t* state, int32_t* placed_records, float* us);

int flame_nltgv2_layout_selftest(flame_nltgv2_ctx* ctx, int64_t* mismatches);
int flame_nltgv2_pack_probe(const flame_nltgv2_graph* g, int32_t* perm, int32_t* slice_row,
                            int32_t* rec_nbr, int32_t* rec_edge, int64_t capacity_rows, int64_t* rows_out);

#ifdef __cplusplus
}
#endif
#endif
```

Before: 1.093 million.

## Add measured XCD-pair latency mapping of patch groups to XCDs

Adds an XCD remapping step: calibration measures pairwise XCD latencies, the classify kernel records per-group-pair weights from patch degree costs, and a branch-and-bound search picks a permutation of patch groups onto XCDs that minimises the worst pair cost. The persistent kernel uses the chosen map to pick which group a workgroup serves, and record placement uses the inverse map. The intent is to cut cross-XCD exchange latency on the critical path. It adds host-side weight fetches, events and search work, and the default option value (1) may keep the identity map unless the search is enabled.

New measurement: 1.075 million. 0.984x the previous value.

```diff
diff --git a/flame_amd/csrc/flame_nltgv2_test_options.h b/flame_amd/csrc/flame_nltgv2_test_options.h
--- a/flame_amd/csrc/flame_nltgv2_test_options.h
+++ b/flame_amd/csrc/flame_nltgv2_test_options.h
@@ -8,7 +8,8 @@
   FLAME_NLTGV2_OPT_PRESLEEP = 108,
   FLAME_NLTGV2_OPT_XCDS = 109,
   FLAME_NLTGV2_OPT_FAULT_INJECT = 110,
-  FLAME_NLTGV2_OPT_POLL_GAP = 113
+  FLAME_NLTGV2_OPT_POLL_GAP = 113,
+  FLAME_NLTGV2_OPT_XCD_MAP = 114
 };
 
 #endif
diff --git a/flame_amd/csrc/nltgv2_context.hip b/flame_amd/csrc/nltgv2_context.hip
--- a/flame_amd/csrc/nltgv2_context.hip
+++ b/flame_amd/csrc/nltgv2_context.hip
@@ -276,9 +276,12 @@
   if (want_e2)
     LAUNCHCHK(ctx, launch_build_patches2(t.c, t.f, L.wg2_count, t.wg2_info, t.order_m, t.rid_of, t.wg2_vfirst, t.iperm, t.wg2_slot, t.wg2_vid,
                                          t.wg2_meta, t.wg2_nbr, t.wg2_fetch, t.wg2_rmax, stream));
-  if (t.rec_off)
-    LAUNCHCHK(ctx, launch_place_records(t.c, t.f, t.per_xcd, t.order_m, t.rid_of, t.place_patch, (int8_t*)(t.place_patch + t.stride),
+  if (t.rec_off) {
+    LAUNCHCHK(ctx, launch_place_records(t.c, t.f, t.per_xcd, xcd_map::invert(t.xcd_map), ctx->opt_xcd_map != 1, t.order_m, t.rid_of, t.place_patch, (int8_t*)(t.place_patch + t.stride),
                                         (const uint16_t*)ctx->place_rank.p, kPlacePages, t.place_fill, t.rec_off, (int)t.stride, stream));
+    const int rc = pair_w_fetch(ctx, t.place_fill, t.w_slot, stream);
+    if (rc) return rc;
+  }
   return 0;
 }
 
@@ -301,6 +304,7 @@
   }
   if (!launched && placement_applies(ctx, L)) {
     refresh_args(ctx);
+    xcd_map_poll(ctx);
     const int rc = place_records(ctx, (L.wg_count + 7) / 8);
     if (rc) return rc;
   }
@@ -476,6 +480,9 @@
   ok = ok && hipHostMalloc((void**)&ctx->h_err, kErrBytes, hipHostMallocDefault) == hipSuccess;
   ok = ok && hipHostMalloc((void**)&ctx->h_cost, 2 * sizeof(float), hipHostMallocDefault) == hipSuccess;
   ok = ok && hipHostMalloc((void**)&ctx->h_stop, 64, hipHostMallocDefault) == hipSuccess;
+  ok = ok && hipHostMalloc((void**)&ctx->pair_w_slot[0].h, 2 * 64 * sizeof(int32_t), hipHostMallocDefault) == hipSuccess;
+  if (ok) ctx->pair_w_slot[1].h = ctx->pair_w_slot[0].h + 64;
+  for (auto& w : ctx->pair_w_slot) ok = ok && hipEventCreateWithFlags(&w.ev, hipEventDisableTiming) == hipSuccess;
   if (ctx->h_stop) *ctx->h_stop = 0u;
   ok = ok && hipStreamCreateWithPriority(&ctx->ctl_stream, hipStreamNonBlocking, -1) == hipSuccess;
   if (!ok) {
@@ -543,6 +550,9 @@
   if (ctx->topo_stream) (void)hipStreamSynchronize(ctx->topo_stream), (void)hipStreamDestroy(ctx->topo_stream);
   if (ctx->ev_topo_ready) (void)hipEventDestroy(ctx->ev_topo_ready);
   if (ctx->ev_expanded) (void)hipEventDestroy(ctx->ev_expanded);
+  for (auto& w : ctx->pair_w_slot)
+    if (w.ev) (void)hipEventDestroy(w.ev);
+  if (ctx->pair_w_slot[0].h) (void)hipHostFree(ctx->pair_w_slot[0].h);
   if (ctx->raster_stream) (void)hipStreamSynchronize(ctx->raster_stream), (void)hipStreamDestroy(ctx->raster_stream);
   if (ctx->ev_canon) (void)hipEventDestroy(ctx->ev_canon);
   if (ctx->ev_snap) (void)hipEventDestroy(ctx->ev_snap);
@@ -593,6 +603,11 @@
     case FLAME_NLTGV2_OPT_PLACEMENT:
       if (value < 0 || value > 1) return fail(ctx, FLAME_NLTGV2_ERR_INVALID_ARG);
       ctx->opt_place = value;
+      return 0;
+    case FLAME_NLTGV2_OPT_XCD_MAP:
+      if (value < 0 || (value > 2 && value < 16) || (value >= 16 && !xcd_map::is_bijection((unsigned)value))) return fail(ctx, FLAME_NLTGV2_ERR_INVALID_ARG);
+      if (value != ctx->opt_xcd_map) ctx->place_topo = ~0ull;
+      ctx->opt_xcd_map = value, ctx->xcd_map_dirty = true;
       return 0;
     case FLAME_NLTGV2_OPT_POLL_GAP:
       if (value < 0 || value > 256) return fail(ctx, FLAME_NLTGV2_ERR_INVALID_ARG);
@@ -790,6 +805,20 @@
       std::sort(used.begin(), used.end());
       for (size_t i = 1; i < used.size(); ++i) bad += used[i] == used[i - 1];
     }
+    if (ctx->place_cls_dev) {
+      std::vector<int8_t> cls((size_t)V);
+      if (hipMemcpy(cls.data(), ctx->place_cls_dev, (size_t)V, hipMemcpyDeviceToHost) != hipSuccess) return fail(ctx, FLAME_NLTGV2_ERR_HIP);
+      const unsigned inv = xcd_map::invert(ctx->place_map);
+      for (int32_t u = 0; u < V; ++u) {
+        const int32_t r = H.rid_of[(size_t)u], a = patch_of_rec[(size_t)r] / per;
+        int c = -1;
+        for (int32_t h = H.row_ptr[(size_t)u]; h < H.row_ptr[(size_t)u + 1] && c < 0; ++h) {
+          const int32_t b = patch_of_rec[(size_t)H.rid_of[(size_t)H.half_nbr[(size_t)h]]] / per;
+          if (b != a) c = 8 * xcd_map::nibble(inv, a & 7) + xcd_map::nibble(inv, b & 7);
+        }
+        bad += (int)cls[(size_t)r] != c;
+      }
+    }
   }
   *mismatches = bad;
   return FLAME_NLTGV2_OK;
@@ -812,6 +841,24 @@
   return FLAME_NLTGV2_OK;
 }
 
+int flame_nltgv2_xcd_map_info(flame_nltgv2_ctx* ctx, int32_t* map, float* pair_us, int32_t* weight, float* j_us) {
+  int rc = enter(ctx);
+  if (rc) return rc;
+  for (auto& w : ctx->pair_w_slot)
+    if (w.pending && w.topo == ctx->topo && w.ev) HIPCHK(ctx, hipEventSynchronize(w.ev));
+  if (!ctx->pending.active) xcd_map_poll(ctx);
+  float L[64];
+  xcd_map_mean_pair_us(ctx, L);
+  const bool placed = ctx->have_graph && ctx->place_state == 1 && ctx->place_topo == ctx->topo;
+  const unsigned in_use = placed ? ctx->place_map : xcd_map::kIdentity;
+  if (map)
+    for (int x = 0; x < 8; ++x) map[x] = xcd_map::nibble(in_use, x);
+  if (pair_us) std::memcpy(pair_us, L, sizeof L);
+  if (weight) std::memcpy(weight, ctx->pair_w, sizeof ctx->pair_w);
+  if (j_us) j_us[0] = xcd_map::cost(L, ctx->pair_w, xcd_map::kIdentity).j_us(), j_us[1] = xcd_map::cost(L, ctx->pair_w, in_use).j_us();
+  return FLAME_NLTGV2_OK;
+}
+
 int flame_nltgv2_pack_probe(const flame_nltgv2_graph* g, int32_t* perm, int32_t* slice_row, int32_t* rec_nbr,
                             int32_t* rec_edge, int64_t capacity_rows, int64_t* rows_out) {
   PackedLayout L;
diff --git a/flame_amd/csrc/nltgv2_context.hpp b/flame_amd/csrc/nltgv2_context.hpp
--- a/flame_amd/csrc/nltgv2_context.hpp
+++ b/flame_amd/csrc/nltgv2_context.hpp
@@ -19,6 +19,7 @@
 #include "flame_nltgv2_test_options.h"
 #include "nltgv2_kernels.h"
 #include "nltgv2_pack.hpp"
+#include "nltgv2_xcd_map.hpp"
 #include "roctx_ranges.hpp"
 
 namespace flame_hip {
@@ -180,6 +181,22 @@
   float place_best_us = 0.0f, place_mean_us = 0.0f, place_worst_us = 0.0f;
   DevBuf place_pool, place_rank, place_fill, place_rec_off, place_patch, place_meas;
   std::vector<uint16_t> place_rank_host;
+  int opt_xcd_map = 1;
+  bool xcd_map_dirty = false;
+  float place_pair_us[2][64] = {};
+  unsigned xcd_map = 0x76543210u;
+  unsigned place_map = 0x76543210u;
+  unsigned place_map_nx = 0x76543210u;
+  const int8_t* place_cls_dev = nullptr;
+  bool place_cls_from_nx = false;
+  int32_t pair_w[64] = {};
+  uint64_t pair_w_topo = ~0ull;
+  struct PairWSlot {
+    int32_t* h = nullptr;
+    hipEvent_t ev = nullptr;
+    uint64_t topo = ~0ull;
+    bool pending = false;
+  } pair_w_slot[2];
   struct PendingOp {
     int kind = 0;
     flame_nltgv2_params params{};
@@ -403,6 +420,8 @@
   int* place_fill = nullptr;
   int per_xcd = 0;
   size_t stride = 0;
+  unsigned xcd_map = 0x76543210u;
+  int w_slot = 0;
 };
 ExpandTables live_tables(flame_nltgv2_ctx* ctx);
 bool placement_applies(const flame_nltgv2_ctx* ctx, const PackedLayout& L);
@@ -435,6 +454,9 @@
            bool* behind_launched = nullptr);
 int snapshot_chain_start(flame_nltgv2_ctx* ctx);
 int place_records(flame_nltgv2_ctx* ctx, int per_xcd);
+int pair_w_fetch(flame_nltgv2_ctx* ctx, const int* fill, int slot, hipStream_t s);
+void xcd_map_poll(flame_nltgv2_ctx* ctx);
+void xcd_map_mean_pair_us(const flame_nltgv2_ctx* ctx, float* L);
 int place_calibrate(flame_nltgv2_ctx* ctx);
 void place_pool_release(flame_nltgv2_ctx* ctx);
 bool cooperative_allowed();
diff --git a/flame_amd/csrc/nltgv2_kernels.h b/flame_amd/csrc/nltgv2_kernels.h
--- a/flame_amd/csrc/nltgv2_kernels.h
+++ b/flame_amd/csrc/nltgv2_kernels.h
@@ -95,6 +95,7 @@
   const int32_t* rec_off = nullptr;
   int rec_off_stride = 0;
   unsigned* rot_word = nullptr;
+  unsigned xcd_map = 0x76543210u;
   unsigned* probe = nullptr;
   int* abort_flag = nullptr;
   int* err = nullptr;
@@ -108,8 +109,9 @@
                           int presleep, int dual, int xcds, const RunTail* tail, bool cooperative,
                           hipStream_t stream);
 constexpr int kPlacePages = 96;
+constexpr int kPlaceFillInts = 2 * kPlacePages + 16 + 128 + 64;
 int launch_place_calibrate(char* pool, int n_pages, int iters, unsigned* out, int* xcc_out, int* fail, hipStream_t s);
-int launch_place_records(const CanonArgs& c, const FusedArgs& a, int per_xcd, const int32_t* order_m, const int32_t* rid_of,
+int launch_place_records(const CanonArgs& c, const FusedArgs& a, int per_xcd, unsigned inv, bool report, const int32_t* order_m, const int32_t* rid_of,
                          int32_t* patch_of_rec, int8_t* cls, const uint16_t* ranking, int n_pages, int* fill, int32_t* rec_off,
                          int stride, hipStream_t s);
 constexpr uint32_t kScatterFill = 0xffffffffu;
diff --git a/flame_amd/csrc/nltgv2_layout.hip b/flame_amd/csrc/nltgv2_layout.hip
--- a/flame_amd/csrc/nltgv2_layout.hip
+++ b/flame_amd/csrc/nltgv2_layout.hip
@@ -306,27 +306,34 @@
                         int32_t* __restrict__ rec_off, const int stride, int* __restrict__ fill, const int n_fill) {
   const int p = blockIdx.x * blockDim.x + threadIdx.x;
   if (p < n_fill) fill[p] = 0;
-  if (p < 128) fill[n_fill + 16 + p] = 0;
+  if (p < 128 + 64) fill[n_fill + 16 + p] = 0;
   if (p >= n_patches) return;
   const int r0 = wg_info[4 * p], n = wg_info[4 * p + 2] & 0xffff;
   for (int i = 0; i < n; ++i) patch_of_rec[r0 + i] = p, rec_off[r0 + i] = -1, rec_off[stride + r0 + i] = -1;
 }
 
-__global__ void __launch_bounds__(256)
-k_place_classify(const int V, const int per_xcd, const int32_t* __restrict__ order_m, const int32_t* __restrict__ rid_of,
+__device__ __forceinline__ int place_shifts(const int d) {
+  return d <= 8 ? 7 : d <= 10 ? 9 : d <= 12 ? 11 : d <= 16 ? 15 : 15 + 19 * ((d - 1) / 16);
+}
+
+__global__ void __launch_bounds__(256)
+k_place_classify(const int V, const int n_patches, const int per_xcd, const unsigned inv, const int32_t* __restrict__ order_m, const int32_t* __restrict__ rid_of,
                  const int32_t* __restrict__ row_ptr, const uint32_t* __restrict__ half, const int32_t* __restrict__ src,
-                 const int32_t* __restrict__ dst, const int32_t* __restrict__ patch_of_rec, int8_t* __restrict__ cls) {
+                 const int32_t* __restrict__ dst, const int32_t* __restrict__ patch_of_rec, const int32_t* __restrict__ wg_info,
+                 int8_t* __restrict__ cls, int* __restrict__ pair_w) {
   const int r = blockIdx.x * blockDim.x + threadIdx.x;
   if (r >= V) return;
   const int o = order_m[r];
-  const int a = patch_of_rec[r] / per_xcd;
+  const int pa = patch_of_rec[r], a = pa / per_xcd;
   int c = -1;
-  for (int h = row_ptr[o]; h < row_ptr[o + 1] && c < 0; ++h) {
+  for (int h = row_ptr[o]; h < row_ptr[o + 1] && (c < 0 || pair_w != nullptr); ++h) {
     const uint32_t hh = half[h];
     const int e = (int)(hh & ~kRole);
     const int other = (hh & kRole) ? src[e] : dst[e];
-    const int xb = patch_of_rec[rid_of[other]] / per_xcd;
-    if (xb != a) c = a * 8 + xb;
+    const int pb = patch_of_rec[rid_of[other]], xb = pb / per_xcd;
+    if (xb == a || (unsigned)pa >= (unsigned)n_patches || (unsigned)pb >= (unsigned)n_patches || a > 7 || xb > 7) continue;
+    if (c < 0) c = (int)((inv >> (4 * a)) & 7u) * 8 + (int)((inv >> (4 * xb)) & 7u);
+    if (pair_w != nullptr) atomicMax(&pair_w[8 * a + xb], 1 + place_shifts(wg_info[4 * pa + 3]) + place_shifts(wg_info[4 * pb + 3]));
   }
   cls[r] = (int8_t)c;
 }
@@ -384,15 +391,15 @@
   return (int)hipGetLastError();
 }
 
-int launch_place_records(const CanonArgs& c, const FusedArgs& a, int per_xcd, const int32_t* order_m, const int32_t* rid_of,
+int launch_place_records(const CanonArgs& c, const FusedArgs& a, int per_xcd, unsigned inv, bool report, const int32_t* order_m, const int32_t* rid_of,
                          int32_t* patch_of_rec, int8_t* cls, const uint16_t* ranking, int n_pages, int* fill, int32_t* rec_off,
                          int stride, hipStream_t s) {
   if (a.wg_count <= 0 || per_xcd <= 0) return 0;
   const int n0 = a.wg_count > 2 * n_pages ? a.wg_count : 2 * n_pages;
   hipLaunchKernelGGL(k_place_patch_of_record, grid1d(n0), dim3(256), 0, s, a.wg_count, a.wg_info, patch_of_rec, rec_off, stride, fill,
                      2 * n_pages);
-  hipLaunchKernelGGL(k_place_classify, grid1d(c.V), dim3(256), 0, s, c.V, per_xcd, order_m, rid_of, c.row_ptr, c.half, c.src, c.dst,
-                     patch_of_rec, cls);
+  hipLaunchKernelGGL(k_place_classify, grid1d(c.V), dim3(256), 0, s, c.V, a.wg_count, per_xcd, inv, order_m, rid_of, c.row_ptr, c.half, c.src, c.dst,
+                     patch_of_rec, a.wg_info, cls, report ? fill + 2 * n_pages + 16 + 128 : nullptr);
   hipLaunchKernelGGL(k_place_assign, dim3((unsigned)a.wg_count), dim3(64), 0, s, a.wg_count, a.wg_info, cls, ranking, n_pages, fill, rec_off,
                      stride);
   return (int)hipGetLastError();
diff --git a/flame_amd/csrc/nltgv2_persistent.hip b/flame_amd/csrc/nltgv2_persistent.hip
--- a/flame_amd/csrc/nltgv2_persistent.hip
+++ b/flame_amd/csrc/nltgv2_persistent.hip
@@ -17,7 +17,7 @@
                 const unsigned max_spins_arg, const int poll_gap_arg, const SolverParams p,
                 int* __restrict__ err, int* __restrict__ abort_flag, const int32_t* __restrict__ perm,
                 const RunTail* __restrict__ tail, unsigned* __restrict__ probe, char* place_pool,
-                const int32_t* __restrict__ rec_off, const int rec_off_stride, unsigned* rot_word) {
+                const int32_t* __restrict__ rec_off, const int rec_off_stride, unsigned* rot_word, const unsigned xcd_map) {
   extern __shared__ float4 lds[];
   constexpr int T = 64;
   const unsigned max_spins = max_spins_arg & 0x7fffffffu;
@@ -44,10 +44,10 @@
     b += (int)(v & 7u);
     if (b >= (int)gridDim.x) b -= (int)gridDim.x;
   }
-  const int xcd = b & 7, idx = b >> 3;
+  const int group = (int)((xcd_map >> (4 * (b & 7))) & 7u), idx = b >> 3;
   if (idx >= wgs_per_xcd) return;
-  if (xcd * wgs_per_xcd + idx >= n_wgs) return;
-  const int wg = wg_begin + xcd * wgs_per_xcd + idx;
+  if (group * wgs_per_xcd + idx >= n_wgs) return;
+  const int wg = wg_begin + group * wgs_per_xcd + idx;
   const int rid_base = wg_info[4 * wg], n_fetch = wg_info[4 * wg + 1];
   const int count_flags = wg_info[4 * wg + 2];
   if ((count_flags & 0xffff) == 0) return;
@@ -514,10 +514,11 @@
     const int32_t* rec_off = a.rec_off;
     int rec_off_stride = a.rec_off_stride;
     unsigned* rot_word = place_pool ? a.rot_word : nullptr;
+    unsigned xcd_map = place_pool ? a.xcd_map : 0x76543210u;
     const unsigned ldsv = pv_lds_bytes(lcap, slab_slots);
     void* vargs[] = {&wave_begin, &n_waves, &wgx, &lcap, &slab_slots, &w0, &w1, &w2, &w3, &w4, &w5, &hrec, &hq, &vstate,
                      &hq_out, &vstate_out, &vaux, &bin, &bout, &vprev, &xbuf, &rec_bytes, &dual, &tag0, &n_iters,
-                     &max_spins, &poll_gap, &pp, &err, &abort_flag, &perm, &tail, &probe, &place_pool, &rec_off, &rec_off_stride, &rot_word};
+                     &max_spins, &poll_gap, &pp, &err, &abort_flag, &perm, &tail, &probe, &place_pool, &rec_off, &rec_off_stride, &rot_word, &xcd_map};
     const bool vr = (dual >> 1) != 0;
     if (!a.wg_rowpack) return (int)hipErrorInvalidConfiguration;
     const void* fv = probe ? (const void*)k_persistent_pv<true, true>
diff --git a/flame_amd/csrc/nltgv2_run.hip b/flame_amd/csrc/nltgv2_run.hip
--- a/flame_amd/csrc/nltgv2_run.hip
+++ b/flame_amd/csrc/nltgv2_run.hip
@@ -256,6 +256,7 @@
   void* mem = nullptr;
   std::vector<uint16_t> rank;
   float best = 0.f, mean = 0.f, worst = 0.f;
+  float pair_us[2][64] = {};
 };
 std::mutex& g_place_mu = *new std::mutex;
 std::vector<PlacePool>& g_place_free = *new std::vector<PlacePool>;
@@ -277,6 +278,7 @@
   PlacePool e;
   e.device = ctx->device, e.mem = ctx->place_pool.p, e.rank.swap(ctx->place_rank_host);
   e.best = ctx->place_best_us, e.mean = ctx->place_mean_us, e.worst = ctx->place_worst_us;
+  std::memcpy(e.pair_us, ctx->place_pair_us, sizeof e.pair_us);
   ctx->device_bytes -= ctx->place_pool.cap;
   ctx->place_pool = DevBuf{};
   ctx->place_base = nullptr, ctx->place_state = 0;
@@ -303,13 +305,14 @@
       ctx->place_pool.p = e.mem, ctx->place_pool.cap = pool_bytes + 4096;
       ctx->device_bytes += ctx->place_pool.cap;
       ctx->place_best_us = e.best, ctx->place_mean_us = e.mean, ctx->place_worst_us = e.worst;
+      std::memcpy(ctx->place_pair_us, e.pair_us, sizeof e.pair_us);
       ctx->place_rank_host.swap(e.rank);
       int rc = ensure(ctx, ctx->place_rank, sizeof(uint16_t) * 2 * 64 * P);
-      if (!rc) rc = ensure(ctx, ctx->place_fill, sizeof(int) * (2 * P + 16 + 128));
+      if (!rc) rc = ensure(ctx, ctx->place_fill, sizeof(int) * kPlaceFillInts);
       if (rc) return rc;
       ctx->place_base = reinterpret_cast<char*>((reinterpret_cast<uintptr_t>(ctx->place_pool.p) + 4095) & ~uintptr_t(4095));
       HIPCHK(ctx, hipMemsetAsync(ctx->place_base, 0, pool_bytes, ctx->stream));
-      HIPCHK(ctx, hipMemsetAsync(ctx->place_fill.p, 0, sizeof(int) * (2 * P + 16 + 128), ctx->stream));
+      HIPCHK(ctx, hipMemsetAsync(ctx->place_fill.p, 0, sizeof(int) * kPlaceFillInts, ctx->stream));
       HIPCHK(ctx, hipMemcpyAsync(ctx->place_rank.p, ctx->place_rank_host.data(), sizeof(uint16_t) * ctx->place_rank_host.size(), hipMemcpyHostToDevice,
                                  ctx->stream));
       HIPCHK(ctx, wait_solver_stream(ctx));
@@ -320,7 +323,7 @@
   int rc = ensure(ctx, ctx->place_pool, pool_bytes + 4096);
   if (!rc) rc = ensure(ctx, ctx->place_meas, sizeof(unsigned) * 64 * 2 * P + sizeof(int) * 64 + sizeof(int));
   if (!rc) rc = ensure(ctx, ctx->place_rank, sizeof(uint16_t) * 2 * 64 * P);
-  if (!rc) rc = ensure(ctx, ctx->place_fill, sizeof(int) * (2 * P + 16 + 128));
+  if (!rc) rc = ensure(ctx, ctx->place_fill, sizeof(int) * kPlaceFillInts);
   if (rc) return rc;
   ctx->place_base = reinterpret_cast<char*>((reinterpret_cast<uintptr_t>(ctx->place_pool.p) + 4095) & ~uintptr_t(4095));
   unsigned* d_out = (unsigned*)ctx->place_meas.p;
@@ -328,7 +331,7 @@
   int* d_fail = d_xcc + 64;
   HIPCHK(ctx, hipMemsetAsync(ctx->place_base, 0, pool_bytes, ctx->stream));
   HIPCHK(ctx, hipMemsetAsync(ctx->place_meas.p, 0, sizeof(unsigned) * 64 * 2 * P + sizeof(int) * 65, ctx->stream));
-  HIPCHK(ctx, hipMemsetAsync(ctx->place_fill.p, 0, sizeof(int) * (2 * P + 16 + 128), ctx->stream));
+  HIPCHK(ctx, hipMemsetAsync(ctx->place_fill.p, 0, sizeof(int) * kPlaceFillInts, ctx->stream));
   LAUNCHCHK(ctx, launch_place_calibrate(ctx->place_base, 2 * P, kIters, d_out, d_xcc, d_fail, ctx->stream));
   std::vector<unsigned> out((size_t)64 * 2 * P);
   int xcc[65];
@@ -365,6 +368,7 @@
       double m = 0.0;
       for (int t = 0; t < P; ++t) m += l[t];
       best += l[r[0]], worst += l[r[P - 1]], mean += m / P;
+      ctx->place_pair_us[par][c] = (float)(l[r[0]] / (100.0 * kIters));
     }
   if (std::getenv("FLAME_NLTGV2_TRACE")) {
     for (int a = 0; a < 8; ++a) {
@@ -390,15 +394,60 @@
 
 int place_records(flame_nltgv2_ctx* ctx, int per_xcd) {
   const size_t stride = records_capacity(ctx->L);
+  const unsigned map = ctx->xcd_map;
   int rc = ensure(ctx, ctx->place_rec_off, sizeof(int32_t) * 2 * stride);
   if (!rc) rc = ensure(ctx, ctx->place_patch, sizeof(int32_t) * stride + stride);
   if (rc) return rc;
-  LAUNCHCHK(ctx, launch_place_records(ctx->c, ctx->f, per_xcd, (const int32_t*)ctx->order_m.p, (const int32_t*)ctx->rid_of.p,
+  LAUNCHCHK(ctx, launch_place_records(ctx->c, ctx->f, per_xcd, xcd_map::invert(map), ctx->opt_xcd_map != 1, (const int32_t*)ctx->order_m.p, (const int32_t*)ctx->rid_of.p,
                                       (int32_t*)ctx->place_patch.p, (int8_t*)((int32_t*)ctx->place_patch.p + stride),
                                       (const uint16_t*)ctx->place_rank.p, kPlacePages, (int*)ctx->place_fill.p,
                                       (int32_t*)ctx->place_rec_off.p, (int)stride, ctx->stream));
-  ctx->place_topo = ctx->topo, ctx->place_per_xcd = per_xcd;
-  return 0;
+  ctx->place_topo = ctx->topo, ctx->place_per_xcd = per_xcd, ctx->place_map = map;
+  ctx->place_cls_dev = (const int8_t*)((const int32_t*)ctx->place_patch.p + stride), ctx->place_cls_from_nx = false;
+  return pair_w_fetch(ctx, (const int*)ctx->place_fill.p, 0, ctx->stream);
+}
+
+int pair_w_fetch(flame_nltgv2_ctx* ctx, const int* fill, int slot, hipStream_t s) {
+  flame_nltgv2_ctx::PairWSlot& w = ctx->pair_w_slot[slot];
+  if (!w.h || !w.ev || ctx->opt_xcd_map == 1) return 0;
+  HIPCHK(ctx, hipMemcpyAsync(w.h, fill + 2 * kPlacePages + 16 + 128, sizeof(int32_t) * 64, hipMemcpyDeviceToHost, s));
+  HIPCHK(ctx, hipEventRecord(w.ev, s));
+  w.topo = slot == 0 ? ctx->topo : ~0ull;
+  w.pending = true;
+  return 0;
+}
+
+void xcd_map_mean_pair_us(const flame_nltgv2_ctx* ctx, float* L) {
+  for (int c = 0; c < 64; ++c) L[c] = 0.5f * (ctx->place_pair_us[0][c] + ctx->place_pair_us[1][c]);
+}
+
+void xcd_map_poll(flame_nltgv2_ctx* ctx) {
+  bool fresh = ctx->xcd_map_dirty;
+  for (int pass = 0; pass < 2; ++pass)
+    for (auto& w : ctx->pair_w_slot) {
+      if (!w.pending || w.topo == ~0ull || (w.topo == ctx->topo) != (pass == 1)) continue;
+      const hipError_t e = hipEventQuery(w.ev);
+      if (e != hipSuccess) {
+        (void)hipGetLastError();
+        continue;
+      }
+      std::memcpy(ctx->pair_w, w.h, sizeof ctx->pair_w);
+      ctx->pair_w_topo = w.topo, w.pending = false, fresh = true;
+    }
+  if (!fresh) return;
+  ctx->xcd_map_dirty = false;
+  unsigned map = xcd_map::kIdentity;
+  if (ctx->opt_xcd_map >= 16) {
+    map = (unsigned)ctx->opt_xcd_map;
+  } else if (ctx->opt_xcd_map != 1 && ctx->place_state == 1 && ctx->pair_w_topo != ~0ull) {
+    float L[64];
+    xcd_map_mean_pair_us(ctx, L);
+    map = xcd_map::choose(L, ctx->pair_w, ctx->opt_xcd_map == 2);
+    if (std::getenv("FLAME_NLTGV2_TRACE"))
+      std::fprintf(stderr, "[flame_nltgv2] XCD map 0x%08x (nibble x: the group on XCD x): J %.3f us, identity %.3f us\n", map,
+                   (double)xcd_map::cost(L, ctx->pair_w, map).j_us(), (double)xcd_map::cost(L, ctx->pair_w, xcd_map::kIdentity).j_us());
+  }
+  ctx->xcd_map = map;
 }
 
 static bool open_run_applies(const flame_nltgv2_ctx* ctx, int form, const std::vector<WaveGroup>& groups) {
@@ -522,14 +571,15 @@
         const int dense_gap = denser ? kPvDenserGap : kPvDenseGap, dense_pre = denser ? kPvDenserPreSleep : kPvDensePreSleep;
         const int gap = ctx->opt_poll_gap > 0 ? ctx->opt_poll_gap - 1 : dense ? (3 | ((dense_gap - 1) << 4)) : kPvPollGap;
         ctx->f.wg_poll_gap = gap | ((ctx->opt_presleep > 0 ? ctx->opt_presleep - 1 : dense ? dense_pre : kPvPreSleep) << 8);
-        ctx->f.rec_off = nullptr, ctx->f.place_pool = nullptr;
+        ctx->f.rec_off = nullptr, ctx->f.place_pool = nullptr, ctx->f.xcd_map = xcd_map::kIdentity;
         if (ctx->opt_place && groups.size() == 1 && gr.begin == 0 && xcds == 8 && (dual & 1)) {
           if (ctx->place_state == 0) {
             rc = place_calibrate(ctx);
             if (rc) return rc;
           }
           const int per_xcd = (gr.count + xcds - 1) / xcds;
-          if (ctx->place_state == 1 && (ctx->place_topo != ctx->topo || ctx->place_per_xcd != per_xcd)) {
+          if (!ctx->pending.active) xcd_map_poll(ctx);
+          if (ctx->place_state == 1 && (ctx->place_topo != ctx->topo || ctx->place_per_xcd != per_xcd || ctx->place_map != ctx->xcd_map)) {
             rc = place_records(ctx, per_xcd);
             if (rc) return rc;
           }
@@ -537,6 +587,7 @@
             ctx->f.place_pool = ctx->place_base, ctx->f.rec_off = (const int32_t*)ctx->place_rec_off.p;
             ctx->f.rec_off_stride = (int)records_capacity(ctx->L);
             ctx->f.rot_word = (unsigned*)ctx->place_fill.p + 2 * kPlacePages;
+            ctx->f.xcd_map = ctx->place_map;
           }
         }
         ctx->f.probe = nullptr;
diff --git a/flame_amd/csrc/nltgv2_topo_capi.hip b/flame_amd/csrc/nltgv2_topo_capi.hip
--- a/flame_amd/csrc/nltgv2_topo_capi.hip
+++ b/flame_amd/csrc/nltgv2_topo_capi.hip
@@ -342,6 +342,7 @@
   Ln.wg2_walked = true, Ln.wg2_ok = dm.max_degree <= 32 && dm.wg2_count > 0, Ln.wg2_count = dm.wg2_count, Ln.wg2_lcap = dm.wg2_lcap;
   Ln.tv_ok = false, Ln.tv_waves = 0;
   const bool want_e2 = wants_e2(ctx, Ln) && Ln.wg2_ok && Ln.wg2_count <= kPv2WavesPerCu * cus * 4;
+  if (!ctx->pending.active) xcd_map_poll(ctx);
   const bool placed = placement_applies(ctx, Ln);
   int rc = 0;
   {
@@ -359,10 +360,11 @@
     for (auto& r : req)
       if (r.bytes && (rc = ensure(ctx, ctx->ex[r.i], r.bytes)) != 0) return rc;
     if (placed) {
+      if (ctx->place_cls_from_nx) ctx->place_cls_dev = nullptr;
       rc = ensure(ctx, ctx->place_patch_nx, sizeof(int32_t) * stride + stride);
       if (!rc && ctx->place_fill_nx.cap == 0) {
-        rc = ensure(ctx, ctx->place_fill_nx, sizeof(int) * (2 * kPlacePages + 16 + 128));
-        if (!rc) HIPCHK(ctx, hipMemsetAsync(ctx->place_fill_nx.p, 0, sizeof(int) * (2 * kPlacePages + 16 + 128), ts));
+        rc = ensure(ctx, ctx->place_fill_nx, sizeof(int) * kPlaceFillInts);
+        if (!rc) HIPCHK(ctx, hipMemsetAsync(ctx->place_fill_nx.p, 0, sizeof(int) * kPlaceFillInts, ts));
       }
       if (rc) return rc;
     }
@@ -388,6 +390,7 @@
     if (placed) {
       t.rec_off = (int32_t*)ctx->ex[C::EX_PLACE_REC_OFF].p, t.place_patch = (int32_t*)ctx->place_patch_nx.p, t.place_fill = (int*)ctx->place_fill_nx.p;
       t.per_xcd = (Ln.wg_count + 7) / 8, t.stride = stride;
+      t.xcd_map = ctx->place_map_nx = ctx->xcd_map, t.w_slot = 1;
     }
     std::vector<StageFill> fills;
     expansion_fills(Ln, t.f.rec_edge, t.f.rec_nbr, want_e2 ? t.wg2_rmax : nullptr, &fills);
@@ -448,7 +451,11 @@
   if (rc) return rc;
   rc = topology_expand(ctx, want_e2, true);
   if (rc) return rc;
-  if (placed) ctx->place_topo = ctx->topo, ctx->place_per_xcd = (L.wg_count + 7) / 8;
+  if (placed) {
+    ctx->place_topo = ctx->topo, ctx->place_per_xcd = (L.wg_count + 7) / 8, ctx->place_map = ctx->place_map_nx;
+    ctx->place_cls_dev = (const int8_t*)((const int32_t*)ctx->place_patch_nx.p + records_capacity(L)), ctx->place_cls_from_nx = true;
+    if (ctx->pair_w_slot[1].pending) ctx->pair_w_slot[1].topo = ctx->topo;
+  }
   HIPCHK(ctx, hipStreamWaitEvent(ctx->stream, ctx->ev_expanded, 0));
   for (int i = 0; i < 9; ++i) std::swap(*cur_v[i], ctx->sp_v[i]);
   for (int i = 0; i < 3; ++i) std::swap(*cur_q[i], ctx->sp_q[i]);
diff --git a/flame_amd/csrc/nltgv2_xcd_map.hpp b/flame_amd/csrc/nltgv2_xcd_map.hpp
--- /dev/null
+++ b/flame_amd/csrc/nltgv2_xcd_map.hpp
@@ -0,0 +1,157 @@
+#ifndef FLAME_NLTGV2_XCD_MAP_HPP_
+#define FLAME_NLTGV2_XCD_MAP_HPP_
+
+#include <algorithm>
+#include <cstdint>
+
+namespace flame_hip {
+namespace xcd_map {
+
+constexpr unsigned kIdentity = 0x76543210u;
+constexpr double kShiftUs = 26.0 / 2400.0;
+
+inline int nibble(unsigned word, int i) { return (int)((word >> (4 * i)) & 15u); }
+
+inline unsigned pack(const int* m) {
+  unsigned w = 0;
+  for (int i = 0; i < 8; ++i) w |= (unsigned)(m[i] & 15) << (4 * i);
+  return w;
+}
+
+inline bool is_bijection(unsigned word) {
+  unsigned seen = 0;
+  for (int i = 0; i < 8; ++i) {
+    const int g = nibble(word, i);
+    if (g > 7) return false;
+    seen |= 1u << g;
+  }
+  return seen == 0xffu;
+}
+
+inline unsigned invert(unsigned word) {
+  int inv[8] = {0, 1, 2, 3, 4, 5, 6, 7};
+  for (int x = 0; x < 8; ++x) inv[nibble(word, x) & 7] = x;
+  return pack(inv);
+}
+
+inline int shifts_of_degree(int d) {
+  if (d <= 8) return 7;
+  if (d <= 10) return 9;
+  if (d <= 12) return 11;
+  if (d <= 16) return 15;
+  return 15 + 19 * ((d - 1) / 16);
+}
+
+inline int64_t q_pair(const float* L, int xa, int xb) { return (int64_t)((double)L[8 * xa + xb] * 1e6 + 0.5); }
+inline int64_t q_weight(const int32_t* W, int a, int b) { return (int64_t)(0.5 * kShiftUs * (double)(W[8 * a + b] - 1) * 1e6 + 0.5); }
+
+inline bool usable(const float* L, const int32_t* W) {
+  if (!L || !W) return false;
+  bool any = false;
+  for (int a = 0; a < 8; ++a)
+    for (int b = 0; b < 8; ++b)
+      if (a != b) {
+        if (!(L[8 * a + b] > 0.0f) || !(L[8 * a + b] < 1e6f)) return false;
+        any = any || W[8 * a + b] > 0;
+      }
+  return any;
+}
+
+struct Cost {
+  int64_t j = 0, sum = 0;
+  float j_us() const { return (float)((double)j * 1e-6); }
+};
+
+inline Cost cost(const float* L, const int32_t* W, unsigned word) {
+  Cost c;
+  if (!usable(L, W) || !is_bijection(word)) return c;
+  const unsigned inv = invert(word);
+  for (int a = 0; a < 8; ++a)
+    for (int b = 0; b < 8; ++b)
+      if (a != b && W[8 * a + b] > 0) {
+        const int64_t t = q_pair(L, nibble(inv, a), nibble(inv, b)) + q_weight(W, a, b);
+        c.j = std::max(c.j, t), c.sum += t;
+      }
+  return c;
+}
+
+namespace detail {
+struct Search {
+  int64_t ql[64], qw[64];
+  struct Entry {
+    int64_t q;
+    int hi;
+  } sorted[56];
+  int map[8];
+  bool have = false;
+  Cost best;
+  unsigned best_word = kIdentity;
+  void go(int x, unsigned used, int64_t j, int64_t sum, int left, int64_t w_left) {
+    if (x == 8) {
+      if (!have || j < best.j || (j == best.j && sum < best.sum)) have = true, best.j = j, best.sum = sum, best_word = pack(map);
+      return;
+    }
+    for (int g = 0; g < 8; ++g) {
+      if (used & (1u << g)) continue;
+      int64_t j2 = j, s2 = sum, w2 = w_left;
+      int left2 = left;
+      for (int y = 0; y < x; ++y) {
+        const int h = map[y];
+        if (qw[8 * g + h] >= 0) {
+          const int64_t t = ql[8 * x + y] + qw[8 * g + h];
+          j2 = std::max(j2, t), s2 += t, w2 -= qw[8 * g + h], --left2;
+        }
+        if (qw[8 * h + g] >= 0) {
+          const int64_t t = ql[8 * y + x] + qw[8 * h + g];
+          j2 = std::max(j2, t), s2 += t, w2 -= qw[8 * h + g], --left2;
+        }
+      }
+      if (have) {
+        if (j2 > best.j) continue;
+        if (j2 == best.j) {
+          int64_t lb = s2 + w2;
+          int n = left2;
+          for (int i = 0; i < 56 && n > 0; ++i)
+            if (sorted[i].hi > x) lb += sorted[i].q, --n;
+          if (lb >= best.sum) continue;
+        }
+      }
+      map[x] = g;
+      go(x + 1, used | (1u << g), j2, s2, left2, w2);
+    }
+  }
+};
+}
+
+inline unsigned choose(const float* L, const int32_t* W, bool worst = false) {
+  if (!usable(L, W)) return kIdentity;
+  if (worst) {
+    int m[8] = {0, 1, 2, 3, 4, 5, 6, 7};
+    unsigned best_word = kIdentity;
+    Cost best = cost(L, W, kIdentity);
+    while (std::next_permutation(m, m + 8)) {
+      const Cost c = cost(L, W, pack(m));
+      if (c.j > best.j || (c.j == best.j && c.sum > best.sum)) best = c, best_word = pack(m);
+    }
+    return best_word;
+  }
+  detail::Search s;
+  int left = 0, n = 0;
+  int64_t w_left = 0;
+  for (int a = 0; a < 8; ++a)
+    for (int b = 0; b < 8; ++b) {
+      const bool used = a != b && W[8 * a + b] > 0;
+      s.ql[8 * a + b] = a != b ? q_pair(L, a, b) : 0;
+      s.qw[8 * a + b] = used ? q_weight(W, a, b) : -1;
+      if (used) ++left, w_left += s.qw[8 * a + b];
+      if (a != b) s.sorted[n].q = s.ql[8 * a + b], s.sorted[n].hi = std::max(a, b), ++n;
+    }
+  std::sort(s.sorted, s.sorted + 56, [](const detail::Search::Entry& u, const detail::Search::Entry& v) { return u.q < v.q; });
+  s.go(0, 0u, 0, 0, left, w_left);
+  return s.best_word;
+}
+
+}
+}
+
+#endif
diff --git a/flame_amd/regularizer.py b/flame_amd/regularizer.py
--- a/flame_amd/regularizer.py
+++ b/flame_amd/regularizer.py
@@ -12,7 +12,7 @@
 _IP = C.POINTER(C.c_int32)
 
 OPT_SOLVER, OPT_USE_HIPGRAPH, OPT_PERSISTENT, OPT_PROBE, OPT_VERIFY_RECORDS, OPT_PLACEMENT, OPT_SYNC_PATH, OPT_COST_SUM, OPT_MESH_STATE = 1, 2, 5, 12, 14, 16, 17, 18, 19
-OPT_BLOCK_WAVES, OPT_UNROLL, OPT_DUAL_PUBLISH, OPT_PRESLEEP, OPT_XCDS, OPT_FAULT_INJECT, OPT_POLL_GAP = 103, 104, 106, 108, 109, 110, 113
+OPT_BLOCK_WAVES, OPT_UNROLL, OPT_DUAL_PUBLISH, OPT_PRESLEEP, OPT_XCDS, OPT_FAULT_INJECT, OPT_POLL_GAP, OPT_XCD_MAP = 103, 104, 106, 108, 109, 110, 113, 114
 RUN_PATHS = {0: "none", 1: "persistent (the lane-per-half-edge form, retired in round 3)", 2: "per-step hipGraph", 3: "per-step eager", 4: "canonical 4-sweep",
              5: "persistent-tv", 6: "persistent-pv", 7: "persistent-pv2"}
 ERR_NAN = -5
@@ -119,7 +119,7 @@
     "flame_nltgv2_costs", "flame_nltgv2_download_state", "flame_nltgv2_export_idepth_device",
     "flame_nltgv2_export_idepth_device_async", "flame_nltgv2_set_export_target",
     "flame_nltgv2_set_option", "flame_nltgv2_get_info", "flame_nltgv2_last_error", "flame_nltgv2_last_hip_error",
-    "flame_nltgv2_status_string", "flame_nltgv2_abi_version", "flame_nltgv2_pack_probe", "flame_nltgv2_read_probe", "flame_nltgv2_layout_selftest", "flame_nltgv2_placement_info",
+    "flame_nltgv2_status_string", "flame_nltgv2_abi_version", "flame_nltgv2_pack_probe", "flame_nltgv2_read_probe", "flame_nltgv2_layout_selftest", "flame_nltgv2_placement_info", "flame_nltgv2_xcd_map_info",
     "flame_nltgv2_photo_set_images", "flame_nltgv2_photo_residual", "flame_nltgv2_photo_fuse",
     "flame_nltgv2_photo_residual_last", "flame_nltgv2_sync_graph", "flame_nltgv2_sync_prepare", "flame_nltgv2_sync_commit",
     "flame_nltgv2_get_topology", "flame_nltgv2_graph_size", "flame_nltgv2_set_feature_ids", "flame_nltgv2_interpolate_mesh",
@@ -177,6 +177,7 @@
         "flame_nltgv2_abi_version": (C.c_int, []),
         "flame_nltgv2_layout_selftest": (C.c_int, [ctx, C.POINTER(C.c_int64)]),
         "flame_nltgv2_placement_info": (C.c_int, [ctx, C.POINTER(C.c_int32), C.POINTER(C.c_int32), C.POINTER(C.c_float)]),
+        "flame_nltgv2_xcd_map_info": (C.c_int, [ctx, C.POINTER(C.c_int32), C.POINTER(C.c_float), C.POINTER(C.c_int32), C.POINTER(C.c_float)]),
         "flame_nltgv2_pack_probe": (C.c_int, [GP, _IP, _IP, _IP, _IP, C.c_int64, C.POINTER(C.c_int64)]),
         "flame_nltgv2_read_probe": (C.c_int, [ctx, C.POINTER(C.c_uint32), C.c_int64, C.POINTER(C.c_int64)]),
         "flame_nltgv2_photo_set_images": (C.c_int, [ctx, C.POINTER(C.c_uint8), C.POINTER(C.c_uint8), C.c_int, C.c_int, C.c_int]),
@@ -372,6 +373,13 @@
         return {"state": int(st.value), "placed_records": int(n.value), "best_us": float(us[0]), "mean_us": float(us[1]),
                 "worst_us": float(us[2])}
 
+    def xcd_map_info(self) -> dict:
+        m, w = (C.c_int32 * 8)(), (C.c_int32 * 64)()
+        L, j = (C.c_float * 64)(), (C.c_float * 2)()
+        self._chk(self._L.flame_nltgv2_xcd_map_info(self._ctx, m, L, w, j), "xcd_map_info")
+        return {"map": [int(v) for v in m], "packed": sum(int(v) << (4 * x) for x, v in enumerate(m)), "pair_us": [float(v) for v in L],
+                "weight": [int(v) for v in w], "j_identity_us": float(j[0]), "j_map_us": float(j[1])}
+
     def layout_selftest(self) -> int:
         n = C.c_int64(-1)
         self._chk(self._L.flame_nltgv2_layout_selftest(self._ctx, C.byref(n)), "layout_selftest")
diff --git a/include/flame_nltgv2.h b/include/flame_nltgv2.h
--- a/include/flame_nltgv2.h
+++ b/include/flame_nltgv2.h
@@ -246,6 +246,8 @@
 
 int flame_nltgv2_placement_info(flame_nltgv2_ctx* ctx, int32_t* state, int32_t* placed_records, float* us);
 
+int flame_nltgv2_xcd_map_info(flame_nltgv2_ctx* ctx, int32_t map[8], float pair_us[64], int32_t weight[64], float j_us[2]);
+
 int flame_nltgv2_layout_selftest(flame_nltgv2_ctx* ctx, int64_t* mismatches);
 int flame_nltgv2_pack_probe(const flame_nltgv2_graph* g, int32_t* perm, int32_t* slice_row,
                             int32_t* rec_nbr, int32_t* rec_edge, int64_t capacity_rows, int64_t* rows_out);
```
